# 0xPolygonHermez/pil2-stark-js

Measured on AMD Instinct MI355X. Metric: STARK prove time (ms_per_step) and trace-cells/s, synthetic Fibonacci AIR, GL Poseidon Merkle + FRI, blow-up 8, higher is better.
Workload: dtype u64; 1 GPU; full proof (commit, Q, evals, FRI 27/22/17/12/7, 64 queries) of 2^24 rows x 100 cols -> 2^27 rows, plain linear hash, per GPU; mode=prove, config=c3, nBits=24, nCols=100, nBitsExt=27, hash=GL-Poseidon-12, parallelism=single GPU

## Files before the change

### include/pil2gl.h

```cpp
#pragma once
#include <stdint.h>
#include "pil2gl_expr.h"
#include "pil2gl_bn_expr.h"
#ifdef __cplusplus
extern "C" {
#endif

#define PIL2GL_OK        0
#define PIL2GL_EINVAL   -1
#define PIL2GL_ENODEV   -2
#define PIL2GL_ENOMEM   -3
#define PIL2GL_EHIP     -4

int         pil2gl_init(int device);
void        pil2gl_shutdown(void);
const char *pil2gl_last_error(void);
int         pil2gl_version(void);
int         pil2gl_device_info(char *name, uint32_t nameLen, uint32_t *numCUs, uint64_t *totalMem);

int pil2gl_dev_alloc(uint64_t nWords, uint64_t **out);
int pil2gl_dev_free(uint64_t *p);
int pil2gl_dev_zero(uint64_t *p, uint64_t nWords, void *stream);
int pil2gl_dev_upload(uint64_t *dst, const uint64_t *hostSrc, uint64_t nWords);
int pil2gl_dev_download(uint64_t *hostDst, const uint64_t *src, uint64_t nWords);
int pil2gl_sync(void *stream);

int pil2gl_host_alloc(uint64_t nWords, uint64_t **out);
int pil2gl_host_free(uint64_t *p);
int pil2gl_host_register(uint64_t *p, uint64_t nWords);
int pil2gl_host_unregister(uint64_t *p);
int pil2gl_dev_upload_async(uint64_t *dst, const uint64_t *hostSrc, uint64_t nWords);
int pil2gl_dev_download_async(uint64_t *hostDst, const uint64_t *src, uint64_t nWords);
int pil2gl_copy_after(void *stream);
int pil2gl_copy_fence(void *stream);
int pil2gl_copy_sync(void);
int pil2gl_land_rows_dev(const uint64_t *src, uint64_t srcCols, uint64_t *dst, uint64_t dstCols, uint64_t nRows,
                         uint64_t *hostFirstBad, void *stream);
int pil2gl_dev_load_file(const char *fileName, uint64_t byteOffset, uint64_t nRows, uint64_t srcCols,
                         uint64_t *dst, uint64_t dstCols, uint64_t chunkWords, uint64_t *hostFirstBad);
int pil2gl_dev_save_file(const char *fileName, uint64_t byteOffset, const uint64_t *src, uint64_t nWords, uint64_t chunkWords);

int pil2gl_interpolate(const uint64_t *src, uint64_t nPols, uint32_t nBits, uint64_t *dst, uint32_t nBitsExt);
int pil2gl_interpolate_dev(const uint64_t *src, uint64_t nPols, uint32_t nBits, uint64_t *dst, uint32_t nBitsExt, void *stream);
int pil2gl_interpolate_cosets_dev(const uint64_t *src, uint64_t nPols, uint32_t nBits, uint64_t *dst, uint32_t nBitsExt,
                                  uint32_t cosetBegin, uint32_t cosetCount, void *stream);
int pil2gl_extend_cosets_unshifted_dev(const uint64_t *src, uint64_t nPols, uint32_t nBits, uint64_t *dst, uint32_t nBitsExt,
                                       uint32_t cosetBegin, uint32_t cosetCount, void *stream);
int pil2gl_extend_coefs_brev_dev(const uint64_t *coefBrev, uint64_t nPols, uint32_t nBits, uint64_t *dst, uint32_t nBitsExt, void *stream);
int pil2gl_extend_coefs_brev_cosets_dev(const uint64_t *coefBrev, uint64_t nPols, uint32_t nBits, uint64_t *dst, uint32_t nBitsExt,
                                        uint32_t cosetBegin, uint32_t cosetCount, void *stream);
int pil2gl_interpolate_cosets_ws_dev(const uint64_t *src, uint64_t nPols, uint32_t nBits, uint64_t *dst, uint32_t nBitsExt,
                                     uint32_t cosetBegin, uint32_t cosetCount, uint64_t *workspace, void *stream);
int pil2gl_fft(const uint64_t *src, uint64_t nPols, uint32_t nBits, uint64_t *dst);
int pil2gl_ifft(const uint64_t *src, uint64_t nPols, uint32_t nBits, uint64_t *dst);
int pil2gl_fft_dev(const uint64_t *src, uint64_t nPols, uint32_t nBits, uint64_t *dst, void *stream);
int pil2gl_ifft_dev(const uint64_t *src, uint64_t nPols, uint32_t nBits, uint64_t *dst, void *stream);
int pil2gl_fft_block_dev(uint64_t *buf, uint64_t start_pos, uint64_t nPols, uint32_t nBits, uint32_t s, uint32_t blockBits, uint32_t layers, void *stream);
int pil2gl_interpolate_prepare_block_dev(uint64_t *buf, uint64_t width, uint64_t height, uint64_t start, uint64_t inc, void *stream);

int pil2gl_poseidon(const uint64_t *in, const uint64_t *cap, uint64_t count, uint32_t nOut, uint64_t *out);
int pil2gl_poseidon_dev(const uint64_t *in, const uint64_t *cap, uint64_t count, uint32_t nOut, uint64_t *out, void *stream);
int pil2gl_sponge_absorb(const uint64_t *hostBlocks, uint64_t nBlocks, const uint64_t hostCap[4], uint64_t hostOut12[12]);
int pil2gl_linear_hash_rows(const uint64_t *in, uint64_t width, uint64_t height, int split, uint64_t *out);
int pil2gl_linear_hash_rows_dev(const uint64_t *in, uint64_t width, uint64_t height, int split, uint64_t *out, void *stream);
int pil2gl_merkelize_level(const uint64_t *in, uint64_t nOps, uint64_t *out);
int pil2gl_merkelize_level_dev(const uint64_t *in, uint64_t nOps, uint64_t *out, void *stream);
uint64_t pil2gl_merkle_num_nodes(uint64_t height);
int pil2gl_merkelize(const uint64_t *elems, uint64_t width, uint64_t height, int split, uint64_t *nodes);
int pil2gl_merkelize_dev(const uint64_t *elems, uint64_t width, uint64_t height, int split, uint64_t *nodes, void *stream);
int pil2gl_merkelize_digests_dev(uint64_t *nodes, uint64_t height, void *stream);
int pil2gl_group_proof_dev(const uint64_t *elems, const uint64_t *nodes, uint64_t width, uint64_t height,
                           uint64_t idx, uint64_t *hostVals, uint64_t *hostSiblings, uint32_t *nLevels);

int pil2gl_group_proofs_dev(const uint64_t *elems, const uint64_t *nodes, uint64_t width, uint64_t height,
                            const uint64_t *hostIdxs, uint32_t nIdx, uint64_t *hostOut, uint32_t *nLevels);
int pil2gl_roots_from_group_proofs(const uint64_t *hostProofs, uint64_t width, uint32_t levels, const uint64_t *hostIdxs, uint32_t nIdx,
                                   int splitLinearHash, uint64_t *hostRoots );

int pil2gl_fri_fold(const uint64_t *pol, uint32_t polBits, uint32_t outBits, uint64_t shiftInv,
                    const uint64_t challenge[3], uint64_t *out);
int pil2gl_fri_fold_dev(const uint64_t *pol, uint32_t polBits, uint32_t outBits, uint64_t shiftInv,
                        const uint64_t challenge[3], uint64_t *out, void *stream);
int pil2gl_fri_verify_fold(const uint64_t *groups, uint32_t foldBits, uint32_t nQueries, const uint64_t *sinv,
                           const uint64_t challenge[3], uint64_t *out );
int pil2gl_fri_verify_fold_dev(const uint64_t *groups, uint32_t foldBits, uint32_t nQueries, const uint64_t *sinv,
                               const uint64_t challenge[3], uint64_t *out, void *stream);
int pil2gl_fri_transpose(const uint64_t *pol, uint32_t polBits, uint32_t transposeBits, uint64_t *out);
int pil2gl_fri_transpose_dev(const uint64_t *pol, uint32_t polBits, uint32_t transposeBits, uint64_t *out, void *stream);

int pil2gl_build_x_dev(uint32_t nBits, uint64_t shift, uint64_t *x, void *stream);
int pil2gl_geometric_dev(uint64_t first, uint64_t ratio, uint64_t n, uint64_t *out, void *stream);
int pil2gl_build_zhinv_dev(uint32_t nBits, uint32_t nBitsExt, uint64_t *out, void *stream);
int pil2gl_build_one_row_zerofier_inv_dev(uint32_t nBits, uint32_t nBitsExt, uint64_t rowIndex, uint64_t *out, void *stream);
int pil2gl_build_frame_zerofier_dev(uint32_t nBits, uint32_t nBitsExt, uint64_t offsetMin, uint64_t offsetMax, uint64_t *out, void *stream);
int pil2gl_compute_q_split_dev(const uint64_t *qq1, uint32_t nBits, uint32_t nBitsExt, uint32_t qDim, uint32_t qDeg, uint64_t *qq2, void *stream);
int pil2gl_compute_q_split_brev_dev(const uint64_t *qq1, uint32_t nBits, uint32_t nBitsExt, uint32_t qDim, uint32_t qDeg, uint64_t *coefBrev, void *stream);
int pil2gl_compute_q_stark_dev(const glx_program *prog, const glx_ctx *ctx, uint32_t qSection, uint32_t nBits, uint32_t nBitsExt,
                               uint32_t qDim, uint32_t qDeg, uint64_t *dstExt, void *stream);
int pil2gl_x_div_x_sub_xi_dev(uint32_t nBitsExt, const uint64_t xi[3], uint64_t nOpen, uint64_t iOpen, uint64_t *out, void *stream);
int pil2gl_x_div_x_sub_xi_cosets_dev(uint32_t nBitsExt, uint32_t extBits, const uint64_t xi[3], uint64_t nOpen, uint64_t iOpen,
                                     uint32_t cosetBegin, uint32_t cosetCount, uint64_t *out, void *stream);
int pil2gl_build_lev_dev(uint32_t nBits, const uint64_t xi[3], uint64_t *lev, void *stream);
typedef struct { const uint64_t *buf; uint64_t width; uint64_t offset; uint32_t dim; uint32_t levIndex; } pil2gl_eval_desc;
int pil2gl_compute_evals_dev(const pil2gl_eval_desc *descs, uint32_t nEvals, uint32_t nBits, uint32_t extendBits,
                             const uint64_t *const *levs, uint32_t nLevs, uint64_t *hostEvals , void *stream);

int pil2gl_rows_dot_ext_dev(const uint64_t *buf, uint64_t width, uint64_t nRows, const uint64_t *hostCoef, uint32_t nOut,
                            uint64_t *acc, int accumulate, void *stream);
int pil2gl_rows_dot_ext_multi_dev(const uint64_t *const *bufs, const uint64_t *widths, uint32_t nBufs, uint64_t nRows,
                                  const uint64_t *const *hostCoefs, uint32_t nOut, uint64_t *acc, int accumulate, void *stream);
int pil2gl_rows_dot_ext_multi_step_dev(const uint64_t *const *bufs, const uint64_t *widths, uint32_t nBufs, uint64_t nRows, uint32_t rowStepBits,
                                       const uint64_t *const *hostCoefs, uint32_t nOut, uint64_t *acc, int accumulate, void *stream);
int pil2gl_fri_combine_dev(const uint64_t *acc, const uint64_t *hostK, const uint64_t vf1[3], const uint64_t *xDivXSubXi,
                           uint32_t nOpen, uint64_t nRows, uint64_t *f, void *stream);
int pil2gl_fri_combine_order_dev(const uint64_t *acc, const uint64_t *hostK, const uint64_t vf1[3], const uint64_t *xDivXSubXi,
                                 uint32_t nOpen, const uint32_t *order, uint64_t nRows, uint64_t *f, void *stream);
int pil2gl_compute_fri_pol_dev(const uint64_t *const *bufs, const uint64_t *widths, uint32_t nBufs, const uint64_t *const *hostCoefs, uint32_t nOpen,
                               const uint64_t *hostK, const uint64_t vf1[3], const uint32_t *order, const uint64_t *xis,
                               uint32_t nBits, uint32_t nBitsExt, uint64_t *fExt, void *stream);
int pil2gl_cols_dot_ext_dev(const uint64_t *buf, uint64_t width, uint64_t nRows, uint64_t rowStep, const uint64_t *const *levs,
                            uint32_t nLev, uint64_t *hostOut, void *stream);
int pil2gl_cols_dot_ext_multi_dev(const uint64_t *const *bufs, const uint64_t *widths, uint32_t nBufs, uint64_t nRows, uint64_t rowStep,
                                  const uint64_t *const *levs, uint32_t nLev, uint64_t *const *hostOuts, void *stream);
int pil2gl_cols_dot_ext_range_dev(const uint64_t *const *bufs, const uint64_t *strides, const uint64_t *colBegin, const uint64_t *widths, uint32_t nBufs,
                                  uint64_t nRows, uint64_t rowStep, const uint64_t *const *levs, uint32_t nLev, uint64_t *const *hostOuts, void *stream);

int pil2gl_eval_program_dev(const glx_program *prog, const glx_ctx *ctx, void *stream);
int pil2gl_jit_cache_set_dir(const char *dir);
int pil2gl_jit_cache_stats(uint64_t out[8]);
int pil2gl_precompile_program(const glx_program *prog, const glx_ctx *ctx, uint32_t outInfo[4]);
int pil2gl_precompile_q_stark(const glx_program *prog, const glx_ctx *ctx, uint32_t qSection, uint32_t nBits, uint32_t nBitsExt,
                              uint32_t qDim, uint32_t qDeg, uint32_t outInfo[4]);
int pil2gl_first_nonzero_row_dev(const uint64_t *col, uint32_t dim, uint64_t first, uint64_t last, uint64_t *hostRow, uint64_t *hostVal, void *stream);

int pil2gl_gprod_dev(const uint64_t *num, uint32_t dimNum, const uint64_t *den, uint32_t dimDen, uint64_t n, uint64_t *out, void *stream);
int pil2gl_gsum_dev(const uint64_t *num, uint32_t dimNum, const uint64_t *den, uint32_t dimDen, uint64_t n, uint64_t *out, void *stream);
int pil2gl_h1h2_dev(const uint64_t *f, const uint64_t *t, uint64_t n, uint32_t dim, uint64_t *h1, uint64_t *h2, void *stream);
int pil2gl_debug_hint_plan(uint64_t n, uint32_t *outInfo );
uint64_t pil2gl_debug_h1h2_home(const uint64_t *words, uint32_t dim, uint64_t capacity);

int pil2gl_bn128_poseidon(const uint64_t *in, const uint64_t *init, uint64_t count, uint32_t nIn, uint32_t nOut, uint64_t *out);
int pil2gl_bn128_sponge_absorb(const uint64_t *hostBlocks, uint64_t nBlocks, uint32_t nIn, const uint64_t hostInit[4], uint64_t *hostOut);
int pil2gl_bn128_poseidon_dev(const uint64_t *in, const uint64_t *init, uint64_t count, uint32_t nIn, uint32_t nOut, uint64_t *out, void *stream);
int pil2gl_bn128_linear_hash_rows(const uint64_t *in, uint64_t width, uint64_t height, uint32_t arity, int custom, uint64_t *out);
int pil2gl_bn128_linear_hash_rows_dev(const uint64_t *in, uint64_t width, uint64_t height, uint32_t arity, int custom, uint64_t *out, void *stream);
int pil2gl_bn128_merkelize_level_dev(const uint64_t *in, uint64_t nOps, uint32_t arity, uint64_t *out, void *stream);
uint64_t pil2gl_bn128_merkle_num_nodes(uint64_t height, uint32_t arity);
int pil2gl_bn128_merkelize(const uint64_t *elems, uint64_t width, uint64_t height, uint32_t arity, int custom, uint64_t *nodes);
int pil2gl_bn128_merkelize_dev(const uint64_t *elems, uint64_t width, uint64_t height, uint32_t arity, int custom, uint64_t *nodes, void *stream);
int pil2gl_bn128_group_proof_dev(const uint64_t *elems, const uint64_t *nodes, uint64_t width, uint64_t height, uint32_t arity,
                                 uint64_t idx, uint64_t *hostVals, uint64_t *hostSiblings, uint32_t *nLevels);
int pil2gl_bn128_group_proofs_dev(const uint64_t *elems, const uint64_t *nodes, uint64_t width, uint64_t height, uint32_t arity,
                                  const uint64_t *hostIdxs, uint32_t nIdx, uint64_t *hostVals, uint64_t *hostSiblings, uint32_t *nLevels);
int pil2gl_bn128_roots_from_group_proofs(const uint64_t *hostVals, const uint64_t *hostSiblings, uint64_t width, uint32_t levels, uint32_t arity,
                                         int custom, int siblingsMontgomery, const uint64_t *hostIdxs, uint32_t nIdx, uint64_t *hostRoots );
int pil2gl_bn128_convert(const uint64_t *in, uint64_t n, int toMontgomery, uint64_t *out);
int pil2gl_bn128_convert_dev(const uint64_t *in, uint64_t n, int toMontgomery, uint64_t *out, void *stream);

int pil2gl_bn128_fft(const uint64_t *src, uint64_t nPols, uint32_t nBits, uint64_t *dst);
int pil2gl_bn128_ifft(const uint64_t *src, uint64_t nPols, uint32_t nBits, uint64_t *dst);
int pil2gl_bn128_interpolate(const uint64_t *src, uint64_t nPols, uint32_t nBits, uint64_t *dstCoefs, uint64_t *dst, uint32_t nBitsExt);
int pil2gl_bn128_fft_dev(const uint64_t *src, uint64_t nPols, uint32_t nBits, uint64_t *dst, void *stream);
int pil2gl_bn128_ifft_dev(const uint64_t *src, uint64_t nPols, uint32_t nBits, uint64_t *dst, void *stream);
int pil2gl_bn128_interpolate_dev(const uint64_t *src, uint64_t nPols, uint32_t nBits, uint64_t *dstCoefs, uint64_t *dst, uint32_t nBitsExt, void *stream);
int pil2gl_debug_bn128_fft_plan(uint32_t nBits, uint32_t *layersPerSweep, uint32_t room, uint32_t *nSweeps);
uint32_t pil2gl_debug_bn128_fft_tile_bytes(void);

int pil2gl_bn128_g1_msm(const uint64_t *bases, const uint64_t *scalars, uint64_t n, uint64_t scalarStride, uint32_t scalarsMontgomery, uint64_t *out);
int pil2gl_bn128_g1_msm_dev(const uint64_t *bases, const uint64_t *scalars, uint64_t n, uint64_t scalarStride, uint32_t scalarsMontgomery,
                            uint64_t *out, void *stream);
int pil2gl_debug_bn128_msm_plan(uint64_t n, uint32_t *out, uint64_t *scratchBytes);
#define PIL2GL_G1_EMPTY_SLOT 0xFFFFFFFFu
typedef struct { uint64_t first, rows; uint32_t m, reserved; } pil2gl_g1_poly;
int pil2gl_bn128_g1_commit(const uint64_t *bases, uint64_t nBases, const uint64_t *scalars, uint64_t rowStride, uint32_t scalarsMontgomery,
                           const pil2gl_g1_poly *polys, uint32_t K, const uint32_t *slots, uint64_t *out);
int pil2gl_bn128_g1_commit_dev(const uint64_t *bases, uint64_t nBases, const uint64_t *scalars, uint64_t rowStride, uint32_t scalarsMontgomery,
                               const pil2gl_g1_poly *polys, uint32_t K, const uint32_t *slots, uint64_t *out, void *stream);
int pil2gl_debug_bn128_msm_batch_plan(uint32_t K, const uint64_t *counts, uint32_t *out, uint64_t *scratchBytes);
int pil2gl_debug_bn128_commit_locate(const pil2gl_g1_poly *polys, uint32_t K, const uint32_t *slots, uint64_t rowStride, uint64_t lane, uint64_t out[4]);
int pil2gl_debug_bn128_msm_digits(const uint64_t scalar[4], uint32_t c, int32_t *digits, uint32_t room, uint32_t *nDigits);

int pil2gl_bn128_eval_program(const glx_program *prog, const bnx_ctx *ctx);
int pil2gl_bn128_eval_program_dev(const glx_program *prog, const bnx_ctx *ctx, void *stream);
int pil2gl_bn128_first_nonzero_row_dev(const uint64_t *col, uint64_t width, uint64_t column, uint64_t first, uint64_t last,
                                       uint64_t *hostRow, uint64_t *hostVal, void *stream);
int pil2gl_debug_bn128_plan_program(const glx_program *prog, const bnx_ctx *ctx, uint32_t *outInfo );

int pil2gl_bn128_poly_div_xk_sub(const uint64_t *src, uint64_t n, uint64_t stride, uint64_t k, const uint64_t hostBeta[4], uint64_t *dst);
int pil2gl_bn128_poly_div_xk_sub_dev(const uint64_t *src, uint64_t n, uint64_t stride, uint64_t k, const uint64_t hostBeta[4], uint64_t *dst, void *stream);
int pil2gl_bn128_poly_eval(const uint64_t *src, uint64_t n, uint64_t stride, const uint64_t *hostPoints, uint32_t nPoints, uint64_t *out);
int pil2gl_bn128_poly_eval_dev(const uint64_t *src, uint64_t n, uint64_t stride, const uint64_t *hostPoints, uint32_t nPoints, uint64_t *out, void *stream);
int pil2gl_debug_bn128_poly_plan(uint64_t n, uint64_t k, uint32_t *outInfo , uint64_t *scratchBytes);

int pil2gl_bn128_poly_fma(uint64_t *acc, uint64_t nAcc, uint64_t accStride, const uint64_t *hostScale ,
                          const uint64_t *src, uint64_t nSrc, uint64_t srcStride,
                          const uint64_t *hostCoefs , const uint64_t *hostExps , uint32_t t);
int pil2gl_bn128_poly_fma_dev(uint64_t *acc, uint64_t nAcc, uint64_t accStride, const uint64_t *hostScale ,
                              const uint64_t *src, uint64_t nSrc, uint64_t srcStride,
                              const uint64_t *hostCoefs , const uint64_t *hostExps , uint32_t t, void *stream);
int pil2gl_bn128_poly_degree(const uint64_t *src, uint64_t n, uint64_t stride, uint64_t *degree);
int pil2gl_bn128_poly_degree_dev(const uint64_t *src, uint64_t n, uint64_t stride, uint64_t *degree, void *stream);

int pil2gl_bn128_batch_inverse(const uint64_t *src, uint64_t srcStride, uint64_t n, uint64_t *dst, uint64_t dstStride);
int pil2gl_bn128_batch_inverse_dev(const uint64_t *src, uint64_t srcStride, uint64_t n, uint64_t *dst, uint64_t dstStride, void *stream);
int pil2gl_bn128_gprod(const uint64_t *num, uint64_t numStride, const uint64_t *den, uint64_t denStride, uint64_t n,
                       uint64_t *out, uint64_t outStride);
int pil2gl_bn128_gprod_dev(const uint64_t *num, uint64_t numStride, const uint64_t *den, uint64_t denStride, uint64_t n,
                           uint64_t *out, uint64_t outStride, void *stream);
int pil2gl_bn128_gsum(const uint64_t hostNum[4], const uint64_t *den, uint64_t denStride, uint64_t n, uint64_t *out, uint64_t outStride);
int pil2gl_bn128_gsum_dev(const uint64_t hostNum[4], const uint64_t *den, uint64_t denStride, uint64_t n,
                          uint64_t *out, uint64_t outStride, void *stream);
int pil2gl_debug_bn128_scan_plan(uint64_t n, uint32_t op, uint32_t *outInfo , uint64_t *scratchBytes);

int pil2gl_bn128_h1h2(const uint64_t *f, uint64_t fStride, const uint64_t *t, uint64_t tStride, uint64_t n,
                      uint64_t *h1, uint64_t h1Stride, uint64_t *h2, uint64_t h2Stride, uint64_t *missingRow);
int pil2gl_bn128_h1h2_dev(const uint64_t *f, uint64_t fStride, const uint64_t *t, uint64_t tStride, uint64_t n,
                          uint64_t *h1, uint64_t h1Stride, uint64_t *h2, uint64_t h2Stride, uint64_t *missingRow, void *stream);
int pil2gl_debug_bn128_h1h2_plan(uint64_t n, uint32_t *outInfo , uint64_t *scratchBytes);

int pil2gl_wtns_adds_plan(const uint64_t *hostAddIdx, uint64_t idxStride, uint64_t nAdds, uint64_t nWitness, const uint64_t *hostCoef,
                          uint64_t coefStride, uint32_t coefWords, uint32_t *outAdds, uint64_t *outCoef, uint32_t *outLevelStart,
                          uint32_t levelCap, uint32_t *nLevels);
int pil2gl_wtns_adds_dev(uint64_t *w, uint64_t nWitness, const uint32_t *adds, const uint64_t *coefs, uint64_t nAdds,
                         const uint32_t *hostLevelStart, uint32_t nLevels, void *stream);
int pil2gl_bn128_wtns_adds_dev(uint64_t *w, uint64_t nWitness, const uint32_t *adds, const uint64_t *coefs, uint64_t nAdds,
                               const uint32_t *hostLevelStart, uint32_t nLevels, void *stream);
int pil2gl_wtns_gather_dev(const uint64_t *w, uint64_t nW, const uint32_t *sMap32, uint64_t nRows, uint64_t nCols, uint64_t *dst,
                           uint64_t dstCols, uint64_t *hostFirstBad, void *stream);
int pil2gl_bn128_wtns_gather_dev(const uint64_t *w, uint64_t nW, const uint32_t *sMap32, uint64_t nRows, uint64_t nCols, uint64_t *dst,
                                 uint64_t dstCols, int toMontgomery, uint64_t *hostFirstBad, void *stream);
int pil2gl_wtns_exec(const uint64_t *hostW, uint64_t nWitness, const uint64_t *hostAddIdx, const uint64_t *hostAddCoef, uint64_t nAdds,
                     const uint64_t *hostSMap64, uint64_t nRows, uint64_t nCols, uint64_t *hostDst);
int pil2gl_bn128_wtns_exec(const uint64_t *hostW, uint64_t nWitness, const uint64_t *hostAddIdx, const uint64_t *hostAddCoef, uint64_t nAdds,
                           const uint64_t *hostSMap64, uint64_t nRows, uint64_t nCols, uint64_t *hostDst, int toMontgomery);
int pil2gl_debug_wtns_plan(const uint64_t *hostAddIdx, uint64_t idxStride, uint64_t nAdds, uint64_t nWitness, uint32_t *outInfo ,
                           uint32_t *outWidths, uint32_t widthCap);

#define PIL2GL_CONN_SMAP_ROWS_U64 0
#define PIL2GL_CONN_SMAP_COLS_U32 1
int pil2gl_conn_plan(uint64_t nRows, uint64_t nCols, uint64_t nW, uint64_t N, uint32_t elemWords, uint32_t *outInfo , uint64_t *scratchBytes);
int pil2gl_conn_pols_dev(const uint32_t *sMap32, uint64_t nRows, uint64_t nCols, uint64_t nW, uint64_t N, const uint64_t *hostW, const uint64_t *hostKs1,
                         uint64_t *dst, uint64_t dstStride, uint64_t dstOffset, uint64_t *scratch, uint64_t scratchBytes, uint64_t *hostFirstBad,
                         void *stream);
int pil2gl_bn128_conn_pols_dev(const uint32_t *sMap32, uint64_t nRows, uint64_t nCols, uint64_t nW, uint64_t N, const uint64_t *hostW,
                               const uint64_t *hostKs1, uint64_t *dst, uint64_t dstStride, uint64_t dstOffset, uint64_t *scratch, uint64_t scratchBytes,
                               uint64_t *hostFirstBad, void *stream);
int pil2gl_conn_pols(const void *hostSMap, int sMapLayout, uint64_t nRows, uint64_t nCols, uint64_t nW, uint64_t N, const uint64_t *hostW,
                     const uint64_t *hostKs1, uint64_t *hostDst);
int pil2gl_bn128_conn_pols(const void *hostSMap, int sMapLayout, uint64_t nRows, uint64_t nCols, uint64_t nW, uint64_t N, const uint64_t *hostW,
                           const uint64_t *hostKs1, uint64_t *hostDst);

int pil2gl_conn_check_plan(uint64_t N, uint64_t nCols, uint32_t elemWords, uint32_t *outInfo , uint64_t *scratchBytes);
int pil2gl_conn_check_dev(const uint64_t *a, uint64_t aStride, uint64_t aOffset, const uint64_t *S, uint64_t sStride, uint64_t sOffset, uint64_t N,
                          uint64_t nCols, const uint64_t *hostW, const uint64_t *hostKs1, uint64_t *scratch, uint64_t scratchBytes,
                          uint64_t *hostReport , void *stream);
int pil2gl_bn128_conn_check_dev(const uint64_t *a, uint64_t aStride, uint64_t aOffset, const uint64_t *S, uint64_t sStride, uint64_t sOffset, uint64_t N,
                                uint64_t nCols, const uint64_t *hostW, const uint64_t *hostKs1, uint64_t *scratch, uint64_t scratchBytes,
                                uint64_t *hostReport , void *stream);
int pil2gl_conn_check(const uint64_t *hostA, const uint64_t *hostS, uint64_t N, uint64_t nCols, const uint64_t *hostW, const uint64_t *hostKs1,
                      uint64_t *hostReport );
int pil2gl_bn128_conn_check(const uint64_t *hostA, const uint64_t *hostS, uint64_t N, uint64_t nCols, const uint64_t *hostW, const uint64_t *hostKs1,
                            uint64_t *hostReport );
uint64_t pil2gl_debug_conn_check_probe(void);

int pil2gl_tuple_check_plan(uint64_t n, uint64_t k, uint32_t elemWords, uint32_t mode, uint32_t *outInfo , uint64_t *scratchBytes);
int pil2gl_tuple_check_dev(const uint64_t *f, uint64_t fStride, const uint64_t *hostFCols, const uint64_t *t, uint64_t tStride,
                           const uint64_t *hostTCols, const uint64_t *selF, uint64_t selFStride, uint64_t selFCol, const uint64_t *selT,
                           uint64_t selTStride, uint64_t selTCol, uint64_t n, uint64_t k, uint32_t mode, uint64_t *scratch,
                           uint64_t scratchBytes, uint64_t *hostReport , void *stream);
int pil2gl_bn128_tuple_check_dev(const uint64_t *f, uint64_t fStride, const uint64_t *hostFCols, const uint64_t *t, uint64_t tStride,
                                 const uint64_t *hostTCols, const uint64_t *selF, uint64_t selFStride, uint64_t selFCol, const uint64_t *selT,
                                 uint64_t selTStride, uint64_t selTCol, uint64_t n, uint64_t k, uint32_t mode, uint64_t *scratch,
                                 uint64_t scratchBytes, uint64_t *hostReport , void *stream);
int pil2gl_tuple_check(const uint64_t *hostF, uint64_t fStride, const uint64_t *hostFCols, const uint64_t *hostT, uint64_t tStride,
                       const uint64_t *hostTCols, const uint64_t *hostSelF, uint64_t selFStride, uint64_t selFCol, const uint64_t *hostSelT,
                       uint64_t selTStride, uint64_t selTCol, uint64_t n, uint64_t k, uint32_t mode, uint64_t *hostReport );
int pil2gl_bn128_tuple_check(const uint64_t *hostF, uint64_t fStride, const uint64_t *hostFCols, const uint64_t *hostT, uint64_t tStride,
                             const uint64_t *hostTCols, const uint64_t *hostSelF, uint64_t selFStride, uint64_t selFCol,
                             const uint64_t *hostSelT, uint64_t selTStride, uint64_t selTCol, uint64_t n, uint64_t k, uint32_t mode,
                             uint64_t *hostReport );
uint64_t pil2gl_debug_tuple_home(const uint64_t *words, uint64_t k, uint32_t elemWords, uint64_t capacity);
uint64_t pil2gl_debug_tuple_check_probe(void);

typedef struct pil2gl_tuple_side {
    const uint64_t *base;
    uint64_t stride;
    const uint64_t *hostCols;
    const uint64_t *sel;
    uint64_t selStride, selCol;
} pil2gl_tuple_side;
int pil2gl_lookup_mult_plan(uint64_t n, uint64_t k, uint64_t nF, uint32_t elemWords, uint32_t *outInfo , uint64_t *scratchBytes);
int pil2gl_lookup_mult_dev(const pil2gl_tuple_side *hostF, uint64_t nF, const pil2gl_tuple_side *hostT, uint64_t *m, uint64_t mStride,
                           uint64_t mCol, uint64_t n, uint64_t k, uint64_t *scratch, uint64_t scratchBytes, uint64_t *hostReport ,
                           void *stream);
int pil2gl_bn128_lookup_mult_dev(const pil2gl_tuple_side *hostF, uint64_t nF, const pil2gl_tuple_side *hostT, uint64_t *m, uint64_t mStride,
                                 uint64_t mCol, uint64_t n, uint64_t k, uint64_t *scratch, uint64_t scratchBytes,
                                 uint64_t *hostReport , void *stream);
int pil2gl_lookup_mult(const pil2gl_tuple_side *hostF, uint64_t nF, const pil2gl_tuple_side *hostT, uint64_t *hostM, uint64_t mStride,
                       uint64_t mCol, uint64_t n, uint64_t k, uint64_t *hostReport );
int pil2gl_bn128_lookup_mult(const pil2gl_tuple_side *hostF, uint64_t nF, const pil2gl_tuple_side *hostT, uint64_t *hostM, uint64_t mStride,
                             uint64_t mCol, uint64_t n, uint64_t k, uint64_t *hostReport );
uint64_t pil2gl_debug_lookup_mult_probe(void);

int pil2gl_synth_fibonacci_dev(uint32_t nBits, uint32_t nPairs, const uint64_t *hostInit, uint64_t *cm, void *stream);

uint64_t pil2gl_add(uint64_t a, uint64_t b);
uint64_t pil2gl_mul(uint64_t a, uint64_t b);
uint64_t pil2gl_square(uint64_t a);

int pil2gl_selftest_field(const uint64_t *a, const uint64_t *b, uint64_t n, uint64_t *mul, uint64_t *add, uint64_t *sub);
int pil2gl_debug_compact_program(const glx_program *prog, glx_op *outOps, uint32_t *outInfo);
int pil2gl_debug_jit_compile(const glx_program *prog, const glx_ctx *ctx, uint64_t *codeBytes, uint32_t *fusedOps);
int pil2gl_debug_plan_program(const glx_program *prog, const glx_ctx *ctx, uint32_t *outInfo);
uint64_t pil2gl_debug_bn128_path_launches(void);
#define PIL2GL_PLAN_FFT 0
#define PIL2GL_PLAN_IFFT 1
#define PIL2GL_PLAN_INTERPOLATE 2
#define PIL2GL_PLAN_EXTEND_COEFS 3
#define PIL2GL_PLAN_LAUNCH_WORDS 14
int pil2gl_debug_plan_transform(uint32_t op, uint32_t nBits, uint64_t nPols, uint32_t nBitsExt, uint32_t cosetCount,
                                uint32_t *out, uint32_t maxLaunches, uint32_t *nLaunches);
#define PIL2GL_PLAN_GRID_WORDS 5
int pil2gl_debug_plan_transform_grid(uint32_t op, uint32_t nBits, uint64_t nPols, uint32_t nBitsExt, uint32_t cosetCount,
                                     uint32_t *out, uint32_t maxLaunches, uint32_t *nLaunches);
int pil2gl_debug_transform_walk(uint32_t op, uint32_t nBits, uint64_t nPols, uint32_t nBitsExt, uint32_t cosetCount, uint32_t launch,
                                uint32_t firstBlock, uint32_t count, uint32_t *out);
int pil2gl_debug_transform_walk_cover(uint32_t op, uint32_t nBits, uint64_t nPols, uint32_t nBitsExt, uint32_t cosetCount, uint32_t launch,
                                      uint64_t *counts);
int pil2gl_selftest_products(const uint64_t *a, const uint64_t *b, uint64_t n, uint64_t *x, uint64_t *pb, uint64_t *flag);
int pil2gl_selftest_mds(const uint64_t *states, uint64_t n, uint32_t layers, int mfma, uint64_t *out);
int pil2gl_selftest_poseidon(const uint64_t *states, uint64_t n, int what, uint64_t *out);
int pil2gl_selftest_clock(uint32_t iters, double *mhz);
int pil2gl_selftest_ext(const uint64_t *a, const uint64_t *b, uint64_t n, uint64_t *mul, uint64_t *inv);

#ifdef __cplusplus
}
#endif
```

### pil2-stark-js_amd/csrc/expr.hip

```cpp
#include "common.h"
#include "gl_field.cuh"
#include <vector>
#include <string.h>
#include <algorithm>
#include <array>
#include <map>
#include <stdlib.h>

using namespace gl;

namespace {

struct DevRef { u32 kind_dim;
                u32 section;
                int32_t rowOff;
                u32 index; };
struct DevOp { u32 op; u32 aux; DevRef dest, src[2]; };

enum { GLX_LZ_BEGIN = 4, GLX_LZ_MAD = 5, GLX_LZ_END = 6 };

#define GLX_MAX_SECTIONS 24
struct DevCtx {
    const DevOp *__restrict__ ops; u32 nOps;
    u32 nBits;
// ... 49 lines not shown
    extern __shared__ u64 lds_tmp[];
    u64 *T; u32 stride;
    if (LDS_TMP) { T = lds_tmp + threadIdx.x; stride = blockDim.x; }
    else { T = gtmp + (size_t)blockIdx.x * blockDim.x + threadIdx.x; stride = gridDim.x * blockDim.x; }
    const u64 nRows = 1ull << c.nBits;
    for (u64 row = (u64)blockIdx.x * blockDim.x + threadIdx.x; row < nRows; row += (u64)gridDim.x * blockDim.x) {
        u64 LZ[3][6];
        for (u32 k = 0; k < c.nOps; k++) {
            const DevOp op = c.ops[k];
            u64 a0, a1, a2, b0 = 0, b1 = 0, b2 = 0, r0, r1, r2;
            if (op.op == GLX_LZ_BEGIN) {
#pragma unroll
                for (int q = 0; q < 3; q++)
#pragma unroll
                    for (int i = 0; i < 6; i++) LZ[q][i] = 0;
                continue;
            }
            if (op.op == GLX_LZ_MAD) {
                load_ref(op.src[0], c, row, T, stride, a0, a1, a2);
                const u32 *L = c.limbs + op.aux;
                lz_mad(LZ, a0, L);
                if ((op.src[0].kind_dim >> 8) == 3) { lz_mad(LZ, a1, L + 9); lz_mad(LZ, a2, L + 18); }
                continue;
            }
            const u32 da = op.src[0].kind_dim >> 8;
            u32 db = 1;
            if (op.op != GLX_LZ_END) load_ref(op.src[0], c, row, T, stride, a0, a1, a2);
            if (op.op < GLX_OP_COPY) { load_ref(op.src[1], c, row, T, stride, b0, b1, b2); db = op.src[1].kind_dim >> 8; }
            if (op.op == GLX_LZ_END) { r0 = fold6(LZ[0]); r1 = fold6(LZ[1]); r2 = fold6(LZ[2]); }
            else if (op.op == GLX_OP_ADD) {
                r0 = add(a0, b0);
                if (da == 3 && db == 3) { r1 = add(a1, b1); r2 = add(a2, b2); }
                else if (da == 3) { r1 = a1; r2 = a2; } else { r1 = b1; r2 = b2; }
            } else if (op.op == GLX_OP_SUB) {
                r0 = sub(a0, b0);
                if (da == 3 && db == 3) { r1 = sub(a1, b1); r2 = sub(a2, b2); }
                else if (da == 3) { r1 = a1; r2 = a2; } else { r1 = neg(b1); r2 = neg(b2); }
            } else if (op.op == GLX_OP_MUL) {
                if (da == 3 && db == 3) { E3 x = { { a0, a1, a2 } }, y = { { b0, b1, b2 } }; E3 z = e3_mul(x, y); r0 = z.v[0]; r1 = z.v[1]; r2 = z.v[2]; }
                else if (da == 3) { r0 = mul(a0, b0); r1 = mul(a1, b0); r2 = mul(a2, b0); }
                else { r0 = mul(a0, b0); r1 = mul(a0, b1); r2 = mul(a0, b2); }
            } else { r0 = a0; r1 = a1; r2 = a2; }
            const DevRef d = op.dest;
            if ((d.kind_dim & 0xff) == GLX_TMP) {
                u64 *t = T + (size_t)(3 * d.index) * stride;
                t[0] = r0; t[stride] = r1; t[2 * (size_t)stride] = r2;
            } else {
                const u64 mask = (1ull << c.nBits) - 1;
                const u64 rr = (row + (u64)(int64_t)d.rowOff) & mask;
                u64 *q = c.secPtr[d.section] + rr * c.secWidth[d.section] + d.index;
                q[0] = r0;
                if ((d.kind_dim >> 8) == 3) { q[1] = r1; q[2] = r2; }
            }
        }
    }
}

}

using namespace pil2gl;

struct IOp { u32 op; u32 aux; glx_ref dest; glx_ref src[2]; };
static inline int n_src(u32 op) { return op < GLX_OP_COPY ? 2 : (op == GLX_OP_COPY || op == GLX_LZ_MAD) ? 1 : 0; }
static inline bool has_dest(u32 op) { return op <= GLX_OP_COPY || op == GLX_LZ_END; }

static int validate_program(const glx_program *prog, const glx_ctx *ctx) {
    for (u32 k = 0; k < prog->nOps; k++) {
        const glx_op &o = prog->ops[k];
        if (o.op > GLX_OP_COPY) return fail(PIL2GL_EINVAL, "Invalid op: %u", o.op);
        const int ns = o.op == GLX_OP_COPY ? 1 : 2;
        for (int s = 0; s < ns + 1; s++) {
            const glx_ref &r = s < ns ? o.src[s] : o.dest;
            if (r.dim != 1 && r.dim != 3) return fail(PIL2GL_EINVAL, "invalid dim %u in op %u", r.dim, k);
            if (r.kind == GLX_TMP) { if (r.index >= prog->nTmp) return fail(PIL2GL_EINVAL, "tmp %u out of range in op %u", r.index, k); }
            else if (r.kind == GLX_SEC) {
                if (!ctx) continue;
                if (r.section >= ctx->nSections) return fail(PIL2GL_EINVAL, "section %u out of range in op %u", r.section, k);
                if ((u64)r.index + r.dim > ctx->sections[r.section].width) return fail(PIL2GL_EINVAL, "column %u out of range in op %u", r.index, k);
            } else if (r.kind == GLX_SCALAR) {
                if (s == ns) return fail(PIL2GL_EINVAL, "Invalid reference type set");
                if (ctx && (u64)r.index + r.dim > ctx->nScalars) return fail(PIL2GL_EINVAL, "scalar %u out of range in op %u", r.index, k);
            } else return fail(PIL2GL_EINVAL, "Invalid reference type get");
        }
    }
    return PIL2GL_OK;
}

static int value_number(const glx_program *prog, const glx_ctx *ctx, std::vector<IOp> &out, u32 &nVal) {
    std::map<std::array<u64, 4>, u32> scalarIndex;
    struct Key { u32 op; u64 a, b; bool operator<(const Key &o) const { return op != o.op ? op < o.op : a != o.a ? a < o.a : b < o.b; } };
    std::map<Key, u32> table;
    std::map<std::pair<u64, u64>, u32> loads;
    std::vector<u32> valDim;
    const u32 NONE = 0xFFFFFFFFu;
    std::vector<u32> cur(prog->nTmp, NONE);
    auto tmp_ref = [&](u32 v) { glx_ref r; memset(&r, 0, sizeof r); r.kind = GLX_TMP; r.dim = (uint8_t)valDim[v]; r.index = v; return r; };
    auto operand_key = [](const glx_ref &r) { return ((u64)r.kind << 60) | ((u64)r.dim << 56) | (u64)r.index; };
    out.clear();
    for (u32 k = 0; k < prog->nOps; k++) {
        const glx_op &o = prog->ops[k];
        const int ns = o.op == GLX_OP_COPY ? 1 : 2;
        glx_ref src[2]; memset(src, 0, sizeof src);
        for (int s = 0; s < ns; s++) {
            const glx_ref &r = o.src[s];
            if (r.kind == GLX_TMP) {
                if (cur[r.index] == NONE) return fail(PIL2GL_EINVAL, "tmp %u read before written in op %u", r.index, k);
                src[s] = tmp_ref(cur[r.index]);
                src[s].dim = r.dim < src[s].dim ? r.dim : src[s].dim;
            } else if (r.kind == GLX_SEC) {
                const std::pair<u64, u64> lk(((u64)r.section << 40) | ((u64)r.dim << 32) | (u32)r.prime, r.index);
                auto it = loads.find(lk);
                if (it == loads.end()) {
                    const u32 v = (u32)valDim.size(); valDim.push_back(r.dim);
                    IOp ld; memset(&ld, 0, sizeof ld); ld.op = GLX_OP_COPY; ld.dest = tmp_ref(v); ld.src[0] = r;
                    out.push_back(ld);
                    it = loads.emplace(lk, v).first;
                }
                src[s] = tmp_ref(it->second);
            } else {
                src[s] = r;
                if (ctx && ctx->scalars) {
                    const u64 *w = ctx->scalars + r.index;
                    const std::array<u64, 4> key = { r.dim, w[0], r.dim == 3 ? w[1] : 0, r.dim == 3 ? w[2] : 0 };
                    src[s].index = scalarIndex.emplace(key, r.index).first->second;
                }
            }
        }
        if (o.dest.kind == GLX_SEC) {
            IOp st; memset(&st, 0, sizeof st); st.op = o.op; st.dest = o.dest; st.src[0] = src[0]; st.src[1] = src[1];
            out.push_back(st);
            for (auto it = loads.begin(); it != loads.end();) { if ((it->first.first >> 40) == o.dest.section) it = loads.erase(it); else ++it; }
            continue;
        }
        if (o.op == GLX_OP_COPY && src[0].kind == GLX_TMP && src[0].dim == o.dest.dim) { cur[o.dest.index] = src[0].index; continue; }
        Key key = { o.op | ((u32)o.dest.dim << 8), operand_key(src[0]), ns == 2 ? operand_key(src[1]) : 0 };
        if ((o.op == GLX_OP_ADD || o.op == GLX_OP_MUL) && key.b < key.a) std::swap(key.a, key.b);
        auto it = table.find(key);
        if (it == table.end()) {
            const u32 v = (u32)valDim.size(); valDim.push_back(o.dest.dim);
            IOp n; memset(&n, 0, sizeof n); n.op = o.op; n.dest = tmp_ref(v); n.src[0] = src[0]; n.src[1] = src[1];
            out.push_back(n);
            it = table.emplace(key, v).first;
        }
        cur[o.dest.index] = it->second;
    }
    nVal = (u32)valDim.size();
    return PIL2GL_OK;
}

static void push_limbs(std::vector<u32> &pool, u64 v) {
    pool.push_back((u32)v & 0x3FFFFF); pool.push_back((u32)(v >> 22) & 0x3FFFFF); pool.push_back((u32)(v >> 44));
}

static void fuse_horner(std::vector<IOp> &ops, u32 nVal, const glx_ctx *ctx, std::vector<u32> &limbPool) {
    const u32 NONE = 0xFFFFFFFFu;
    std::vector<u32> def(nVal, NONE), uses(nVal, 0);
    for (u32 k = 0; k < ops.size(); k++) {
        for (int s = 0; s < n_src(ops[k].op); s++) if (ops[k].src[s].kind == GLX_TMP) uses[ops[k].src[s].index]++;
        if (has_dest(ops[k].op) && ops[k].dest.kind == GLX_TMP) def[ops[k].dest.index] = k;
    }
    struct Link { u32 mulIdx, addIdx; glx_ref X, A, C; };
    auto link_at = [&](u32 k, Link &L) {
        const IOp &a = ops[k];
        if (a.op != GLX_OP_ADD || a.dest.dim != 3) return false;
        for (int s = 0; s < 2; s++) {
            const glx_ref &m = a.src[s];
            if (m.kind != GLX_TMP || uses[m.index] != 1 || def[m.index] == NONE) continue;
            const IOp &mu = ops[def[m.index]];
            if (mu.op != GLX_OP_MUL) continue;
            for (int t = 0; t < 2; t++) {
                if (mu.src[t].kind == GLX_SCALAR && mu.src[t].dim == 3 && mu.src[1 - t].kind != GLX_SEC) {
                    L.mulIdx = def[m.index]; L.addIdx = k; L.X = mu.src[t]; L.A = mu.src[1 - t]; L.C = a.src[1 - s];
                    return L.C.kind != GLX_SEC;
                }
            }
        }
        return false;
    };
    std::vector<bool> removed(ops.size(), false);
    std::vector<std::vector<IOp>> insertAt(ops.size());
    u32 busyUntil = 0;
    std::vector<bool> consumed(ops.size(), false);
    for (u32 k = (u32)ops.size(); k-- > 0;) {
        Link L;
        if (consumed[k] || !link_at(k, L)) continue;
        std::vector<Link> chain; chain.push_back(L);
        for (;;) {
            const glx_ref &A = chain.back().A;
            if (A.kind != GLX_TMP || uses[A.index] != 1 || def[A.index] == NONE) break;
            Link P2;
            if (!link_at(def[A.index], P2) || P2.X.index != L.X.index) break;
            chain.push_back(P2);
        }
        const u32 n = (u32)chain.size();
        if (n < 4 || n > 300) continue;
        const u32 first = chain.back().mulIdx, last = chain.front().addIdx;
        if (busyUntil && last >= busyUntil) continue;
        bool ordered = true;
        for (u32 i = 0; i + 1 < n; i++) ordered &= chain[i + 1].addIdx < chain[i].mulIdx;
        if (!ordered) continue;
        busyUntil = first;
        const u64 *xp = ctx->scalars + L.X.index;
        std::vector<std::array<u64, 3>> pw(n + 1);
        pw[0] = { 1, 0, 0 };
        for (u32 i = 1; i <= n; i++) { u64 t[3]; h_e3_mul(pw[i - 1].data(), xp, t); pw[i] = { t[0], t[1], t[2] }; }
        auto weight = [&](const std::array<u64, 3> &W, u32 dim) {
            const u32 off = (u32)limbPool.size();
            std::array<u64, 3> w = W;
            for (u32 t = 0; t < dim; t++) {
                for (int q = 0; q < 3; q++) push_limbs(limbPool, w[q]);
                w = { w[2], h_add(w[0], w[2]), w[1] };
            }
            return off;
        };
        auto mad = [&](const glx_ref &v, const std::array<u64, 3> &W) {
            IOp m; memset(&m, 0, sizeof m); m.op = GLX_LZ_MAD; m.src[0] = v; m.aux = weight(W, v.dim); return m;
        };
        for (u32 i = 0; i < n; i++) { removed[chain[i].mulIdx] = true; removed[chain[i].addIdx] = true; consumed[chain[i].addIdx] = true; }
        IOp bg; memset(&bg, 0, sizeof bg); bg.op = GLX_LZ_BEGIN;
        insertAt[first].push_back(bg);
        insertAt[first].push_back(mad(chain[n - 1].A, pw[n]));
        for (u32 i = 0; i < n; i++) {
            const Link &lk = chain[n - 1 - i];
            insertAt[lk.addIdx].push_back(mad(lk.C, pw[n - 1 - i]));
        }
        IOp en; memset(&en, 0, sizeof en); en.op = GLX_LZ_END; en.dest = ops[last].dest;
        insertAt[last].push_back(en);
    }
    std::vector<IOp> res;
    for (u32 k = 0; k < ops.size(); k++) {
        for (const IOp &i : insertAt[k]) res.push_back(i);
        if (!removed[k]) res.push_back(ops[k]);
    }
    ops.swap(res);
}

static int allocate_slots(std::vector<IOp> &ops, u32 nVal, u32 &nSlots) {
    const u32 NONE = 0xFFFFFFFFu;
    std::vector<u32> lastUse(nVal, NONE);
    for (u32 k = 0; k < ops.size(); k++)
        for (int s = 0; s < n_src(ops[k].op); s++) if (ops[k].src[s].kind == GLX_TMP) lastUse[ops[k].src[s].index] = k;
    std::vector<u32> slotOf(nVal, NONE), freeSlots;
    nSlots = 0;
    for (u32 k = 0; k < ops.size(); k++) {
        IOp &o = ops[k];
        u32 dying[2]; int nd = 0;
        for (int s = 0; s < n_src(o.op); s++) {
            glx_ref &r = o.src[s];
            if (r.kind != GLX_TMP) continue;
            const u32 id = r.index;
            if (slotOf[id] == NONE) return fail(PIL2GL_EINVAL, "internal: value %u used before definition", id);
            r.index = slotOf[id];
            if (lastUse[id] == k && !(nd == 1 && dying[0] == id)) dying[nd++] = id;
        }
        for (int f = 0; f < nd; f++) { freeSlots.push_back(slotOf[dying[f]]); slotOf[dying[f]] = NONE; }
        if (has_dest(o.op) && o.dest.kind == GLX_TMP) {
            const u32 id = o.dest.index;
            if (!freeSlots.empty()) { slotOf[id] = freeSlots.back(); freeSlots.pop_back(); }
            else slotOf[id] = nSlots++;
            o.dest.index = slotOf[id];
            if (lastUse[id] == NONE) { freeSlots.push_back(slotOf[id]); slotOf[id] = NONE; }
        }
    }
    return PIL2GL_OK;
}

static int compile_program(const glx_program *prog, const glx_ctx *ctx, std::vector<IOp> &ops, u32 &nSlots, std::vector<u32> &limbPool, bool fuse) {
    P2_TRY(validate_program(prog, ctx));
    u32 nVal = 0;
    P2_TRY(value_number(prog, ctx, ops, nVal));
    if (fuse && ctx && ctx->scalars) fuse_horner(ops, nVal, ctx, limbPool);
    return allocate_slots(ops, nVal, nSlots);
}

extern "C" int pil2gl_debug_compact_program(const glx_program *prog, glx_op *outOps, uint32_t *nSlots ) {
    if (!prog || !outOps || !nSlots) return fail(PIL2GL_EINVAL, "null argument");
    std::vector<IOp> ops; std::vector<u32> pool; u32 n = 0;
    P2_TRY(compile_program(prog, nullptr, ops, n, pool, false));
    if (ops.size() > 2ull * prog->nOps + 16) return fail(PIL2GL_EINVAL, "internal: program grew unexpectedly");
    for (size_t k = 0; k < ops.size(); k++) { memset(&outOps[k], 0, sizeof(glx_op)); outOps[k].op = ops[k].op; outOps[k].dest = ops[k].dest; outOps[k].src[0] = ops[k].src[0]; outOps[k].src[1] = ops[k].src[1]; }
    nSlots[0] = n; nSlots[1] = (uint32_t)ops.size();
    return PIL2GL_OK;
}

#include <hip/hiprtc.h>
#include <sstream>
#include <set>
#include <string>

static const char *kFieldSrc =
#include "gl_field_src.inc"
    ;

struct JitArgs {
    const u64 *scalars; const u32 *limbs; u64 *sec[GLX_MAX_SECTIONS]; u32 nBits; u32 pad_;
};
struct JitEntry { hipModule_t mod; hipFunction_t fn; };
static std::map<std::string, JitEntry> g_jit_cache;
namespace pil2gl {
void jit_clear() {
    std::lock_guard<std::recursive_mutex> lk(runtime_lock());
    for (auto &kv : g_jit_cache) (void)hipModuleUnload(kv.second.mod);
    g_jit_cache.clear();
}
}

static std::string jit_source(const std::vector<IOp> &ops, u32 nSlots, const glx_ctx *ctx) {
    std::ostringstream o;
    o << "typedef unsigned long uint64_t; typedef unsigned int uint32_t; typedef long int64_t; typedef int int32_t;\n" << kFieldSrc << "\nusing namespace gl;\n";
    o << "struct JitArgs { const u64 *scalars; const u32 *limbs; u64 *sec[" << GLX_MAX_SECTIONS << "]; u32 nBits; u32 pad_; };\n";
    o << "__device__ __forceinline__ u64 fold6(const u64 S[6]) { u64 r = canon(S[0]); r = add(r, mul(S[1], 1ull << 22)); r = add(r, mul(S[2], 1ull << 44));"
         " r = add(r, mul(S[3], 1ull << 32)); r = add(r, mul(S[4], 1ull << 54)); r = add(r, mul(S[5], ((1ull << 32) - 1) << 12)); return r; }\n";
    o << "__device__ __forceinline__ void lz_mad(u64 S[3][6], u64 v, const u32 *__restrict__ L) { const u32 p0 = (u32)v, p1 = (u32)(v >> 32);\n"
         " _Pragma(\"unroll\") for (int k = 0; k < 3; k++) { const u32 w0 = L[3*k], w1 = L[3*k+1], w2 = L[3*k+2];\n"
         "  S[k][0] += (u64)p0 * w0; S[k][1] += (u64)p0 * w1; S[k][2] += (u64)p0 * w2; S[k][3] += (u64)p1 * w0; S[k][4] += (u64)p1 * w1; S[k][5] += (u64)p1 * w2; } }\n";
    o << "__device__ __noinline__ E3 e3_mul_call(E3 a, E3 b) { return e3_mul(a, b); }\n";
    const char *mcEnv = getenv("PIL2GL_EXPR_MULCALL");
    const bool mulCall = mcEnv ? mcEnv[0] == '1' : ops.size() >= 200;
    const char *lzEnv = getenv("PIL2GL_EXPR_LAZYMUL");
    const bool lazyMul = !(lzEnv && lzEnv[0] == '0');
    const std::string MULC = mulCall ? "mul_call(" : "mul(", MULC_END = ")";
    const std::string MULL = (mulCall && lazyMul) ? "mull_call(" : MULC, MULL_END = ")";
    if (mulCall) {
        o << "__device__ __noinline__ u64 mul_call(u64 a, u64 b) { return " << (lazyMul ? "canon(mul_lazy_x(a, b))" : "mul(a, b)") << "; }\n";
        if (lazyMul) o << "__device__ __noinline__ u64 mull_call(u64 a, u64 b) { return mul_lazy_x(a, b); }\n";
    }
    std::vector<bool> lazyOK(ops.size(), false);
    for (size_t k = 0; k < ops.size(); k++) {
        const IOp &p = ops[k];
        if (p.op != GLX_OP_MUL || p.dest.kind != GLX_TMP || (p.src[0].dim == 3 && p.src[1].dim == 3)) continue;
        bool ok = true, live = true;
        for (size_t j = k + 1; j < ops.size() && ok && live; j++) {
            const IOp &q = ops[j];
            for (int t = 0; t < n_src(q.op); t++) {
                if (q.src[t].kind != GLX_TMP || q.src[t].index != p.dest.index) continue;
                const bool tolerant = q.op == GLX_LZ_MAD || (q.op == GLX_OP_MUL && !(q.src[0].dim == 3 && q.src[1].dim == 3));
                ok &= tolerant;
            }
            if (has_dest(q.op) && q.dest.kind == GLX_TMP && q.dest.index == p.dest.index) live = false;
        }
        lazyOK[k] = ok;
    }
    auto row_off = [&](const glx_ref &r) { return (int64_t)r.prime * ((int64_t)1 << ctx->primeShift); };
    o << "extern \"C\" __global__ void __launch_bounds__(256) jit_eval(JitArgs A) {\n";
    o << " const u64 row = (u64)blockIdx.x * blockDim.x + threadIdx.x; if (row >= (1ull << A.nBits)) return;\n";
    o << " const u64 mask = (1ull << A.nBits) - 1; const u64 *__restrict__ SC = A.scalars; const u32 *__restrict__ LM = A.limbs;\n";
    o << " u64 LZ[3][6];\n";
    for (u32 s = 0; s < nSlots; s++) o << " u64 t" << s << "_0 = 0, t" << s << "_1 = 0, t" << s << "_2 = 0;\n";
    auto addr = [&](const glx_ref &r) {
        std::ostringstream a;
        a << "A.sec[" << r.section << "] + ((row + (u64)(" << row_off(r) << "ll)) & mask) * " << ctx->sections[r.section].width << "ull + " << r.index;
        return a.str();
    };
    auto rd = [&](const glx_ref &r, int c) {
        std::ostringstream a;
        if (c >= (int)r.dim) { a << "0ull"; return a.str(); }
        if (r.kind == GLX_TMP) a << "t" << r.index << "_" << c;
        else if (r.kind == GLX_SCALAR) a << "SC[" << (r.index + c) << "]";
        else a << "(" << addr(r) << ")[" << c << "]";
        return a.str();
    };
    for (size_t k = 0; k < ops.size(); k++) {
        const IOp &p = ops[k];
        if (p.op == GLX_LZ_BEGIN) { o << " for (int q = 0; q < 3; q++) for (int i = 0; i < 6; i++) LZ[q][i] = 0;\n"; continue; }
        if (p.op == GLX_LZ_MAD) {
            o << " lz_mad(LZ, " << rd(p.src[0], 0) << ", LM + " << p.aux << ");";
            if (p.src[0].dim == 3) o << " lz_mad(LZ, " << rd(p.src[0], 1) << ", LM + " << p.aux + 9 << "); lz_mad(LZ, " << rd(p.src[0], 2) << ", LM + " << p.aux + 18 << ");";
            o << "\n"; continue;
        }
        const glx_ref &a = p.src[0], &b = p.src[1];
        std::string r[3];
        const u32 da = a.dim, db = b.dim;
        switch (p.op) {
        case GLX_LZ_END: r[0] = "fold6(LZ[0])"; r[1] = "fold6(LZ[1])"; r[2] = "fold6(LZ[2])"; break;
        case GLX_OP_ADD:
            r[0] = "add(" + rd(a, 0) + ", " + rd(b, 0) + ")";
            for (int c = 1; c < 3; c++) r[c] = (da == 3 && db == 3) ? "add(" + rd(a, c) + ", " + rd(b, c) + ")" : da == 3 ? rd(a, c) : rd(b, c);
            break;
        case GLX_OP_SUB:
            r[0] = "sub(" + rd(a, 0) + ", " + rd(b, 0) + ")";
            for (int c = 1; c < 3; c++) r[c] = (da == 3 && db == 3) ? "sub(" + rd(a, c) + ", " + rd(b, c) + ")" : da == 3 ? rd(a, c) : "neg(" + rd(b, c) + ")";
            break;
        case GLX_OP_MUL:
            if (da == 3 && db == 3) {
                o << " { E3 x_ = { { " << rd(a, 0) << ", " << rd(a, 1) << ", " << rd(a, 2) << " } }, y_ = { { " << rd(b, 0) << ", " << rd(b, 1) << ", " << rd(b, 2) << " } }; E3 z_ = e3_mul_call(x_, y_);";
                r[0] = "z_.v[0]"; r[1] = "z_.v[1]"; r[2] = "z_.v[2]";
            } else {
                const std::string &M = lazyOK[k] ? MULL : MULC, &ME = lazyOK[k] ? MULL_END : MULC_END;
                if (da == 3) { for (int c = 0; c < 3; c++) r[c] = M + rd(a, c) + ", " + rd(b, 0) + ME; }
                else { for (int c = 0; c < 3; c++) r[c] = c < (int)db || c == 0 ? M + rd(a, 0) + ", " + rd(b, c) + ME : "0ull"; }
            }
            break;
        default: for (int c = 0; c < 3; c++) r[c] = rd(a, c); break;
        }
        const glx_ref &d = p.dest;
        const bool braced = (p.op == GLX_OP_MUL && da == 3 && db == 3);
        if (!braced) o << " {";
        if (d.kind == GLX_TMP) {
            o << " const u64 n0_ = " << r[0] << ", n1_ = " << (d.dim == 3 ? r[1] : "0ull") << ", n2_ = " << (d.dim == 3 ? r[2] : "0ull") << ";";
            o << " t" << d.index << "_0 = n0_; t" << d.index << "_1 = n1_; t" << d.index << "_2 = n2_; }\n";
        } else {
            o << " u64 *q_ = " << addr(d) << "; q_[0] = " << r[0] << ";";
            if (d.dim == 3) o << " q_[1] = " << r[1] << "; q_[2] = " << r[2] << ";";
            o << " }\n";
        }
    }
    o << "}\n";
    return o.str();
}

static std::string jit_arch() {
    int dev = 0;
    hipDeviceProp_t pr;
    if (hipGetDevice(&dev) == hipSuccess && hipGetDeviceProperties(&pr, dev) == hipSuccess && pr.gcnArchName[0]) {
        std::string a(pr.gcnArchName);
        return a.substr(0, a.find(':'));
    }
    (void)hipGetLastError();
    return "gfx950";
}

static std::vector<std::string> jit_options(const std::string &arch) {
    return { "--offload-arch=" + arch, "-O3", "-ffp-contract=off" };
}
static int jit_build(const std::string &src, std::vector<char> &code) {
    if (const char *dump = getenv("PIL2GL_EXPR_DUMP")) {
        if (FILE *f = fopen(dump, "w")) { fwrite(src.data(), 1, src.size(), f); fclose(f); }
    }
    hiprtcProgram prog;
    if (hiprtcCreateProgram(&prog, src.c_str(), "pil2gl_expr.hip", 0, nullptr, nullptr) != HIPRTC_SUCCESS) return fail(PIL2GL_EHIP, "hiprtcCreateProgram failed");
    const std::vector<std::string> optStr = jit_options(jit_arch());
    std::vector<const char *> opts;
    for (const std::string &o : optStr) opts.push_back(o.c_str());
    hiprtcResult rc = hiprtcCompileProgram(prog, (int)opts.size(), opts.data());
    if (rc != HIPRTC_SUCCESS) {
        size_t n = 0; hiprtcGetProgramLogSize(prog, &n);
        std::string log(n, 0); if (n) hiprtcGetProgramLog(prog, &log[0]);
        hiprtcDestroyProgram(&prog);
        return fail(PIL2GL_EHIP, "hiprtc compile failed: %.300s", log.c_str());
    }
    size_t sz = 0; hiprtcGetCodeSize(prog, &sz);
    code.resize(sz); hiprtcGetCode(prog, code.data());
    hiprtcDestroyProgram(&prog);
    return PIL2GL_OK;
}

#include <errno.h>
#include <fcntl.h>
#include <sys/stat.h>
#include <unistd.h>
#include <chrono>

#define JIT_FILE_VERSION 1u
static const char kJitMagic[8] = { 'P', '2', 'G', 'L', 'J', 'I', 'T', 0 };
enum { JS_MEM_HITS, JS_DISK_HITS, JS_COMPILES, JS_DISK_WRITES, JS_REJECTED, JS_FAILED_WRITES, JS_COMPILE_NS, JS_LOAD_NS };
static u64 g_jit_stats[8];
static std::string g_jit_dir;
static bool g_jit_dir_init = false;

static inline u64 rotl64(u64 x, int r) { return (x << r) | (x >> (64 - r)); }
static inline u64 avalanche64(u64 x) { x ^= x >> 33; x *= 0xFF51AFD7ED558CCDull; x ^= x >> 33; x *= 0xC4CEB9FE1A85EC53ull; x ^= x >> 33; return x; }
static void jit_hash128(const void *data, size_t n, u64 out[2]) {
    const unsigned char *p = (const unsigned char *)data;
    u64 a = 0x9E3779B97F4A7C15ull ^ (u64)n, b = 0xC2B2AE3D27D4EB4Full + (u64)n;
    for (size_t i = 0; i < n; i += 8) {
        u64 w = 0;
        const size_t m = n - i < 8 ? n - i : 8;
        for (size_t k = 0; k < m; k++) w |= (u64)p[i + k] << (8 * k);
        a = rotl64(a ^ w, 27) * 0x87C37B91114253D5ull + 0x52DCE729ull;
        b = rotl64(b + w, 31) * 0x4CF5AD432745937Full ^ (a >> 29);
    }
    a += b; b += a;
    a = avalanche64(a); b = avalanche64(b ^ rotl64(a, 17));
    out[0] = a + b; out[1] = b;
}

struct JitIdent { std::string arch, opts; int rtcMajor, rtcMinor; };
static JitIdent jit_ident() {
    JitIdent id; id.arch = jit_arch(); id.rtcMajor = id.rtcMinor = 0;
    for (const std::string &o : jit_options(id.arch)) { if (!id.opts.empty()) id.opts += '\n'; id.opts += o; }
    (void)hiprtcVersion(&id.rtcMajor, &id.rtcMinor);
    return id;
}
static std::string jit_key(const JitIdent &id, const std::string &src) {
    std::string all = "p2gl-jit " + std::to_string(JIT_FILE_VERSION) + "\n" + id.arch + "\n" + id.opts + "\n" + std::to_string(id.rtcMajor) + "." + std::to_string(id.rtcMinor) + "\n";
    all += src;
    u64 h[2]; jit_hash128(all.data(), all.size(), h);
    char hex[33]; snprintf(hex, sizeof hex, "%016llx%016llx", (unsigned long long)h[0], (unsigned long long)h[1]);
    return hex;
}
static void put_u32(std::string &s, u32 v) { for (int k = 0; k < 4; k++) s += (char)(v >> (8 * k)); }
static void put_u64(std::string &s, u64 v) { for (int k = 0; k < 8; k++) s += (char)(v >> (8 * k)); }
static u64 get_le(const unsigned char *p, int n) { u64 v = 0; for (int k = 0; k < n; k++) v |= (u64)p[k] << (8 * k); return v; }

static std::string jit_dir_apply(const char *dir) {
    if (!dir || !dir[0]) { g_jit_dir.clear(); return ""; }
    if (mkdir(dir, 0700) != 0 && errno != EEXIST) return std::string("cannot create ") + dir + ": " + strerror(errno);
    struct stat st;
    if (stat(dir, &st) != 0 || !S_ISDIR(st.st_mode)) return std::string(dir) + " is not a directory";
    if (access(dir, R_OK | W_OK | X_OK) != 0) return std::string(dir) + " cannot be written: " + strerror(errno);
    g_jit_dir = dir;
    return "";
}
static void jit_dir_init() {
    if (g_jit_dir_init) return;
    g_jit_dir_init = true;
    const std::string why = jit_dir_apply(getenv("PIL2GL_JIT_CACHE_DIR"));
    if (!why.empty()) fprintf(stderr, "pil2gl: PIL2GL_JIT_CACHE_DIR ignored (%s)\n", why.c_str());
}
static u64 now_ns() { return (u64)std::chrono::duration_cast<std::chrono::nanoseconds>(std::chrono::steady_clock::now().time_since_epoch()).count(); }

static int jit_disk_load(const std::string &path, const JitIdent &id, const std::string &src, std::vector<char> &code) {
    const int fd = open(path.c_str(), O_RDONLY | O_NOFOLLOW | O_CLOEXEC);
    if (fd < 0) return errno == ENOENT ? 0 : -1;
    struct stat st;
    std::vector<unsigned char> f;
    bool ok = fstat(fd, &st) == 0 && S_ISREG(st.st_mode) && st.st_uid == geteuid() && (st.st_mode & 022) == 0 && st.st_size >= 64 && st.st_size < ((off_t)1 << 31);
    if (ok) {
        f.resize((size_t)st.st_size);
        size_t got = 0;
        while (got < f.size()) { const ssize_t r = read(fd, f.data() + got, f.size() - got); if (r <= 0) break; got += (size_t)r; }
        char extra;
        ok = got == f.size() && read(fd, &extra, 1) == 0;
    }
    close(fd);
    if (!ok) return -1;
    if (memcmp(f.data(), kJitMagic, 8) != 0 || get_le(&f[8], 4) != JIT_FILE_VERSION) return -1;
    const u64 hdr = get_le(&f[12], 4), aLen = get_le(&f[24], 4), oLen = get_le(&f[28], 4), sLen = get_le(&f[32], 8), cLen = get_le(&f[40], 8);
    if ((int)get_le(&f[16], 4) != id.rtcMajor || (int)get_le(&f[20], 4) != id.rtcMinor) return -1;
    if (aLen != id.arch.size() || oLen != id.opts.size() || sLen != src.size() || hdr != 64 + aLen + oLen || cLen == 0) return -1;
    if (cLen > f.size() || hdr + sLen + cLen != f.size()) return -1;
    if (memcmp(&f[64], id.arch.data(), aLen) != 0 || memcmp(&f[64 + aLen], id.opts.data(), oLen) != 0 || memcmp(&f[hdr], src.data(), sLen) != 0) return -1;
    u64 sum[2]; jit_hash128(&f[hdr + sLen], cLen, sum);
    if (sum[0] != get_le(&f[48], 8) || sum[1] != get_le(&f[56], 8)) return -1;
    code.assign((const char *)&f[hdr + sLen], (const char *)&f[hdr + sLen] + cLen);
    return 1;
}
static bool jit_disk_store(const std::string &path, const JitIdent &id, const std::string &src, const std::vector<char> &code) {
    std::string h(kJitMagic, 8);
    u64 sum[2]; jit_hash128(code.data(), code.size(), sum);
    put_u32(h, JIT_FILE_VERSION); put_u32(h, (u32)(64 + id.arch.size() + id.opts.size())); put_u32(h, (u32)id.rtcMajor); put_u32(h, (u32)id.rtcMinor);
    put_u32(h, (u32)id.arch.size()); put_u32(h, (u32)id.opts.size()); put_u64(h, src.size()); put_u64(h, code.size()); put_u64(h, sum[0]); put_u64(h, sum[1]);
    h += id.arch; h += id.opts;
    static unsigned serial = 0;
    const std::string tmp = path + ".tmp." + std::to_string((long)getpid()) + "." + std::to_string(serial++);
    const int fd = open(tmp.c_str(), O_WRONLY | O_CREAT | O_EXCL | O_NOFOLLOW | O_CLOEXEC, 0600);
    if (fd < 0) return false;
    bool ok = true;
    const struct { const char *p; size_t n; } parts[3] = { { h.data(), h.size() }, { src.data(), src.size() }, { code.data(), code.size() } };
    for (int k = 0; k < 3 && ok; k++)
        for (size_t put = 0; put < parts[k].n && ok;) { const ssize_t w = write(fd, parts[k].p + put, parts[k].n - put); if (w <= 0) ok = false; else put += (size_t)w; }
    ok = fchmod(fd, 0600) == 0 && ok;
    ok = close(fd) == 0 && ok;
    if (ok && rename(tmp.c_str(), path.c_str()) != 0) ok = false;
    if (!ok) (void)unlink(tmp.c_str());
    return ok;
}
static int jit_code(const std::string &src, std::vector<char> &code, u32 *origin) {
    jit_dir_init();
    JitIdent id; std::string path;
    if (!g_jit_dir.empty()) {
        const u64 t0 = now_ns();
        id = jit_ident();
        path = g_jit_dir + "/" + jit_key(id, src) + ".p2gl";
        const int r = jit_disk_load(path, id, src, code);
        g_jit_stats[JS_LOAD_NS] += now_ns() - t0;
        if (r == 1) { g_jit_stats[JS_DISK_HITS]++; if (origin) *origin = 2; return PIL2GL_OK; }
        if (r < 0) g_jit_stats[JS_REJECTED]++;
    }
    const u64 t0 = now_ns();
    P2_TRY(jit_build(src, code));
    g_jit_stats[JS_COMPILES]++; g_jit_stats[JS_COMPILE_NS] += now_ns() - t0;
    if (origin) *origin = 1;
    if (!g_jit_dir.empty()) g_jit_stats[jit_disk_store(path, id, src, code) ? JS_DISK_WRITES : JS_FAILED_WRITES]++;
    return PIL2GL_OK;
}
static int jit_get(const std::string &src, hipFunction_t *fn) {
    std::lock_guard<std::recursive_mutex> lk(runtime_lock());
    auto it = g_jit_cache.find(src);
    if (it != g_jit_cache.end()) { g_jit_stats[JS_MEM_HITS]++; *fn = it->second.fn; return PIL2GL_OK; }
    std::vector<char> code;
    P2_TRY(jit_code(src, code, nullptr));
    JitEntry e;
    HIP_TRY(hipModuleLoadData(&e.mod, code.data()));
    HIP_TRY(hipModuleGetFunction(&e.fn, e.mod, "jit_eval"));
    g_jit_cache.emplace(src, e);
    *fn = e.fn;
    return PIL2GL_OK;
}
extern "C" int pil2gl_jit_cache_set_dir(const char *dir) {
    std::lock_guard<std::recursive_mutex> lk(runtime_lock());
    const std::string why = jit_dir_apply(dir);
    if (!why.empty()) return fail(PIL2GL_EINVAL, "jit cache directory: %s", why.c_str());
    g_jit_dir_init = true;
    memset(g_jit_stats, 0, sizeof g_jit_stats);
    return PIL2GL_OK;
}
extern "C" int pil2gl_jit_cache_stats(uint64_t out[8]) {
    if (!out) return fail(PIL2GL_EINVAL, "null argument");
    std::lock_guard<std::recursive_mutex> lk(runtime_lock());
    for (int k = 0; k < 8; k++) out[k] = k >= JS_COMPILE_NS ? (g_jit_stats[k] + 500000) / 1000000 : g_jit_stats[k];
    return PIL2GL_OK;
}

static bool jit_routed(size_t nOps, u32 nBits, u32 nSlots) {
    const char *e = getenv("PIL2GL_EXPR_JIT");
    const bool want = e ? atoi(e) != 0 : (nOps >= 64 && nBits >= 16);
    return want && nSlots <= 200;
}
static int plan_program(const glx_program *prog, const glx_ctx *ctx, std::vector<IOp> &ops, u32 &nSlots, std::vector<u32> &limbPool) {
    P2_TRY(compile_program(prog, ctx, ops, nSlots, limbPool, getenv("PIL2GL_EXPR_NOFUSE") == nullptr));
    if (ctx->nSections > GLX_MAX_SECTIONS) return fail(PIL2GL_EINVAL, "too many sections (%u > %d)", ctx->nSections, GLX_MAX_SECTIONS);
    for (size_t k = 0; k < ops.size(); k++)
        for (int s = 0; s < 3; s++) {
            const glx_ref &r = s < 2 ? ops[k].src[s] : ops[k].dest;
            const int64_t off = (int64_t)r.prime * ((int64_t)1 << ctx->primeShift);
            if (off != (int64_t)(int32_t)off) return fail(PIL2GL_EINVAL, "row offset overflow in op %zu", k);
        }
    for (u32 i = 0; i < ctx->nSections; i++) if (ctx->sections[i].width >> 32) return fail(PIL2GL_EINVAL, "section %u too wide", i);
    return PIL2GL_OK;
}

extern "C" int pil2gl_precompile_program(const glx_program *prog, const glx_ctx *ctx, uint32_t outInfo[4]) {
    if (!prog || !ctx || !outInfo || (prog->nOps && !prog->ops) || (ctx->nSections && !ctx->sections)) return fail(PIL2GL_EINVAL, "null argument");
    if (ctx->nBits > 31) return fail(PIL2GL_EINVAL, "domain too large");
    std::lock_guard<std::recursive_mutex> lk(runtime_lock());
    jit_dir_init();
    if (g_jit_dir.empty()) return fail(PIL2GL_EINVAL, "no jit cache directory set (pil2gl_jit_cache_set_dir / PIL2GL_JIT_CACHE_DIR)");
    outInfo[0] = outInfo[1] = outInfo[2] = outInfo[3] = 0;
    if (prog->nOps == 0) return PIL2GL_OK;
    std::vector<IOp> ops; std::vector<u32> limbPool; u32 nSlots = 0;
    P2_TRY(plan_program(prog, ctx, ops, nSlots, limbPool));
    outInfo[3] = nSlots;
    if (!jit_routed(ops.size(), ctx->nBits, nSlots)) return PIL2GL_OK;
    std::vector<char> code; u32 origin = 0;
    P2_TRY(jit_code(jit_source(ops, nSlots, ctx), code, &origin));
    outInfo[0] = 1; outInfo[1] = origin; outInfo[2] = (uint32_t)code.size();
    return PIL2GL_OK;
}

extern "C" int pil2gl_debug_jit_compile(const glx_program *prog, const glx_ctx *ctx, uint64_t *codeBytes, uint32_t *fusedOps) {
    if (!prog || !ctx || !codeBytes) return fail(PIL2GL_EINVAL, "null argument");
    std::vector<IOp> ops; std::vector<u32> pool; u32 n = 0;
    P2_TRY(compile_program(prog, ctx, ops, n, pool, true));
    std::vector<char> code;
    P2_TRY(jit_build(jit_source(ops, n, ctx), code));
    *codeBytes = code.size();
    if (fusedOps) { u32 f = 0; for (const IOp &o : ops) f += o.op == GLX_LZ_MAD; *fusedOps = f; }
    return PIL2GL_OK;
}

extern "C" int pil2gl_debug_plan_program(const glx_program *prog, const glx_ctx *ctx, uint32_t *outInfo ) {
    if (!prog || !ctx || !outInfo) return fail(PIL2GL_EINVAL, "null argument");
    std::vector<IOp> ops; std::vector<u32> pool; u32 n = 0;
    P2_TRY(compile_program(prog, ctx, ops, n, pool, getenv("PIL2GL_EXPR_NOFUSE") == nullptr));
    u32 f = 0; for (const IOp &o : ops) f += o.op == GLX_LZ_MAD;
    outInfo[0] = n; outInfo[1] = (uint32_t)ops.size(); outInfo[2] = f;
    return PIL2GL_OK;
}

extern "C" int pil2gl_eval_program_dev(const glx_program *prog, const glx_ctx *ctx, void *stream) {
    P2_TRY(ensure_init());
    if (!prog || !ctx || (prog->nOps && !prog->ops)) return fail(PIL2GL_EINVAL, "null program");
    if (ctx->nBits > 31) return fail(PIL2GL_EINVAL, "domain too large");
    if (prog->nOps == 0) return PIL2GL_OK;
    hipStream_t st = as_stream(stream);
    std::vector<IOp> ops; std::vector<u32> limbPool; u32 nSlots = 0;
    P2_TRY(plan_program(prog, ctx, ops, nSlots, limbPool));
    std::vector<DevOp> dops(ops.size());
    for (size_t k = 0; k < ops.size(); k++) {
        auto cv = [&](const glx_ref &r) { DevRef d; d.kind_dim = (u32)r.kind | ((u32)r.dim << 8); d.section = r.section; d.rowOff = (int32_t)((int64_t)r.prime * ((int64_t)1 << ctx->primeShift)); d.index = r.index; return d; };
        dops[k].op = ops[k].op; dops[k].aux = ops[k].aux; dops[k].dest = cv(ops[k].dest); dops[k].src[0] = cv(ops[k].src[0]); dops[k].src[1] = cv(ops[k].src[1]);
    }
    const u64 opsWords = ((u64)dops.size() * sizeof(DevOp) + 7) / 8, limbWords = (limbPool.size() * 4 + 7) / 8;
    u64 *d;
    P2_TRY(scratch(SCR_EXPR_PROGRAM, opsWords + ctx->nScalars + limbWords + 2, &d));
    HIP_TRY(hipMemcpyAsync(d, dops.data(), dops.size() * sizeof(DevOp), hipMemcpyHostToDevice, st));
    if (ctx->nScalars) HIP_TRY(hipMemcpyAsync(d + opsWords, ctx->scalars, (u64)ctx->nScalars * 8, hipMemcpyHostToDevice, st));
    if (!limbPool.empty()) HIP_TRY(hipMemcpyAsync(d + opsWords + ctx->nScalars + 1, limbPool.data(), limbPool.size() * 4, hipMemcpyHostToDevice, st));
    DevCtx c;
    c.ops = (const DevOp *)d; c.nOps = (u32)dops.size();
    c.scalars = d + opsWords;
    c.limbs = (const u32 *)(d + opsWords + ctx->nScalars + 1);
    c.nBits = ctx->nBits;
    for (u32 i = 0; i < GLX_MAX_SECTIONS; i++) { c.secPtr[i] = i < ctx->nSections ? ctx->sections[i].ptr : nullptr; c.secWidth[i] = i < ctx->nSections ? (u32)ctx->sections[i].width : 0; }
    const u64 nRows = 1ull << ctx->nBits;
    {
        if (jit_routed(ops.size(), ctx->nBits, nSlots)) {
            hipFunction_t fn;
            if (jit_get(jit_source(ops, nSlots, ctx), &fn) != PIL2GL_OK) {
                static bool warned = false;
                if (!warned) { fprintf(stderr, "pil2gl: run-time compilation unavailable (%s); using the interpreter kernel\n", pil2gl_last_error()); warned = true; }
                goto interpreter;
            }
            if (getenv("PIL2GL_JIT_INFO") && getenv("PIL2GL_JIT_INFO")[0] == '1') {
                int regs = 0, lds = 0, loc = 0, maxt = 0;
                (void)hipFuncGetAttribute(&regs, HIP_FUNC_ATTRIBUTE_NUM_REGS, fn); (void)hipFuncGetAttribute(&lds, HIP_FUNC_ATTRIBUTE_SHARED_SIZE_BYTES, fn);
                (void)hipFuncGetAttribute(&loc, HIP_FUNC_ATTRIBUTE_LOCAL_SIZE_BYTES, fn); (void)hipFuncGetAttribute(&maxt, HIP_FUNC_ATTRIBUTE_MAX_THREADS_PER_BLOCK, fn);
                fprintf(stderr, "pil2gl jit_eval: %zu ops, regs %d, lds %d, scratch %d, max threads %d\n", ops.size(), regs, lds, loc, maxt);
            }
            JitArgs A; memset(&A, 0, sizeof A);
            A.scalars = c.scalars; A.limbs = c.limbs; A.nBits = ctx->nBits;
            for (u32 i = 0; i < ctx->nSections; i++) A.sec[i] = ctx->sections[i].ptr;
            size_t asz = sizeof A;
            void *cfg[] = { HIP_LAUNCH_PARAM_BUFFER_POINTER, &A, HIP_LAUNCH_PARAM_BUFFER_SIZE, &asz, HIP_LAUNCH_PARAM_END };
            HIP_TRY(hipModuleLaunchKernel(fn, (unsigned)((nRows + 255) / 256), 1, 1, 256, 1, 1, 0, st, nullptr, cfg));
            HIP_TRY(hipStreamSynchronize(st));
            return PIL2GL_OK;
        }
    }
interpreter:
    const u32 slots = nSlots ? nSlots : 1;
    if ((size_t)slots * 3 * 64 * 8 <= 60 * 1024) {
        u32 threads = 256;
        while ((size_t)slots * 3 * threads * 8 > 60 * 1024) threads /= 2;
        const size_t lds = (size_t)slots * 3 * threads * 8;
        HIP_TRY(hipFuncSetAttribute((const void *)eval_kernel<true>, hipFuncAttributeMaxDynamicSharedMemorySize, 64 * 1024));
        const u64 blocks = std::min<u64>((nRows + threads - 1) / threads, 256ull * 64);
        eval_kernel<true><<<(unsigned)blocks, threads, lds, st>>>(c, nullptr);
    } else {
        const u32 threads = 256;
        const u64 blocks = std::min<u64>((nRows + threads - 1) / threads, 256ull * 8);
        u64 *gtmp;
        P2_TRY(scratch(SCR_EXPR_TMP, (u64)slots * 3 * blocks * threads, &gtmp));
        eval_kernel<false><<<(unsigned)blocks, threads, 0, st>>>(c, gtmp);
    }
    KERNEL_CHECK();
    HIP_TRY(hipStreamSynchronize(st));
    return PIL2GL_OK;
}

__global__ void first_nonzero_kernel(const u64 *__restrict__ col, u32 dim, u64 first, u64 last, unsigned long long *__restrict__ best) {
    const u64 r = first + (u64)blockIdx.x * blockDim.x + threadIdx.x;
    bool nz = false;
    if (r < last) for (u32 k = 0; k < dim; k++) nz |= col[r * dim + k] != 0;
    const u64 mask = __ballot(nz);
    if (mask && (threadIdx.x & 63) == 0) atomicMin(best, (unsigned long long)(r + __builtin_ctzll(mask)));
}
extern "C" int pil2gl_first_nonzero_row_dev(const uint64_t *col, uint32_t dim, uint64_t first, uint64_t last, uint64_t *hostRow, uint64_t *hostVal, void *stream) {
    P2_TRY(ensure_init());
    if (!hostRow || !hostVal) return fail(PIL2GL_EINVAL, "null buffer");
    if (dim != 1 && dim != 3) return fail(PIL2GL_EINVAL, "dim must be 1 or 3 (got %u)", dim);
    if (last < first) return fail(PIL2GL_EINVAL, "empty range [%llu, %llu)", (unsigned long long)first, (unsigned long long)last);
    *hostRow = ~0ull;
    for (u32 k = 0; k < dim; k++) hostVal[k] = 0;
    if (last == first) return PIL2GL_OK;
    if (!col) return fail(PIL2GL_EINVAL, "null buffer");
    const u64 blocks = (last - first + 255) / 256;
    if (blocks > 0x7fffffffull) return fail(PIL2GL_EINVAL, "grid too large");
    hipStream_t st = as_stream(stream);
    u64 *d;
    P2_TRY(scratch(SCR_EXPR_PROGRAM, 1, &d));
    HIP_TRY(hipMemsetAsync(d, 0xff, 8, st));
    first_nonzero_kernel<<<(unsigned)blocks, 256, 0, st>>>(col, dim, first, last, (unsigned long long *)d);
    KERNEL_CHECK();
    HIP_TRY(hipMemcpyAsync(hostRow, d, 8, hipMemcpyDeviceToHost, st));
    HIP_TRY(hipStreamSynchronize(st));
    if (*hostRow != ~0ull) HIP_TRY(hipMemcpy(hostVal, col + *hostRow * dim, (size_t)dim * 8, hipMemcpyDeviceToHost));
    return PIL2GL_OK;
}
```

### pil2-stark-js_amd/csrc/merkle.hip

```cpp
#include "common.h"
#include <vector>
#include <string.h>
#include "poseidon_gl.cuh"
#include <algorithm>

using namespace gl;

namespace {

__device__ __forceinline__ void sponge(const u64 *__restrict__ v, u32 width, u64 digest[4], const MdsMfma &m) {
    u64 st[12];
    st[8] = st[9] = st[10] = st[11] = 0;
    for (u32 i = 0; i < width; i += 8) {
        const u32 n = min(8u, width - i);
#pragma unroll
        for (u32 j = 0; j < 8; j++) st[j] = j < n ? v[i + j] : 0;
        poseidon_perm<0, 4>(st, m);
        st[8] = st[0]; st[9] = st[1]; st[10] = st[2]; st[11] = st[3];
    }
    digest[0] = canon(st[8]); digest[1] = canon(st[9]); digest[2] = canon(st[10]); digest[3] = canon(st[11]);
}
__device__ __forceinline__ void linear_hash_plain(const u64 *__restrict__ v, u32 width, u64 digest[4], const MdsMfma &m) {
    if (width <= 4) {
#pragma unroll
// ... 82 lines not shown
    u64 *o = out + 4 * i;
    o[0] = st[0]; o[1] = st[1]; o[2] = st[2]; o[3] = st[3];
}

__global__ void __launch_bounds__(256, 2) merkle_path_roots_kernel(const u64 *__restrict__ leaf, const u64 *__restrict__ sib, const u64 *__restrict__ idx,
                                                                  u64 count, u32 levels, u64 *__restrict__ roots) {
    const u64 i0 = (u64)blockIdx.x * blockDim.x + threadIdx.x;
    const bool live = i0 < count;
    const u64 i = live ? i0 : count - 1;
    MdsMfma m;
    poseidon_init(m);
    u64 cur[4];
#pragma unroll
    for (int j = 0; j < 4; j++) cur[j] = canon(leaf[4 * i + j]);
    u64 pos = idx[i];
    for (u32 l = 0; l < levels; l++) {
        const u64 *s = sib + (i * levels + l) * 4;
        const bool right = pos & 1;
        u64 st[12];
#pragma unroll
        for (int j = 0; j < 4; j++) { const u64 sv = canon(s[j]); st[j] = right ? sv : cur[j]; st[4 + j] = right ? cur[j] : sv; }
        st[8] = st[9] = st[10] = st[11] = 0;
        poseidon_perm(st, m);
#pragma unroll
        for (int j = 0; j < 4; j++) cur[j] = st[j];
        pos >>= 1;
    }
    if (!live) return;
#pragma unroll
    for (int j = 0; j < 4; j++) roots[4 * i + j] = cur[j];
}

__global__ void __launch_bounds__(64) sponge_chain_kernel(const u64 *__restrict__ blocks, u64 nBlocks, const u64 *__restrict__ cap, u64 *__restrict__ out12) {
    constexpr u32 MC[12] = { 17, 15, 41, 16, 2, 28, 13, 13, 39, 18, 34, 20 };
    __shared__ u64 sh[12];
    const u32 lane = threadIdx.x;
    const bool act = lane < 12;
    const u32 l = act ? lane : 0;
    u32 mrow[12];
#pragma unroll
    for (int j = 0; j < 12; j++) mrow[j] = MC[(j + 12 - l) % 12] + ((l == 0 && j == 0) ? 8u : 0u);
    u64 carry = (act && l >= 8) ? canon(cap[l - 8]) : 0;
    u64 s = 0;
    for (u64 b = 0; b < nBlocks; b++) {
        s = l < 8 ? canon(blocks[8 * b + l]) : carry;
        for (int r = 0; r < 30; r++) {
            s = add_lazy_canon(s, POSEIDON_GL_RC[r * 12 + l]);
            const bool full = r < 4 || r >= 26;
            if (full || l == 0) s = pow7_lazy(s);
            if (act) sh[l] = s;
            __builtin_amdgcn_s_waitcnt(0xC07F);
            __builtin_amdgcn_wave_barrier();
            u64 al = 0, ah = 0;
#pragma unroll
            for (int j = 0; j < 12; j++) { const u64 v = sh[j]; al += (u64)(u32)v * mrow[j]; ah += (u64)(u32)(v >> 32) * mrow[j]; }
            __builtin_amdgcn_wave_barrier();
            const u64 lo = al + (ah << 32);
            const u64 hi = (ah >> 32) + (lo < al ? 1 : 0);
            s = reduce128_lazy(lo, hi);
        }
        s = canon(s);
        if (act) sh[l] = s;
        __builtin_amdgcn_s_waitcnt(0xC07F);
        __builtin_amdgcn_wave_barrier();
        carry = (l >= 8) ? sh[l - 8] : 0;
        __builtin_amdgcn_wave_barrier();
    }
    if (act) out12[l] = s;
}

__global__ void __launch_bounds__(256, 4) poseidon_batch_kernel(const u64 *__restrict__ in, const u64 *__restrict__ cap, u64 count, u32 nOut, u64 *__restrict__ out) {
    const u64 i0 = (u64)blockIdx.x * blockDim.x + threadIdx.x;
    const bool live = i0 < count;
    const u64 i = live ? i0 : count - 1;
    MdsMfma m;
    poseidon_init(m);
    u64 st[12];
#pragma unroll
    for (int j = 0; j < 8; j++) st[j] = canon(in[8 * i + j]);
#pragma unroll
    for (int j = 0; j < 4; j++) st[8 + j] = cap ? canon(cap[4 * i + j]) : 0;
    poseidon_perm(st, m);
    if (!live) return;
    for (u32 j = 0; j < nOut; j++) out[(u64)nOut * i + j] = st[j];
}

__global__ void __launch_bounds__(256, 2) mds_selftest_kernel(const u64 *__restrict__ in, u64 n, u32 layers, int mfma, u64 *__restrict__ out) {
    const u64 i0 = (u64)blockIdx.x * blockDim.x + threadIdx.x;
    const bool live = i0 < n;
    const u64 i = live ? i0 : n - 1;
    MdsMfma m;
    mds_mfma_init(m);
    u64 st[12];
#pragma unroll
    for (int j = 0; j < 12; j++) st[j] = in[12 * i + j];
    for (u32 l = 0; l < layers; l++) { if (mfma) mds_layer_mfma(st, m); else mds_layer(st); }
    if (!live) return;
#pragma unroll
    for (int j = 0; j < 12; j++) out[12 * i + j] = canon(st[j]);
}

__global__ void __launch_bounds__(256, 2) poseidon_selftest_kernel(const u64 *__restrict__ in, u64 n, int what, u64 *__restrict__ out) {
    const u64 i0 = (u64)blockIdx.x * blockDim.x + threadIdx.x;
    const bool live = i0 < n;
    const u64 i = live ? i0 : n - 1;
    MdsMfma m;
    mds_mfma_init(m);
    poseidon_init(m);
    u64 st[12];
#pragma unroll
    for (int j = 0; j < 12; j++) st[j] = in[12 * i + j];
    if (what == 0) poseidon_perm(st, m);
    else if (what == 1) poseidon_perm_single(st, m);
    else if (what == 2) poseidon_perm(st);
    else poseidon_partial_rounds(st, m, what == 3 ? 0 : 1);
    if (!live) return;
#pragma unroll
    for (int j = 0; j < 12; j++) out[12 * i + j] = canon(st[j]);
}

__global__ void __launch_bounds__(256, 4) clock_probe_kernel(u64 *__restrict__ sink, int iters, u64 *__restrict__ clk) {
    MdsMfma m;
    poseidon_init(m);
    u64 st[12];
    const u64 id = (u64)blockIdx.x * blockDim.x + threadIdx.x;
#pragma unroll
    for (int j = 0; j < 12; j++) st[j] = ((id * 12 + j) * 0x9E3779B97F4A7C15ull) >> 1;
    const u64 c0 = __builtin_readcyclecounter(), r0 = wall_clock64();
    for (int i = 0; i < iters; i++) poseidon_perm<0>(st, m);
    const u64 c1 = __builtin_readcyclecounter(), r1 = wall_clock64();
    u64 x = 0;
#pragma unroll
    for (int j = 0; j < 12; j++) x ^= st[j];
    sink[id] = x;
    if (threadIdx.x == 0) { clk[2 * blockIdx.x] = c1 - c0; clk[2 * blockIdx.x + 1] = r1 - r0; }
}

__global__ void group_proofs_kernel(const u64 *__restrict__ elems, const u64 *__restrict__ nodes, u64 width, u64 height,
                                    const u64 *__restrict__ idxs, u32 nLevels, u64 *__restrict__ out) {
    const u64 stride = width + 4ull * nLevels;
    u64 *o = out + (u64)blockIdx.x * stride;
    u64 idx = idxs[blockIdx.x];
    for (u64 c = threadIdx.x; c < width; c += blockDim.x) o[c] = elems[idx * width + c];
    if (threadIdx.x < 4) {
        u64 offset = 0, n = height * 4;
        for (u32 l = 0; l < nLevels; l++) {
            o[width + 4 * l + threadIdx.x] = nodes[offset + (idx ^ 1) * 4 + threadIdx.x];
            const u64 nextN = ((n - 1) / 8 + 1) * 4;
            offset += nextN * 2; n = nextN; idx >>= 1;
        }
    }
}

}

using namespace pil2gl;

extern "C" {

uint64_t pil2gl_merkle_num_nodes(uint64_t height) {
    if (height == 0) return 0;
    uint64_t n = height * 4;
    uint64_t nextN = ((n - 1) / 8 + 1) * 4;
    uint64_t acc = nextN * 2;
    while (n > 4) {
        n = nextN;
        nextN = ((n - 1) / 8 + 1) * 4;
        if (n > 4) acc += nextN * 2; else acc += 4;
    }
    return acc;
}

int pil2gl_linear_hash_rows_dev(const uint64_t *in, uint64_t width, uint64_t height, int split, uint64_t *out, void *stream) {
    P2_TRY(ensure_init());
    if (height == 0) return PIL2GL_OK;
    if (!out || (!in && width)) return fail(PIL2GL_EINVAL, "null buffer");
    if (width >= (1ull << 31)) return fail(PIL2GL_EINVAL, "row width too large");
    u64 blocks = (height + 255) / 256;
    if (blocks > 0x7fffffffull) return fail(PIL2GL_EINVAL, "grid too large");
    if (split && width > 8) linear_hash_split_kernel<<<(unsigned)((height + SPLIT_BLOCK - 1) / SPLIT_BLOCK), SPLIT_BLOCK, 0, as_stream(stream)>>>(in, width, height, out);
    else linear_hash_kernel<<<(unsigned)blocks, 256, 0, as_stream(stream)>>>(in, width, height, out);
    KERNEL_CHECK();
    return PIL2GL_OK;
}

int pil2gl_merkelize_level_dev(const uint64_t *in, uint64_t nOps, uint64_t *out, void *stream) {
    P2_TRY(ensure_init());
    if (nOps == 0) return PIL2GL_OK;
    if (!in || !out) return fail(PIL2GL_EINVAL, "null buffer");
    if (nOps > (0x7fffffffull << 8)) return fail(PIL2GL_EINVAL, "grid too large");
    merkle_level_kernel<<<(unsigned)((nOps + 255) / 256), 256, 0, as_stream(stream)>>>(in, nOps, out);
    KERNEL_CHECK();
    return PIL2GL_OK;
}

int pil2gl_poseidon_dev(const uint64_t *in, const uint64_t *cap, uint64_t count, uint32_t nOut, uint64_t *out, void *stream) {
    P2_TRY(ensure_init());
    if (count == 0) return PIL2GL_OK;
    if (!in || !out) return fail(PIL2GL_EINVAL, "null buffer");
    if (nOut < 1 || nOut > 12) return fail(PIL2GL_EINVAL, "nOut must be 1..12");
    if (count > (0x7fffffffull << 8)) return fail(PIL2GL_EINVAL, "grid too large");
    poseidon_batch_kernel<<<(unsigned)((count + 255) / 256), 256, 0, as_stream(stream)>>>(in, cap, count, nOut, out);
    KERNEL_CHECK();
    return PIL2GL_OK;
}

int pil2gl_merkelize_digests_dev(uint64_t *nodes, uint64_t height, void *stream) {
    P2_TRY(ensure_init());
    if (height == 0) return fail(PIL2GL_EINVAL, "height must be > 0");
    if (!nodes) return fail(PIL2GL_EINVAL, "null buffer");
    hipStream_t st = as_stream(stream);
    u64 total = pil2gl_merkle_num_nodes(height);
    if (total > height * 4) HIP_TRY(hipMemsetAsync(nodes + height * 4, 0, (total - height * 4) * 8, st));
    u64 pIn = 0, n64 = height * 4;
    u64 nextN64 = ((n64 - 1) / 8 + 1) * 4;
    u64 pOut = pIn + nextN64 * 2;
    while (n64 > 4) {
        P2_TRY(pil2gl_merkelize_level_dev(nodes + pIn, nextN64 / 4, nodes + pOut, stream));
        n64 = nextN64;
        nextN64 = ((n64 - 1) / 8 + 1) * 4;
        pIn = pOut;
        pOut = pIn + nextN64 * 2;
    }
    return PIL2GL_OK;
}

int pil2gl_merkelize_dev(const uint64_t *elems, uint64_t width, uint64_t height, int split, uint64_t *nodes, void *stream) {
    P2_TRY(ensure_init());
    if (height == 0) return fail(PIL2GL_EINVAL, "height must be > 0");
    if (!nodes || (!elems && width)) return fail(PIL2GL_EINVAL, "null buffer");
    P2_TRY(pil2gl_linear_hash_rows_dev(elems, width, height, split, nodes, stream));
    return pil2gl_merkelize_digests_dev(nodes, height, stream);
}

int pil2gl_group_proof_dev(const uint64_t *elems, const uint64_t *nodes, uint64_t width, uint64_t height,
                           uint64_t idx, uint64_t *hostVals, uint64_t *hostSiblings, uint32_t *nLevels) {
    P2_TRY(ensure_init());
    if (idx >= height) return fail(PIL2GL_EINVAL, "Out of range");
    if (!nodes || !hostSiblings || (width && (!elems || !hostVals))) return fail(PIL2GL_EINVAL, "null buffer");
    if (width) HIP_TRY(hipMemcpy(hostVals, elems + idx * width, width * 8, hipMemcpyDeviceToHost));
    u64 offset = 0, n = height * 4;
    uint32_t lvl = 0;
    while (n > 4) {
        u64 si = (idx ^ 1) * 4;
        HIP_TRY(hipMemcpy(hostSiblings + 4 * lvl, nodes + offset + si, 32, hipMemcpyDeviceToHost));
        u64 nextN = ((n - 1) / 8 + 1) * 4;
        offset += nextN * 2; n = nextN; idx >>= 1; lvl++;
    }
    if (nLevels) *nLevels = lvl;
    return PIL2GL_OK;
}

int pil2gl_group_proofs_dev(const uint64_t *elems, const uint64_t *nodes, uint64_t width, uint64_t height,
                            const uint64_t *hostIdxs, uint32_t nIdx, uint64_t *hostOut, uint32_t *nLevels) {
    P2_TRY(ensure_init());
    if (!nIdx) return PIL2GL_OK;
    if (!nodes || !hostIdxs || !hostOut || (!elems && width)) return fail(PIL2GL_EINVAL, "null buffer");
    u32 lv = 0;
    for (u64 n = height * 4; n > 4; n = ((n - 1) / 8 + 1) * 4) lv++;
    for (u32 i = 0; i < nIdx; i++) if (hostIdxs[i] >= height) return fail(PIL2GL_EINVAL, "Out of range");
    const u64 stride = width + 4ull * lv;
    u64 *d;
    P2_TRY(scratch(SCR_GROUP_PROOFS, (u64)nIdx * (stride + 1), &d));
    u64 *dIdx = d + (u64)nIdx * stride;
    HIP_TRY(hipMemcpy(dIdx, hostIdxs, (u64)nIdx * 8, hipMemcpyHostToDevice));
    group_proofs_kernel<<<nIdx, 64>>>(elems, nodes, width, height, dIdx, lv, d);
    KERNEL_CHECK();
    HIP_TRY(hipMemcpy(hostOut, d, (u64)nIdx * stride * 8, hipMemcpyDeviceToHost));
    if (nLevels) *nLevels = lv;
    return PIL2GL_OK;
}

int pil2gl_roots_from_group_proofs(const uint64_t *hostProofs, uint64_t width, uint32_t levels, const uint64_t *hostIdxs, uint32_t nIdx,
                                   int splitLinearHash, uint64_t *hostRoots) {
    P2_TRY(ensure_init());
    if (!nIdx) return PIL2GL_OK;
    if (!hostProofs || !hostIdxs || !hostRoots) return fail(PIL2GL_EINVAL, "null buffer");
    if (levels > 64) return fail(PIL2GL_EINVAL, "too many levels");
    const u64 stride = width + 4ull * levels, nv = (u64)nIdx * width, ns = (u64)nIdx * levels * 4;
    std::vector<u64> h(nv + ns + nIdx + 1);
    for (u32 q = 0; q < nIdx; q++) {
        memcpy(h.data() + (u64)q * width, hostProofs + q * stride, width * 8);
        memcpy(h.data() + nv + (u64)q * levels * 4, hostProofs + q * stride + width, 4ull * levels * 8);
        h[nv + ns + q] = hostIdxs[q];
    }
    u64 *d;
    P2_TRY(scratch(SCR_GROUP_PROOFS, nv + ns + nIdx + 8ull * nIdx + 1, &d));
    u64 *dVals = d, *dSib = d + nv, *dIdx = dSib + ns, *dLeaf = dIdx + nIdx, *dRoots = dLeaf + 4ull * nIdx;
    HIP_TRY(hipMemcpy(d, h.data(), (nv + ns + nIdx) * 8, hipMemcpyHostToDevice));
    P2_TRY(pil2gl_linear_hash_rows_dev(dVals, width, nIdx, splitLinearHash, dLeaf, nullptr));
    merkle_path_roots_kernel<<<(nIdx + 255) / 256, 256>>>(dLeaf, dSib, dIdx, nIdx, levels, dRoots);
    KERNEL_CHECK();
    HIP_TRY(hipMemcpy(hostRoots, dRoots, 4ull * nIdx * 8, hipMemcpyDeviceToHost));
    return PIL2GL_OK;
}

int pil2gl_sponge_absorb(const uint64_t *hostBlocks, uint64_t nBlocks, const uint64_t hostCap[4], uint64_t hostOut12[12]) {
    P2_TRY(ensure_init());
    if (!hostBlocks || !hostCap || !hostOut12) return fail(PIL2GL_EINVAL, "null buffer");
    if (nBlocks == 0) return fail(PIL2GL_EINVAL, "nothing to absorb");
    Stage s(8 * nBlocks + 4 + 12);
    const u64 *dBlocks = s.put(hostBlocks, 8 * nBlocks), *dCap = s.put(hostCap, 4);
    u64 *dOut = s.take(12);
    P2_TRY(s.rc());
    sponge_chain_kernel<<<1, 64>>>(dBlocks, nBlocks, dCap, dOut);
    KERNEL_CHECK();
    return s.get(hostOut12, dOut, 12);
}

int pil2gl_linear_hash_rows(const uint64_t *in, uint64_t width, uint64_t height, int split, uint64_t *out) {
    Stage s(width * height + height * 4);
    const u64 *dIn = s.put(in, width * height);
    u64 *dOut = s.take(height * 4);
    P2_TRY(s.rc());
    P2_TRY(pil2gl_linear_hash_rows_dev(dIn, width, height, split, dOut, nullptr));
    return s.get(out, dOut, height * 4);
}
int pil2gl_merkelize_level(const uint64_t *in, uint64_t nOps, uint64_t *out) {
    Stage s(nOps * 12);
    const u64 *dIn = s.put(in, nOps * 8);
    u64 *dOut = s.take(nOps * 4);
    P2_TRY(s.rc());
    P2_TRY(pil2gl_merkelize_level_dev(dIn, nOps, dOut, nullptr));
    return s.get(out, dOut, nOps * 4);
}
int pil2gl_poseidon(const uint64_t *in, const uint64_t *cap, uint64_t count, uint32_t nOut, uint64_t *out) {
    if (nOut < 1 || nOut > 12) return fail(PIL2GL_EINVAL, "nOut must be 1..12");
    const u64 nCap = cap ? count * 4 : 0;
    Stage s(count * 8 + nCap + count * nOut);
    const u64 *dIn = s.put(in, count * 8), *dCap = s.put(cap, nCap);
    u64 *dOut = s.take(count * nOut);
    P2_TRY(s.rc());
    P2_TRY(pil2gl_poseidon_dev(dIn, dCap, count, nOut, dOut, nullptr));
    return s.get(out, dOut, count * nOut);
}
int pil2gl_selftest_mds(const uint64_t *states, uint64_t n, uint32_t layers, int mfma, uint64_t *out) {
    if (n == 0) return PIL2GL_OK;
    Stage s(n * 24);
    const u64 *dIn = s.put(states, n * 12);
    u64 *dOut = s.take(n * 12);
    P2_TRY(s.rc());
    mds_selftest_kernel<<<(unsigned)((n + 255) / 256), 256>>>(dIn, n, layers, mfma, dOut);
    KERNEL_CHECK();
    return s.get(out, dOut, n * 12);
}
int pil2gl_selftest_poseidon(const uint64_t *states, uint64_t n, int what, uint64_t *out) {
    if (n == 0) return PIL2GL_OK;
    if (what < 0 || what > 4) return fail(PIL2GL_EINVAL, "what must be 0..4");
    Stage s(n * 24);
    const u64 *dIn = s.put(states, n * 12);
    u64 *dOut = s.take(n * 12);
    P2_TRY(s.rc());
    poseidon_selftest_kernel<<<(unsigned)((n + 255) / 256), 256>>>(dIn, n, what, dOut);
    KERNEL_CHECK();
    return s.get(out, dOut, n * 12);
}
int pil2gl_selftest_clock(uint32_t iters, double *mhz ) {
    P2_TRY(ensure_init());
    if (!mhz || iters == 0 || iters > 4096) return fail(PIL2GL_EINVAL, "iters must be 1..4096");
    const unsigned blocks = 256 * 4 * 8;
    u64 *d;
    P2_TRY(scratch(SCR_CLOCK_PROBE, (u64)blocks * 256 + 2ull * blocks, &d));
    clock_probe_kernel<<<blocks, 256>>>(d, (int)iters, d + (u64)blocks * 256);
    KERNEL_CHECK();
    std::vector<u64> h(2 * blocks);
    HIP_TRY(hipMemcpy(h.data(), d + (u64)blocks * 256, 16ull * blocks, hipMemcpyDeviceToHost));
    std::vector<double> v;
    for (unsigned i = 0; i < blocks; i++) if (h[2 * i + 1]) v.push_back(100.0 * (double)h[2 * i] / (double)h[2 * i + 1]);
    if (v.empty()) return fail(PIL2GL_EHIP, "no clock samples");
    std::sort(v.begin(), v.end());
    mhz[0] = v[v.size() / 2]; mhz[1] = v[v.size() / 20]; mhz[2] = v[v.size() * 19 / 20];
    return PIL2GL_OK;
}
int pil2gl_merkelize(const uint64_t *elems, uint64_t width, uint64_t height, int split, uint64_t *nodes) {
    if (height == 0) return fail(PIL2GL_EINVAL, "height must be > 0");
    const u64 nN = pil2gl_merkle_num_nodes(height);
    Stage s(width * height + nN);
    const u64 *dElems = s.put(elems, width * height);
    u64 *dNodes = s.take(nN);
    P2_TRY(s.rc());
    P2_TRY(pil2gl_merkelize_dev(dElems, width, height, split, dNodes, nullptr));
    return s.get(nodes, dNodes, nN);
}

}
```

### pil2-stark-js_amd/python/pil2gl/__init__.py

```python
import ctypes as C

import numpy as np

from . import _lib
from ._lib import Pil2glError, load, call

P = 0xFFFFFFFF00000001
SHIFT = 7

try:
    import torch
except Exception:
    torch = None


def _is_dev(b):
    return torch is not None and isinstance(b, torch.Tensor)


def _ptr(b):
    if b is None:
        return None
    if _is_dev(b):
        if not b.is_cuda:
# ... 178 lines not shown
        raise Pil2glError("h1h2_home: a key is dim words")
    home = int(load().pil2gl_debug_h1h2_home(C.c_void_p(w.ctypes.data), dim, capacity))
    if home == 0xFFFFFFFFFFFFFFFF:
        raise Pil2glError("h1h2_home: dim is 1 or 3 and the capacity a power of two")
    return home


def firstNonZeroRow(col, dim, first, last):
    row = np.zeros(1, np.uint64); val = np.zeros(3, np.uint64)
    call("pil2gl_first_nonzero_row_dev", _ptr(col), dim, first, last, _ptr(row), _ptr(val), _stream())
    return None if int(row[0]) == 0xFFFFFFFFFFFFFFFF else (int(row[0]), [int(v) for v in val[:dim]])


def poseidon(inputs, capacity=None, nOuts=4):
    if len(inputs) != 8:
        raise Pil2glError("Invalid Input size (must be 8)")
    if capacity is not None and len(capacity) != 4:
        raise Pil2glError("Invalid Capacity size (must be 4)")
    i = np.array([int(v) % P for v in inputs], dtype=np.uint64)
    c = np.array([int(v) % P for v in capacity], dtype=np.uint64) if capacity is not None else None
    o = np.zeros(nOuts, np.uint64)
    call("pil2gl_poseidon", _ptr(i), _ptr(c), 1, nOuts, _ptr(o))
    return [int(v) for v in o]


def poseidon_batch(inp, cap=None, nOuts=4):
    inp = np.ascontiguousarray(inp, dtype=np.uint64).reshape(-1, 8)
    if cap is not None:
        cap = np.ascontiguousarray(cap, dtype=np.uint64).reshape(-1, 4)
    out = np.zeros((inp.shape[0], nOuts), np.uint64)
    call("pil2gl_poseidon", _ptr(inp), _ptr(cap), inp.shape[0], nOuts, _ptr(out))
    return out


def linearHash(buffIn, width, splitLinearHash=False, out=None):
    n = int(np.prod(buffIn.shape))
    height = n // width if width else 0
    if _is_dev(buffIn):
        if out is None:
            out = torch.empty(height * 4, dtype=torch.int64, device=buffIn.device)
        call("pil2gl_linear_hash_rows_dev", _ptr(buffIn), width, height, int(bool(splitLinearHash)), _ptr(out), _stream())
    else:
        if out is None:
            out = np.zeros(height * 4, np.uint64)
        call("pil2gl_linear_hash_rows", _ptr(buffIn), width, height, int(bool(splitLinearHash)), _ptr(out))
    return out


def merkelizeLevel(buffIn, out=None):
    nOps = int(np.prod(buffIn.shape)) // 8
    if _is_dev(buffIn):
        if out is None:
            out = torch.empty(nOps * 4, dtype=torch.int64, device=buffIn.device)
        call("pil2gl_merkelize_level_dev", _ptr(buffIn), nOps, _ptr(out), _stream())
    else:
        if out is None:
            out = np.zeros(nOps * 4, np.uint64)
        call("pil2gl_merkelize_level", _ptr(buffIn), nOps, _ptr(out))
    return out


class _LinearHash:

    def __init__(self, split):
        self.split = bool(split)

    def hash(self, vals):
        flat = []
        for v in vals:
            if isinstance(v, (list, tuple, np.ndarray)):
                flat.extend(int(x) for x in v)
            else:
                flat.append(int(v))
        if not flat:
            return [0, 0, 0, 0]
        a = np.array(flat, dtype=np.uint64)
        return [int(x) for x in linearHash(a, len(flat), self.split)]


class MerkleHash:

    def __init__(self, splitLinearHash=False):
        self.splitLinearHash = bool(splitLinearHash)
        self.lh = _LinearHash(splitLinearHash)
        load()

    def _getNNodes(self, n):
        return int(load().pil2gl_merkle_num_nodes(n // 4))

    def merkelize(self, buff, width, height):
        if height <= 0:
            raise Pil2glError("height must be > 0")
        _check_len(buff, width * height, "buff")
        n_nodes = self._getNNodes(height * 4)
        if _is_dev(buff):
            nodes = torch.empty(n_nodes, dtype=torch.int64, device=buff.device)
            call("pil2gl_merkelize_dev", _ptr(buff), width, height, int(self.splitLinearHash), _ptr(nodes), _stream())
        else:
            nodes = np.zeros(n_nodes, np.uint64)
            call("pil2gl_merkelize", _ptr(buff), width, height, int(self.splitLinearHash), _ptr(nodes))
        return {"elements": buff, "nodes": nodes, "width": width, "height": height}

    def merkelizeDigests(self, leaves, height):
        n_nodes = self._getNNodes(height * 4)
        _check_len(leaves, height * 4, "leaves")
        nodes = torch.empty(n_nodes, dtype=torch.int64, device=leaves.device)
        nodes[:height * 4] = leaves.reshape(-1)[:height * 4]
        call("pil2gl_merkelize_digests_dev", _ptr(nodes), height, _stream())
        return nodes

    def getElement(self, tree, idx, subIdx):
        return _word(tree["elements"], tree["width"] * idx + subIdx)

    def root(self, tree):
        n = tree["nodes"]
        last = n[-4:]
        if _is_dev(last):
            last = last.cpu().numpy().view(np.uint64)
        return [int(v) for v in last]

    def getGroupProof(self, tree, idx):
        if idx < 0 or idx >= tree["height"]:
            raise Pil2glError("Out of range")
        width, height = tree["width"], tree["height"]
        if _is_dev(tree["nodes"]):
            vals = np.zeros(max(width, 1), np.uint64); sib = np.zeros((64, 4), np.uint64); nl = C.c_uint32()
            call("pil2gl_group_proof_dev", _ptr(tree["elements"]), _ptr(tree["nodes"]), width, height, idx,
                 _ptr(vals), _ptr(sib), C.byref(nl))
            return [int(v) for v in vals[:width]], [[int(x) for x in s] for s in sib[:nl.value]]
        el = tree["elements"].reshape(-1)
        v = [int(x) for x in el[idx * width:(idx + 1) * width]]
        nodes = tree["nodes"]; mp = []; offset = 0; n = height * 4
        while n > 4:
            si = (idx ^ 1) * 4
            mp.append([int(x) for x in nodes[offset + si:offset + si + 4]])
            nextN = ((n - 1) // 8 + 1) * 4
            offset += nextN * 2; n = nextN; idx >>= 1
        return v, mp

    def getGroupProofs(self, tree, idxs):
        if not _is_dev(tree["nodes"]):
            return [self.getGroupProof(tree, i) for i in idxs]
        width, height = tree["width"], tree["height"]
        for i in idxs:
            if i < 0 or i >= height:
                raise Pil2glError("Out of range")
        nl = 0; n = height * 4
        while n > 4:
            n = ((n - 1) // 8 + 1) * 4; nl += 1
        ii = np.array(idxs, dtype=np.uint64); out = np.zeros((len(idxs), width + 4 * nl), np.uint64); lv = C.c_uint32()
        call("pil2gl_group_proofs_dev", _ptr(tree["elements"]), _ptr(tree["nodes"]), width, height, _ptr(ii), len(idxs), _ptr(out), C.byref(lv))
        vals, sibs = out[:, :width].tolist(), out[:, width:].reshape(len(idxs), nl, 4).tolist()
        return list(zip(vals, sibs))

    def calculateRootFromGroupProof(self, mp, idx, vals):
        value = self.lh.hash(vals)
        for sib in mp:
            if idx & 1 == 0:
                value = poseidon(list(value) + list(sib))
            else:
                value = poseidon(list(sib) + list(value))
            idx >>= 1
        return value

    def calculateRootsFromGroupProofs(self, proofs, idxs):
        if not proofs:
            return []
        width, nl = len(proofs[0][0]), len(proofs[0][1])
        packed = np.zeros((len(proofs), width + 4 * nl), np.uint64)
        for q, (vals, sib) in enumerate(proofs):
            if len(vals) != width or len(sib) != nl:
                raise Pil2glError("openings of different shapes in one batch")
            packed[q, :width] = [int(v) % P for v in vals]
            packed[q, width:] = [int(x) % P for s_ in sib for x in s_]
        ii = np.array([int(i) for i in idxs], dtype=np.uint64); roots = np.zeros((len(proofs), 4), np.uint64)
        call("pil2gl_roots_from_group_proofs", _ptr(packed), width, nl, _ptr(ii), len(proofs), int(self.splitLinearHash), _ptr(roots))
        return [[int(v) for v in r] for r in roots]

    def verifyGroupProofs(self, root, proofs, idxs):
        return all(self.eqRoot(r, root) for r in self.calculateRootsFromGroupProofs(proofs, idxs))

    def eqRoot(self, r1, r2):
        return all(int(a) % P == int(b) % P for a, b in zip(r1, r2))

    def verifyGroupProof(self, root, mp, idx, groupElements):
        return self.eqRoot(self.calculateRootFromGroupProof(mp, idx, groupElements), root)

    def writeToFile(self, tree, fileName):
        with open(fileName, "wb") as f:
            np.array([tree["width"], tree["height"]], dtype="<u8").tofile(f)
            _to_host(tree["elements"]).astype("<u8", copy=False).tofile(f)
            _to_host(tree["nodes"]).astype("<u8", copy=False).tofile(f)

    def readFromFile(self, fileName, device=None):
        with open(fileName, "rb") as f:
            width, height = (int(v) for v in np.fromfile(f, dtype="<u8", count=2))
            elements = np.fromfile(f, dtype="<u8", count=width * height).astype(np.uint64)
            nodes = np.fromfile(f, dtype="<u8", count=self._getNNodes(height * 4)).astype(np.uint64)
        if device is not None:
            elements = torch.from_numpy(elements.view(np.int64)).to(device)
            nodes = torch.from_numpy(nodes.view(np.int64)).to(device)
        return {"elements": elements, "nodes": nodes, "width": width, "height": height}


def buildMerkleHash(splitLinearHash=False):
    return MerkleHash(splitLinearHash)


def _to_host(b):
    if _is_dev(b):
        return b.reshape(-1).cpu().numpy().view(np.uint64)
    return b.reshape(-1)


def _word(b, i):
    if _is_dev(b):
        return int(b.reshape(-1)[i:i + 1].cpu().numpy().view(np.uint64)[0])
    return int(b.reshape(-1)[i])


class Transcript:

    def __init__(self):
        self.state = [0, 0, 0, 0]
        self.pending = []
        self.out = []

    def getState(self):
        if self.pending:
            self.updateState()
        return self.state

    def getField(self):
        return [self.getFields1(), self.getFields1(), self.getFields1()]

    def getFields1(self):
        if not self.out:
            self.updateState()
        return self.out.pop(0)

    def put(self, a):
        flat = []

        def walk(v):
            if isinstance(v, (list, tuple, np.ndarray)):
                for x in v:
                    walk(x)
            else:
                flat.append(int(v) % P)
        walk(a)
        i = 0
        while i < len(flat):
            need = 8 - len(self.pending)
            if len(flat) - i < need:
                self.pending.extend(flat[i:]); self.out = []
                return
            n_full = 1 + (len(flat) - i - need) // 8
            take = need + 8 * (n_full - 1)
            blocks = np.array(self.pending + flat[i:i + take], dtype=np.uint64)
            if n_full == 1:
                self.out = poseidon(blocks.tolist(), self.state, 12)
            else:
                cap = np.array([int(x) % P for x in self.state], dtype=np.uint64); out = np.zeros(12, np.uint64)
                call("pil2gl_sponge_absorb", _ptr(blocks), n_full, _ptr(cap), _ptr(out))
                self.out = [int(v) for v in out]
            self.pending = []; self.state = self.out[:4]
            i += take

    def updateState(self):
        while len(self.pending) < 8:
            self.pending.append(0)
        self.out = poseidon(self.pending, self.state, 12)
        self.pending = []
        self.state = self.out[:4]

    def _add1(self, a):
        self.out = []
        self.pending.append(a)
        if len(self.pending) == 8:
            self.out = poseidon(self.pending, self.state, 12)
            self.pending = []
            self.state = self.out[:4]

    def getPermutations(self, n, nBits):
        totalBits = n * nBits
        NFields = (totalBits - 1) // 63 + 1
        fields = [self.getFields1() for _ in range(NFields)]
        res = []; curField = 0; curBit = 0
        for _ in range(n):
            a = 0
            for j in range(nBits):
                if (fields[curField] >> curBit) & 1:
                    a += 1 << j
                curBit += 1
                if curBit == 63:
                    curBit = 0; curField += 1
            res.append(a)
        return res


def _inv(a):
    return pow(int(a), P - 2, P)


def _root_of_unity(bits):
    w = 7277203076849721926
# ... 121 lines not shown
```

### pil2-stark-js_amd/python/pil2gl/_lib.py

```python
import ctypes as C
import os

_HERE = os.path.dirname(os.path.abspath(__file__))
PKG_ROOT = os.path.dirname(os.path.dirname(_HERE))
LIB_PATH = os.environ.get("PIL2GL_LIB") or os.path.join(PKG_ROOT, "lib", "libpil2gl.so")

u64p = C.POINTER(C.c_uint64)
vp = C.c_void_p


class Pil2glError(RuntimeError):
    pass


class GlxRef(C.Structure):
    _fields_ = [("kind", C.c_uint8), ("dim", C.c_uint8), ("section", C.c_uint16),
                ("prime", C.c_int32), ("index", C.c_uint32), ("pad_", C.c_uint32)]


class GlxOp(C.Structure):
    _fields_ = [("op", C.c_uint32), ("pad_", C.c_uint32), ("dest", GlxRef), ("src", GlxRef * 2)]


class GlxSection(C.Structure):
    _fields_ = [("ptr", C.c_void_p), ("width", C.c_uint64)]


class GlxCtx(C.Structure):
    _fields_ = [("nBits", C.c_uint32), ("primeShift", C.c_uint32), ("nSections", C.c_uint32),
                ("nScalars", C.c_uint32), ("sections", C.POINTER(GlxSection)), ("scalars", u64p)]


class BnxCtx(C.Structure):
    _fields_ = [("nBits", C.c_uint32), ("primeShift", C.c_uint32), ("nSections", C.c_uint32),
                ("nScalars", C.c_uint32), ("sections", C.POINTER(GlxSection)), ("scalars", u64p)]


class GlxProgram(C.Structure):
    _fields_ = [("nOps", C.c_uint32), ("nTmp", C.c_uint32), ("ops", C.POINTER(GlxOp))]


class EvalDesc(C.Structure):
    _fields_ = [("buf", C.c_void_p), ("width", C.c_uint64), ("offset", C.c_uint64),
                ("dim", C.c_uint32), ("levIndex", C.c_uint32)]


class TupleSide(C.Structure):
    _fields_ = [("base", C.c_void_p), ("stride", C.c_uint64), ("hostCols", C.c_void_p), ("sel", C.c_void_p),
                ("selStride", C.c_uint64), ("selCol", C.c_uint64)]


class G1Poly(C.Structure):
    _fields_ = [("first", C.c_uint64), ("rows", C.c_uint64), ("m", C.c_uint32), ("reserved", C.c_uint32)]


_U64, _U32, _I = C.c_uint64, C.c_uint32, C.c_int
SIGNATURES = {
    "pil2gl_init": (_I, [_I]),
    "pil2gl_shutdown": (None, []),
    "pil2gl_last_error": (C.c_char_p, []),
    "pil2gl_version": (_I, []),
    "pil2gl_device_info": (_I, [C.c_char_p, _U32, C.POINTER(_U32), C.POINTER(_U64)]),
    "pil2gl_dev_alloc": (_I, [_U64, C.POINTER(vp)]),
    "pil2gl_dev_free": (_I, [vp]),
    "pil2gl_dev_zero": (_I, [vp, _U64, vp]),
    "pil2gl_dev_upload": (_I, [vp, vp, _U64]),
    "pil2gl_add": (_U64, [_U64, _U64]),
    "pil2gl_mul": (_U64, [_U64, _U64]),
    "pil2gl_square": (_U64, [_U64]),
    "pil2gl_dev_download": (_I, [vp, vp, _U64]),
    "pil2gl_sync": (_I, [vp]),
    "pil2gl_host_alloc": (_I, [_U64, C.POINTER(vp)]),
    "pil2gl_host_free": (_I, [vp]),
    "pil2gl_host_register": (_I, [vp, _U64]),
    "pil2gl_host_unregister": (_I, [vp]),
    "pil2gl_dev_upload_async": (_I, [vp, vp, _U64]),
    "pil2gl_dev_download_async": (_I, [vp, vp, _U64]),
    "pil2gl_copy_after": (_I, [vp]),
    "pil2gl_copy_fence": (_I, [vp]),
    "pil2gl_copy_sync": (_I, []),
    "pil2gl_land_rows_dev": (_I, [vp, _U64, vp, _U64, _U64, C.POINTER(_U64), vp]),
    "pil2gl_dev_load_file": (_I, [C.c_char_p, _U64, _U64, _U64, vp, _U64, _U64, C.POINTER(_U64)]),
    "pil2gl_dev_save_file": (_I, [C.c_char_p, _U64, vp, _U64, _U64]),
    "pil2gl_interpolate": (_I, [vp, _U64, _U32, vp, _U32]),
    "pil2gl_interpolate_dev": (_I, [vp, _U64, _U32, vp, _U32, vp]),
    "pil2gl_interpolate_cosets_dev": (_I, [vp, _U64, _U32, vp, _U32, _U32, _U32, vp]),
    "pil2gl_extend_cosets_unshifted_dev": (_I, [vp, _U64, _U32, vp, _U32, _U32, _U32, vp]),
    "pil2gl_interpolate_cosets_ws_dev": (_I, [vp, _U64, _U32, vp, _U32, _U32, _U32, vp, vp]),
    "pil2gl_fft": (_I, [vp, _U64, _U32, vp]),
    "pil2gl_ifft": (_I, [vp, _U64, _U32, vp]),
    "pil2gl_fft_dev": (_I, [vp, _U64, _U32, vp, vp]),
    "pil2gl_ifft_dev": (_I, [vp, _U64, _U32, vp, vp]),
    "pil2gl_poseidon": (_I, [vp, vp, _U64, _U32, vp]),
    "pil2gl_poseidon_dev": (_I, [vp, vp, _U64, _U32, vp, vp]),
    "pil2gl_linear_hash_rows": (_I, [vp, _U64, _U64, _I, vp]),
    "pil2gl_linear_hash_rows_dev": (_I, [vp, _U64, _U64, _I, vp, vp]),
    "pil2gl_merkelize_level": (_I, [vp, _U64, vp]),
    "pil2gl_merkelize_level_dev": (_I, [vp, _U64, vp, vp]),
    "pil2gl_merkle_num_nodes": (_U64, [_U64]),
    "pil2gl_merkelize": (_I, [vp, _U64, _U64, _I, vp]),
    "pil2gl_merkelize_dev": (_I, [vp, _U64, _U64, _I, vp, vp]),
    "pil2gl_merkelize_digests_dev": (_I, [vp, _U64, vp]),
    "pil2gl_group_proof_dev": (_I, [vp, vp, _U64, _U64, _U64, vp, vp, C.POINTER(_U32)]),
    "pil2gl_group_proofs_dev": (_I, [vp, vp, _U64, _U64, vp, _U32, vp, C.POINTER(_U32)]),
    "pil2gl_roots_from_group_proofs": (_I, [vp, _U64, _U32, vp, _U32, C.c_int, vp]),
    "pil2gl_sponge_absorb": (_I, [vp, _U64, vp, vp]),
    "pil2gl_bn128_sponge_absorb": (_I, [vp, _U64, _U32, vp, vp]),
    "pil2gl_fri_fold": (_I, [vp, _U32, _U32, _U64, vp, vp]),
    "pil2gl_fri_fold_dev": (_I, [vp, _U32, _U32, _U64, vp, vp, vp]),
    "pil2gl_fri_verify_fold": (_I, [vp, _U32, _U32, vp, vp, vp]),
    "pil2gl_fri_verify_fold_dev": (_I, [vp, _U32, _U32, vp, vp, vp, vp]),
    "pil2gl_fri_transpose": (_I, [vp, _U32, _U32, vp]),
    "pil2gl_fri_transpose_dev": (_I, [vp, _U32, _U32, vp, vp]),
    "pil2gl_build_x_dev": (_I, [_U32, _U64, vp, vp]),
    "pil2gl_geometric_dev": (_I, [_U64, _U64, _U64, vp, vp]),
    "pil2gl_build_zhinv_dev": (_I, [_U32, _U32, vp, vp]),
    "pil2gl_build_one_row_zerofier_inv_dev": (_I, [_U32, _U32, _U64, vp, vp]),
    "pil2gl_build_frame_zerofier_dev": (_I, [_U32, _U32, _U64, _U64, vp, vp]),
    "pil2gl_compute_q_split_dev": (_I, [vp, _U32, _U32, _U32, _U32, vp, vp]),
    "pil2gl_compute_q_split_brev_dev": (_I, [vp, _U32, _U32, _U32, _U32, vp, vp]),
    "pil2gl_compute_q_stark_dev": (_I, [C.POINTER(GlxProgram), C.POINTER(GlxCtx), _U32, _U32, _U32, _U32, _U32, vp, vp]),
    "pil2gl_extend_coefs_brev_dev": (_I, [vp, _U64, _U32, vp, _U32, vp]),
    "pil2gl_extend_coefs_brev_cosets_dev": (_I, [vp, _U64, _U32, vp, _U32, _U32, _U32, vp]),
    "pil2gl_x_div_x_sub_xi_dev": (_I, [_U32, vp, _U64, _U64, vp, vp]),
    "pil2gl_x_div_x_sub_xi_cosets_dev": (_I, [_U32, _U32, vp, _U64, _U64, _U32, _U32, vp, vp]),
    "pil2gl_build_lev_dev": (_I, [_U32, vp, vp, vp]),
    "pil2gl_compute_evals_dev": (_I, [C.POINTER(EvalDesc), _U32, _U32, _U32, C.POINTER(vp), _U32, vp, vp]),
    "pil2gl_rows_dot_ext_dev": (_I, [vp, _U64, _U64, vp, _U32, vp, _I, vp]),
    "pil2gl_rows_dot_ext_multi_dev": (_I, [vp, vp, _U32, _U64, vp, _U32, vp, _I, vp]),
    "pil2gl_rows_dot_ext_multi_step_dev": (_I, [vp, vp, _U32, _U64, _U32, vp, _U32, vp, _I, vp]),
    "pil2gl_fri_combine_dev": (_I, [vp, vp, vp, vp, _U32, _U64, vp, vp]),
    "pil2gl_fri_combine_order_dev": (_I, [vp, vp, vp, vp, _U32, vp, _U64, vp, vp]),
    "pil2gl_compute_fri_pol_dev": (_I, [vp, vp, _U32, vp, _U32, vp, vp, vp, vp, _U32, _U32, vp, vp]),
    "pil2gl_cols_dot_ext_dev": (_I, [vp, _U64, _U64, _U64, C.POINTER(vp), _U32, vp, vp]),
    "pil2gl_cols_dot_ext_multi_dev": (_I, [vp, vp, _U32, _U64, _U64, vp, _U32, vp, vp]),
    "pil2gl_cols_dot_ext_range_dev": (_I, [vp, vp, vp, vp, _U32, _U64, _U64, vp, _U32, vp, vp]),
    "pil2gl_eval_program_dev": (_I, [C.POINTER(GlxProgram), C.POINTER(GlxCtx), vp]),
    "pil2gl_jit_cache_set_dir": (_I, [C.c_char_p]),
    "pil2gl_jit_cache_stats": (_I, [C.POINTER(_U64)]),
    "pil2gl_precompile_program": (_I, [C.POINTER(GlxProgram), C.POINTER(GlxCtx), C.POINTER(_U32)]),
    "pil2gl_precompile_q_stark": (_I, [C.POINTER(GlxProgram), C.POINTER(GlxCtx), _U32, _U32, _U32, _U32, _U32, C.POINTER(_U32)]),
    "pil2gl_first_nonzero_row_dev": (_I, [vp, _U32, _U64, _U64, vp, vp, vp]),
    "pil2gl_fft_block_dev": (_I, [vp, _U64, _U64, _U32, _U32, _U32, _U32, vp]),
    "pil2gl_interpolate_prepare_block_dev": (_I, [vp, _U64, _U64, _U64, _U64, vp]),
    "pil2gl_synth_fibonacci_dev": (_I, [_U32, _U32, vp, vp, vp]),
    "pil2gl_debug_compact_program": (_I, [C.POINTER(GlxProgram), C.POINTER(GlxOp), C.POINTER(_U32)]),
    "pil2gl_debug_jit_compile": (_I, [C.POINTER(GlxProgram), C.POINTER(GlxCtx), C.POINTER(_U64), C.POINTER(_U32)]),
    "pil2gl_debug_plan_program": (_I, [C.POINTER(GlxProgram), C.POINTER(GlxCtx), C.POINTER(_U32)]),
    "pil2gl_debug_plan_transform": (_I, [_U32, _U32, _U64, _U32, _U32, C.POINTER(_U32), _U32, C.POINTER(_U32)]),
    "pil2gl_debug_plan_transform_grid": (_I, [_U32, _U32, _U64, _U32, _U32, C.POINTER(_U32), _U32, C.POINTER(_U32)]),
    "pil2gl_debug_transform_walk": (_I, [_U32, _U32, _U64, _U32, _U32, _U32, _U32, _U32, vp]),
    "pil2gl_debug_transform_walk_cover": (_I, [_U32, _U32, _U64, _U32, _U32, _U32, C.POINTER(_U64)]),
    "pil2gl_gprod_dev": (_I, [vp, _U32, vp, _U32, _U64, vp, vp]),
    "pil2gl_gsum_dev": (_I, [vp, _U32, vp, _U32, _U64, vp, vp]),
    "pil2gl_h1h2_dev": (_I, [vp, vp, _U64, _U32, vp, vp, vp]),
    "pil2gl_debug_hint_plan": (_I, [_U64, C.POINTER(_U32)]),
    "pil2gl_debug_h1h2_home": (_U64, [vp, _U32, _U64]),
    "pil2gl_bn128_poseidon": (_I, [vp, vp, _U64, _U32, _U32, vp]),
    "pil2gl_bn128_poseidon_dev": (_I, [vp, vp, _U64, _U32, _U32, vp, vp]),
    "pil2gl_bn128_linear_hash_rows": (_I, [vp, _U64, _U64, _U32, _I, vp]),
    "pil2gl_bn128_linear_hash_rows_dev": (_I, [vp, _U64, _U64, _U32, _I, vp, vp]),
    "pil2gl_bn128_merkelize_level_dev": (_I, [vp, _U64, _U32, vp, vp]),
    "pil2gl_bn128_merkle_num_nodes": (_U64, [_U64, _U32]),
    "pil2gl_bn128_merkelize": (_I, [vp, _U64, _U64, _U32, _I, vp]),
    "pil2gl_bn128_merkelize_dev": (_I, [vp, _U64, _U64, _U32, _I, vp, vp]),
    "pil2gl_bn128_group_proof_dev": (_I, [vp, vp, _U64, _U64, _U32, _U64, vp, vp, vp]),
    "pil2gl_bn128_group_proofs_dev": (_I, [vp, vp, _U64, _U64, _U32, vp, _U32, vp, vp, vp]),
    "pil2gl_bn128_roots_from_group_proofs": (_I, [vp, vp, _U64, _U32, _U32, _I, _I, vp, _U32, vp]),
    "pil2gl_debug_bn128_path_launches": (_U64, []),
    "pil2gl_bn128_convert": (_I, [vp, _U64, _I, vp]),
    "pil2gl_bn128_convert_dev": (_I, [vp, _U64, _I, vp, vp]),
    "pil2gl_bn128_fft": (_I, [vp, _U64, _U32, vp]),
    "pil2gl_bn128_ifft": (_I, [vp, _U64, _U32, vp]),
    "pil2gl_bn128_interpolate": (_I, [vp, _U64, _U32, vp, vp, _U32]),
    "pil2gl_bn128_fft_dev": (_I, [vp, _U64, _U32, vp, vp]),
    "pil2gl_bn128_ifft_dev": (_I, [vp, _U64, _U32, vp, vp]),
    "pil2gl_bn128_interpolate_dev": (_I, [vp, _U64, _U32, vp, vp, _U32, vp]),
    "pil2gl_debug_bn128_fft_plan": (_I, [_U32, C.POINTER(_U32), _U32, C.POINTER(_U32)]),
    "pil2gl_debug_bn128_fft_tile_bytes": (_U32, []),
    "pil2gl_bn128_g1_msm": (_I, [vp, vp, _U64, _U64, _U32, vp]),
    "pil2gl_bn128_g1_msm_dev": (_I, [vp, vp, _U64, _U64, _U32, vp, vp]),
    "pil2gl_debug_bn128_msm_plan": (_I, [_U64, C.POINTER(_U32), C.POINTER(_U64)]),
    "pil2gl_bn128_g1_commit": (_I, [vp, _U64, vp, _U64, _U32, C.POINTER(G1Poly), _U32, C.POINTER(_U32), vp]),
    "pil2gl_bn128_g1_commit_dev": (_I, [vp, _U64, vp, _U64, _U32, C.POINTER(G1Poly), _U32, C.POINTER(_U32), vp, vp]),
    "pil2gl_debug_bn128_msm_batch_plan": (_I, [_U32, C.POINTER(_U64), C.POINTER(_U32), C.POINTER(_U64)]),
    "pil2gl_debug_bn128_commit_locate": (_I, [C.POINTER(G1Poly), _U32, C.POINTER(_U32), _U64, _U64, C.POINTER(_U64)]),
    "pil2gl_debug_bn128_msm_digits": (_I, [C.POINTER(_U64), _U32, C.POINTER(C.c_int32), _U32, C.POINTER(_U32)]),
    "pil2gl_bn128_eval_program": (_I, [C.POINTER(GlxProgram), C.POINTER(BnxCtx)]),
    "pil2gl_bn128_eval_program_dev": (_I, [C.POINTER(GlxProgram), C.POINTER(BnxCtx), vp]),
    "pil2gl_bn128_first_nonzero_row_dev": (_I, [vp, _U64, _U64, _U64, _U64, vp, vp, vp]),
    "pil2gl_debug_bn128_plan_program": (_I, [C.POINTER(GlxProgram), C.POINTER(BnxCtx), C.POINTER(_U32)]),
    "pil2gl_bn128_poly_div_xk_sub": (_I, [vp, _U64, _U64, _U64, vp, vp]),
    "pil2gl_bn128_poly_div_xk_sub_dev": (_I, [vp, _U64, _U64, _U64, vp, vp, vp]),
    "pil2gl_bn128_poly_eval": (_I, [vp, _U64, _U64, vp, _U32, vp]),
    "pil2gl_bn128_poly_eval_dev": (_I, [vp, _U64, _U64, vp, _U32, vp, vp]),
    "pil2gl_debug_bn128_poly_plan": (_I, [_U64, _U64, C.POINTER(_U32), C.POINTER(_U64)]),
    "pil2gl_bn128_poly_fma": (_I, [vp, _U64, _U64, vp, vp, _U64, _U64, vp, vp, _U32]),
    "pil2gl_bn128_poly_fma_dev": (_I, [vp, _U64, _U64, vp, vp, _U64, _U64, vp, vp, _U32, vp]),
    "pil2gl_bn128_poly_degree": (_I, [vp, _U64, _U64, C.POINTER(_U64)]),
    "pil2gl_bn128_poly_degree_dev": (_I, [vp, _U64, _U64, C.POINTER(_U64), vp]),
    "pil2gl_bn128_batch_inverse": (_I, [vp, _U64, _U64, vp, _U64]),
    "pil2gl_bn128_batch_inverse_dev": (_I, [vp, _U64, _U64, vp, _U64, vp]),
    "pil2gl_bn128_gprod": (_I, [vp, _U64, vp, _U64, _U64, vp, _U64]),
    "pil2gl_bn128_gprod_dev": (_I, [vp, _U64, vp, _U64, _U64, vp, _U64, vp]),
    "pil2gl_bn128_gsum": (_I, [vp, vp, _U64, _U64, vp, _U64]),
    "pil2gl_bn128_gsum_dev": (_I, [vp, vp, _U64, _U64, vp, _U64, vp]),
    "pil2gl_debug_bn128_scan_plan": (_I, [_U64, _U32, C.POINTER(_U32), C.POINTER(_U64)]),
    "pil2gl_bn128_h1h2": (_I, [vp, _U64, vp, _U64, _U64, vp, _U64, vp, _U64, C.POINTER(_U64)]),
    "pil2gl_bn128_h1h2_dev": (_I, [vp, _U64, vp, _U64, _U64, vp, _U64, vp, _U64, C.POINTER(_U64), vp]),
    "pil2gl_debug_bn128_h1h2_plan": (_I, [_U64, C.POINTER(_U32), C.POINTER(_U64)]),
    "pil2gl_wtns_adds_plan": (_I, [vp, _U64, _U64, _U64, vp, _U64, _U32, vp, vp, vp, _U32, C.POINTER(_U32)]),
    "pil2gl_wtns_adds_dev": (_I, [vp, _U64, vp, vp, _U64, vp, _U32, vp]),
    "pil2gl_bn128_wtns_adds_dev": (_I, [vp, _U64, vp, vp, _U64, vp, _U32, vp]),
    "pil2gl_wtns_gather_dev": (_I, [vp, _U64, vp, _U64, _U64, vp, _U64, C.POINTER(_U64), vp]),
    "pil2gl_bn128_wtns_gather_dev": (_I, [vp, _U64, vp, _U64, _U64, vp, _U64, _I, C.POINTER(_U64), vp]),
    "pil2gl_wtns_exec": (_I, [vp, _U64, vp, vp, _U64, vp, _U64, _U64, vp]),
    "pil2gl_bn128_wtns_exec": (_I, [vp, _U64, vp, vp, _U64, vp, _U64, _U64, vp, _I]),
    "pil2gl_debug_wtns_plan": (_I, [vp, _U64, _U64, _U64, C.POINTER(_U32), vp, _U32]),
    "pil2gl_conn_plan": (_I, [_U64, _U64, _U64, _U64, _U32, C.POINTER(_U32), C.POINTER(_U64)]),
    "pil2gl_conn_pols_dev": (_I, [vp, _U64, _U64, _U64, _U64, vp, vp, vp, _U64, _U64, vp, _U64, C.POINTER(_U64), vp]),
    "pil2gl_bn128_conn_pols_dev": (_I, [vp, _U64, _U64, _U64, _U64, vp, vp, vp, _U64, _U64, vp, _U64, C.POINTER(_U64), vp]),
    "pil2gl_conn_pols": (_I, [vp, _I, _U64, _U64, _U64, _U64, vp, vp, vp]),
    "pil2gl_bn128_conn_pols": (_I, [vp, _I, _U64, _U64, _U64, _U64, vp, vp, vp]),
    "pil2gl_conn_check_plan": (_I, [_U64, _U64, _U32, C.POINTER(_U32), C.POINTER(_U64)]),
    "pil2gl_conn_check_dev": (_I, [vp, _U64, _U64, vp, _U64, _U64, _U64, _U64, vp, vp, vp, _U64, vp, vp]),
    "pil2gl_bn128_conn_check_dev": (_I, [vp, _U64, _U64, vp, _U64, _U64, _U64, _U64, vp, vp, vp, _U64, vp, vp]),
    "pil2gl_conn_check": (_I, [vp, vp, _U64, _U64, vp, vp, vp]),
    "pil2gl_bn128_conn_check": (_I, [vp, vp, _U64, _U64, vp, vp, vp]),
    "pil2gl_debug_conn_check_probe": (_U64, []),
    "pil2gl_tuple_check_plan": (_I, [_U64, _U64, _U32, _U32, C.POINTER(_U32), C.POINTER(_U64)]),
    "pil2gl_tuple_check_dev": (_I, [vp, _U64, vp, vp, _U64, vp, vp, _U64, _U64, vp, _U64, _U64, _U64, _U64, _U32, vp, _U64, vp, vp]),
    "pil2gl_bn128_tuple_check_dev": (_I, [vp, _U64, vp, vp, _U64, vp, vp, _U64, _U64, vp, _U64, _U64, _U64, _U64, _U32, vp, _U64, vp, vp]),
    "pil2gl_tuple_check": (_I, [vp, _U64, vp, vp, _U64, vp, vp, _U64, _U64, vp, _U64, _U64, _U64, _U64, _U32, vp]),
    "pil2gl_bn128_tuple_check": (_I, [vp, _U64, vp, vp, _U64, vp, vp, _U64, _U64, vp, _U64, _U64, _U64, _U64, _U32, vp]),
    "pil2gl_debug_tuple_home": (_U64, [vp, _U64, _U32, _U64]),
    "pil2gl_debug_tuple_check_probe": (_U64, []),
    "pil2gl_lookup_mult_plan": (_I, [_U64, _U64, _U64, _U32, C.POINTER(_U32), C.POINTER(_U64)]),
    "pil2gl_lookup_mult_dev": (_I, [C.POINTER(TupleSide), _U64, C.POINTER(TupleSide), vp, _U64, _U64, _U64, _U64, vp, _U64, vp, vp]),
    "pil2gl_bn128_lookup_mult_dev": (_I, [C.POINTER(TupleSide), _U64, C.POINTER(TupleSide), vp, _U64, _U64, _U64, _U64, vp, _U64, vp, vp]),
    "pil2gl_lookup_mult": (_I, [C.POINTER(TupleSide), _U64, C.POINTER(TupleSide), vp, _U64, _U64, _U64, _U64, vp]),
    "pil2gl_bn128_lookup_mult": (_I, [C.POINTER(TupleSide), _U64, C.POINTER(TupleSide), vp, _U64, _U64, _U64, _U64, vp]),
    "pil2gl_debug_lookup_mult_probe": (_U64, []),
    "pil2gl_selftest_field":(_I, [vp, vp, _U64, vp, vp, vp]),
    "pil2gl_selftest_ext": (_I, [vp, vp, _U64, vp, vp]),
    "pil2gl_selftest_products": (_I, [vp, vp, _U64, vp, vp, vp]),
    "pil2gl_selftest_mds": (_I, [vp, _U64, _U32, _I, vp]),
    "pil2gl_selftest_poseidon": (_I, [vp, _U64, _I, vp]),
    "pil2gl_selftest_clock": (_I, [C.c_uint32, vp]),
}

_lib = None


def load():
    global _lib
    if _lib is not None:
        return _lib
    if not os.path.exists(LIB_PATH):
        raise Pil2glError("libpil2gl.so not built (%s): run `make -C pil2-stark-js_amd` or __graft_entry__.build(); "
                          "there is no CPU fallback" % LIB_PATH)
    L = C.CDLL(LIB_PATH)
    for name, (res, args) in SIGNATURES.items():
        fn = getattr(L, name)
        fn.restype = res
        fn.argtypes = args
    _lib = L
    return L


def check(rc):
    if rc != 0:
        msg = load().pil2gl_last_error()
        raise Pil2glError("pil2gl error %d: %s" % (rc, msg.decode() if msg else "?"))


def call(name, *args):
    check(getattr(load(), name)(*args))
```

### pil2-stark-js_amd/python/pil2gl/stark.py

```python
import ctypes as C

import numpy as np

from . import _lib
from ._lib import call

P = 0xFFFFFFFF00000001
SHIFT = 7
TMP, SEC, SCALAR = 0, 1, 2
OPC = {"add": 0, "sub": 1, "mul": 2, "copy": 3}


def _inv(a):
    return pow(int(a) % P, P - 2, P)


def root_of_unity(bits):
    w = 7277203076849721926
    for _ in range(32 - bits):
        w = w * w % P
    return w


def ext_mul(a, b):
# ... 500 lines not shown
            sec_index[name] = len(sections); sections.append(name)
        return sec_index[name]

    def scalar(v):
        off = len(scalars)
        if isinstance(v, (list, tuple, np.ndarray)):
            scalars.extend(int(x) % P for x in v); return off, 3
        scalars.append(int(v) % P); return off, 1

    def ref(r):
        t = r["type"]
        if t == "tmp":
            return (TMP, r["dim"], 0, 0, r["id"])
        if t == "const":
            return (SEC, 1, section("const_" + dom), r.get("prime", 0), r["id"])
        if t == "cm":
            p = info["cmPolsMap"][r["id"]]
            return (SEC, p["dim"], section("cm%d_%s" % (p["stage"], dom)), r.get("prime", 0), p["stagePos"])
        if t.startswith("tree"):
            return (SEC, r["dim"], section("cm%d_%s" % (int(t[4:]), dom)), 0, r["treePos"])
        if t == "q":
            return (SEC, r["dim"], section("q_ext"), 0, 0)
        if t == "f":
            return (SEC, 3, section("f_ext"), 0, 0)
        if t == "$ret":
            return (SEC, r["dim"], section("$ret"), 0, 0)
        if t == "x":
            return (SEC, r.get("dim", 1), section("x_" + dom), 0, 0)
        if t == "Zi":
            return (SEC, 1, section("Zi_ext#%d" % r["boundaryId"]), 0, 0)
        if t == "xDivXSubXi":
            return (SEC, 3, section("xDivXSubXi_ext"), 0, 3 * r["id"])
        if t == "number":
            v = r["value"]
            o, d = scalar(int(v, 0) if isinstance(v, str) else int(v)); return (SCALAR, d, 0, 0, o)
        if t == "public":
            o, d = scalar(ctx["publics"][r["id"]]); return (SCALAR, d, 0, 0, o)
        if t == "challenge":
            ch = ctx["challenges"][r["stage"] - 1][r["stageId"]] if "stage" in r else ctx["challengesFlat"][r["id"]]
            o, _ = scalar(ch); return (SCALAR, 3, 0, 0, o)
        if t == "subproofValue":
            sv = ctx["subproofValues"]
            v = sv[r["subproofId"]][r["id"]] if ctx.get("global") else sv[r["id"]]
            o, d = scalar(v); return (SCALAR, d, 0, 0, o)
        if t == "eval":
            o, _ = scalar(ctx["evals"][r["id"]]); return (SCALAR, 3, 0, 0, o)
        raise ValueError("Invalid reference type get: " + t)
    ops, n_tmp = [], 0
    for c in code:
        for r in [c["dest"]] + c["src"]:
            if r["type"] == "tmp":
                n_tmp = max(n_tmp, r["id"] + 1)
    for c in code:
        if c["op"] == "muladd":
            prod = (TMP, max(r.get("dim", 1) for r in c["src"][:2]), 0, 0, n_tmp)
            ops.append((OPC["mul"], prod, ref(c["src"][0]), ref(c["src"][1])))
            ops.append((OPC["add"], ref(c["dest"]), prod, ref(c["src"][2])))
            continue
        if c["op"] not in OPC:
            raise ValueError("Invalid op:" + c["op"])
        ops.append((OPC[c["op"]], ref(c["dest"]), ref(c["src"][0]), ref(c["src"][1]) if c["op"] != "copy" else None))
    if any(c["op"] == "muladd" for c in code):
        n_tmp += 1
    return ops, n_tmp, sections, np.array(scalars if scalars else [0], dtype=np.uint64)


def make_c_program(ops, n_tmp):
    arr = (_lib.GlxOp * len(ops))()
    for k, (op, d, s0, s1) in enumerate(ops):
        arr[k].op = op
        for tgt, r in ((arr[k].dest, d), (arr[k].src[0], s0), (arr[k].src[1], s1)):
            if r is not None:
                tgt.kind, tgt.dim, tgt.section, tgt.prime, tgt.index = r
    prog = _lib.GlxProgram(len(ops), n_tmp, arr)
    prog._keep = arr
    return prog


class GpuBackend:
    name = "gpu"

    def __init__(self, device=0, split=False, hash_type="GL", arity=16, custom=False):
        import torch
        import pil2gl
        self.torch, self.gl = torch, pil2gl
        pil2gl.init(device)
        self.dev = torch.device("cuda", device)
        self.hash_type, self.arity, self.custom = hash_type, arity, custom
        if hash_type == "BN128":
            from pil2gl import bn128
            self.bn = bn128
            self.MH = bn128.buildMerkleHash(arity, custom)
        else:
            self.MH = pil2gl.buildMerkleHash(split)

    def _st(self):
        return C.c_void_p(self.torch.cuda.current_stream().cuda_stream)

    def _p(self, t):
        return C.c_void_p(t.data_ptr())

    def empty(self, n):
        return self.torch.empty(int(n), dtype=self.torch.int64, device=self.dev)

    def zeros(self, n):
        return self.torch.zeros(int(n), dtype=self.torch.int64, device=self.dev)

    def from_host(self, a):
        return self.torch.from_numpy(np.ascontiguousarray(a, dtype=np.uint64).reshape(-1).view(np.int64)).to(self.dev)

    def to_host(self, t):
        return t.reshape(-1).cpu().numpy().view(np.uint64)

    def interpolate(self, src, C_, nb, dst, nbe): self.gl.interpolate(src, C_, nb, dst, nbe)
    def fft(self, src, C_, nb, dst): self.gl.fft(src, C_, nb, dst)
    def ifft(self, src, C_, nb, dst): self.gl.ifft(src, C_, nb, dst)
    def merkelize(self, buf, w, h): return self.MH.merkelize(buf, w, h)
    def interpolate_cosets(self, src, C_, nb, dst, nbe, cb, cc, ws=None): self.gl.interpolateCosets(src, C_, nb, dst, nbe, cb, cc, ws)
    def merkelize_digest_block(self, parts, N, cc, r, sliced=False):
        world = len(parts)
        nb_ = N // world
        h = nb_ * cc * world
        nodes = self.torch.empty(self.MH._getNNodes(h * 4), dtype=self.torch.int64, device=self.dev)
        leaf = nodes[:h * 4].view(nb_, world, cc * 4)
        for s_, part in enumerate(parts):
            leaf[:, s_, :] = (part.view(nb_, cc * 4) if sliced else part.view(N, cc * 4)[r * nb_:(r + 1) * nb_]).to(self.dev, non_blocking=True)
        self.gl.call("pil2gl_merkelize_digests_dev", self._p(nodes), h, self._st())
        return nodes

    def extend_cosets_unshifted(self, src, C_, nb, dst, nbe, cb, cc):
        call("pil2gl_extend_cosets_unshifted_dev", self._p(src), C_, nb, self._p(dst), nbe, cb, cc, self._st())

    def extend_coefs_brev_cosets(self, coef_brev, C_, nb, dst, nbe, cb, cc):
        call("pil2gl_extend_coefs_brev_cosets_dev", self._p(coef_brev), C_, nb, self._p(dst), nbe, cb, cc, self._st())

    def linear_hash_rows(self, buf, w, h): return self.gl.linearHash(buf[:w * h], w, self.MH.splitLinearHash)
    def linear_hash_rows_into(self, buf, w, h, out): self.gl.linearHash(buf[:w * h], w, self.MH.splitLinearHash, out=out)
    def merkelize_digests(self, leaves, h): return self.MH.merkelizeDigests(leaves, h)

    def merkelize_digest_parts(self, parts, N, cc):
        world, h = len(parts), N * cc * len(parts)
        nodes = self.torch.empty(self.MH._getNNodes(h * 4), dtype=self.torch.int64, device=self.dev)
        leaf = nodes[:h * 4].view(N, world, cc * 4)
        for r, part in enumerate(parts):
            leaf[:, r, :] = part.view(N, cc * 4).to(self.dev, non_blocking=True)
        self.gl.call("pil2gl_merkelize_digests_dev", self._p(nodes), h, self._st())
        return nodes
    def as_torch(self, t): return t
    def from_torch(self, t): return t.to(self.dev)
    def root(self, tree): return self.MH.root(tree)
    def group_proofs(self, tree, idxs):
        return self.MH.getGroupProofs(tree, idxs)

    def get_column(self, buf, width, off, dim, n): return buf.view(n, width)[:, off:off + dim].contiguous().reshape(-1)
    def set_column(self, buf, width, off, dim, n, col): buf.view(n, width)[:, off:off + dim] = col.view(n, dim)
    def gprod(self, num, dn, den, dd): return self.gl.calculateZ(num, den, dn, dd)
    def gsum(self, num, dn, den, dd): return self.gl.calculateS(num, den, dn, dd)
    def h1h2(self, f, t, dim): return self.gl.calculateH1H2(f, t, dim)

    def merkle_siblings(self, nodes, height, idxs):
        tree = {"elements": self.empty(1), "nodes": nodes, "width": 0, "height": height}
        return [mp for _, mp in self.MH.getGroupProofs(tree, idxs)]

    def new_transcript(self):
        if self.hash_type == "BN128":
            return self.bn.Transcript(self.arity if self.custom else 16)
        return self.gl.Transcript()
    def poseidon(self, inp, cap, n): return self.gl.poseidon(inp, cap, n)

    def build_x(self, nb, shift):
        x = self.empty(1 << nb); call("pil2gl_build_x_dev", nb, shift, self._p(x), self._st()); return x

    def geometric(self, first, ratio, n):
        o = self.empty(n); call("pil2gl_geometric_dev", int(first) % P, int(ratio) % P, int(n), self._p(o), self._st()); return o

    def build_zhinv(self, nb, nbe):
        z = self.empty(1 << nbe); call("pil2gl_build_zhinv_dev", nb, nbe, self._p(z), self._st()); return z

    def build_one_row_zerofier_inv(self, nb, nbe, row):
        z = self.empty(1 << nbe); call("pil2gl_build_one_row_zerofier_inv_dev", nb, nbe, row, self._p(z), self._st()); return z

    def build_frame_zerofier(self, nb, nbe, off_min, off_max):
        z = self.empty(1 << nbe); call("pil2gl_build_frame_zerofier_dev", nb, nbe, off_min, off_max, self._p(z), self._st()); return z

    def q_extend(self, qq1, nb, nbe, qDim, qDeg, out):
        c = self.empty((qDim * qDeg) << nb)
        call("pil2gl_compute_q_split_brev_dev", self._p(qq1), nb, nbe, qDim, qDeg, self._p(c), self._st())
        call("pil2gl_extend_coefs_brev_dev", self._p(c), qDim * qDeg, nb, self._p(out), nbe, self._st())

    def q_stark(self, ops, n_tmp, sections, scalars, q_section, nb, nbe, qDim, qDeg, out):
        prog = make_c_program(ops, n_tmp)
        cs = (_lib.GlxSection * len(sections))()
        for i, (t, w) in enumerate(sections):
            cs[i].ptr = None if t is None else t.data_ptr(); cs[i].width = w
        ctx = _lib.GlxCtx(nbe, nbe - nb, len(sections), scalars.size, cs, scalars.ctypes.data_as(_lib.u64p))
        call("pil2gl_compute_q_stark_dev", C.byref(prog), C.byref(ctx), q_section, nb, nbe, qDim, qDeg, self._p(out), self._st())

    def q_split(self, qq1, nb, nbe, qDim, qDeg):
        o = self.empty((qDim * qDeg) << nbe)
        call("pil2gl_compute_q_split_dev", self._p(qq1), nb, nbe, qDim, qDeg, self._p(o), self._st()); return o

    def x_div_x_sub_xi(self, nbe, xis):
        n_open = len(xis); o = self.empty((3 * n_open) << nbe)
        for i, xi in enumerate(xis):
            a = np.array([int(v) % P for v in xi], dtype=np.uint64)
            call("pil2gl_x_div_x_sub_xi_dev", nbe, C.c_void_p(a.ctypes.data), n_open, i, self._p(o), self._st())
        return o

    def x_div_x_sub_xi_cosets(self, nbe, eb, xis, cb, cc):
        n_open = len(xis); o = self.empty((3 * n_open * cc) << (nbe - eb))
        for i, xi in enumerate(xis):
            a = np.array([int(v) % P for v in xi], dtype=np.uint64)
            call("pil2gl_x_div_x_sub_xi_cosets_dev", nbe, eb, C.c_void_p(a.ctypes.data), n_open, i, cb, cc, self._p(o), self._st())
        return o

    def build_lev(self, nb, xi):
        o = self.empty(3 << nb); a = np.array([int(v) % P for v in xi], dtype=np.uint64)
        call("pil2gl_build_lev_dev", nb, C.c_void_p(a.ctypes.data), self._p(o), self._st()); return o

    def compute_evals(self, descs, nb, eb, levs):
        n = len(descs)
        d = (_lib.EvalDesc * n)()
        for i, (buf, width, off, dim, li) in enumerate(descs):
            d[i].buf = buf.data_ptr(); d[i].width = width; d[i].offset = off; d[i].dim = dim; d[i].levIndex = li
        lv = (C.c_void_p * len(levs))(*[t.data_ptr() for t in levs])
        res = np.zeros((n, 3), np.uint64)
        call("pil2gl_compute_evals_dev", d, n, nb, eb, lv, len(levs), C.c_void_p(res.ctypes.data), self._st())
        return [[int(v) for v in r] for r in res]

    def eval_program(self, ops, n_tmp, sections, scalars, nb, prime_shift):
        prog = make_c_program(ops, n_tmp)
        cs = (_lib.GlxSection * len(sections))()
        for i, (t, w) in enumerate(sections):
            cs[i].ptr = t.data_ptr(); cs[i].width = w
        ctx = _lib.GlxCtx(nb, prime_shift, len(sections), scalars.size, cs, scalars.ctypes.data_as(_lib.u64p))
        call("pil2gl_eval_program_dev", C.byref(prog), C.byref(ctx), self._st())

    def fri_polynomial_fast(self, info, bufs, widths, evals, vf1, vf2, nbe, f_ext):
        plan = fri_polynomial_plan(info, evals, vf2)
        if plan is None:
            return False
        coefs, K, n_open, order = plan
        acc = self.empty((3 * n_open) << nbe)
        names = list(coefs)
        ptrs = (C.c_void_p * len(names))(*[bufs[nm].data_ptr() for nm in names])
        ws = np.array([widths[nm] for nm in names], dtype=np.uint64)
        cps = (C.c_void_p * len(names))(*[coefs[nm].ctypes.data for nm in names])
        call("pil2gl_rows_dot_ext_multi_dev", ptrs, C.c_void_p(ws.ctypes.data), len(names), 1 << nbe, cps, n_open, self._p(acc), 0, self._st())
        v1 = np.array([int(c) % P for c in vf1], dtype=np.uint64)
        od = np.array(order, dtype=np.uint32)
        call("pil2gl_fri_combine_order_dev", self._p(acc), C.c_void_p(K.ctypes.data), C.c_void_p(v1.ctypes.data), self._p(bufs["xDivXSubXi_ext"]),
             n_open, C.c_void_p(od.ctypes.data), 1 << nbe, self._p(f_ext), self._st())
        return True

    def fri_polynomial(self, info, bufs, widths, evals, xis, vf1, vf2, nb, nbe, f_ext):
        plan = fri_polynomial_plan(info, evals, vf2)
        if plan is None:
            return False
        coefs, K, n_open, order = plan
        names = list(coefs)
        ptrs = (C.c_void_p * len(names))(*[bufs[nm].data_ptr() for nm in names])
        ws = np.array([widths[nm] for nm in names], dtype=np.uint64)
        cps = (C.c_void_p * len(names))(*[coefs[nm].ctypes.data for nm in names])
        v1 = np.array([int(c) % P for c in vf1], dtype=np.uint64)
        od = np.array(order, dtype=np.uint32)
        xs = np.array([[int(v) % P for v in xi] for xi in xis], dtype=np.uint64)
        call("pil2gl_compute_fri_pol_dev", ptrs, C.c_void_p(ws.ctypes.data), len(names), cps, n_open, C.c_void_p(K.ctypes.data),
             C.c_void_p(v1.ctypes.data), C.c_void_p(od.ctypes.data), C.c_void_p(xs.ctypes.data), nb, nbe, self._p(f_ext), self._st())
        return True

    def eval_matrices(self, info):
        return sorted({("const_ext" if ev["type"] == "const" else "cm%d_ext" % info["cmPolsMap"][ev["id"]]["stage"]) for ev in info["evMap"]})

    def col_sums(self, names, bufs, widths, nb, eb, levs, ranges=None):
        n_lev = len(levs)
        lv = (C.c_void_p * n_lev)(*[t.data_ptr() for t in levs])
        sums = {name: np.zeros((n_lev, widths[name], 3), np.uint64) for name in names}
        live = [nm for nm in names if ranges is None or ranges[nm][1] > ranges[nm][0]]
        for g0 in range(0, len(live), 8):
            grp = live[g0:g0 + 8]
            ptrs = (C.c_void_p * len(grp))(*[bufs[nm].data_ptr() for nm in grp])
            st = np.array([widths[nm] for nm in grp], dtype=np.uint64)
            c0 = np.array([0 if ranges is None else ranges[nm][0] for nm in grp], dtype=np.uint64)
            ws = np.array([widths[nm] if ranges is None else ranges[nm][1] - ranges[nm][0] for nm in grp], dtype=np.uint64)
            part = [np.zeros((n_lev, int(w), 3), np.uint64) for w in ws]
            outs = (C.c_void_p * len(grp))(*[p.ctypes.data for p in part])
            call("pil2gl_cols_dot_ext_range_dev", ptrs, C.c_void_p(st.ctypes.data), C.c_void_p(c0.ctypes.data), C.c_void_p(ws.ctypes.data), len(grp), 1 << nb, 1 << eb, lv, n_lev, outs, self._st())
            for nm, b, w, p in zip(grp, c0, ws, part):
                sums[nm][:, int(b):int(b) + int(w)] = p
        return sums

    def evals_fast(self, info, bufs, widths, nb, eb, levs):
        return evals_from_col_sums(info, self.col_sums(self.eval_matrices(info), bufs, widths, nb, eb, levs))

    def fri_fold(self, pol, pol_bits, out_bits, shift_inv, challenge):
        o = self.empty(3 << out_bits); ch = np.array([int(c) % P for c in challenge], dtype=np.uint64)
        call("pil2gl_fri_fold_dev", self._p(pol), pol_bits, out_bits, shift_inv, C.c_void_p(ch.ctypes.data), self._p(o), self._st()); return o

    def fri_transpose(self, pol, pol_bits, t_bits):
        o = self.empty(3 << pol_bits); call("pil2gl_fri_transpose_dev", self._p(pol), pol_bits, t_bits, self._p(o), self._st()); return o

    def sync(self):
        self.torch.cuda.synchronize()


def evals_from_col_sums(info, sums):
# ... 324 lines not shown
    for h in exprs.get("hintsInfo", []):
        for f in h["fields"]:
            if f.get("op") == "tmp":
                code, dim = _returning_code(exprs, f["id"])
                pre("hint %s.%s" % (h["name"], f["name"]), code, "n", dim)
    im = exprs.get("imPolsCode", [])
    if len(im) >= nStages and im[nStages - 1].get("code"):
        pre("imPols", im[nStages - 1]["code"], "n")
    c_code = expr_code(exprs, info["cExpId"])["code"]
    if quotient_in_one_call(info):
        ops, n_tmp, secs, scalars = encode_code(c_code, "ext", ctx)
        r = pil2gl.precompile_q_stark(ops, n_tmp, [widths[s_] for s_ in secs], scalars, secs.index("q_ext"), nb, nbe, info["qDim"], info["qDeg"])
        done.append(dict(r, program="constraint (sub-coset)"))
    else:
        pre("constraint", c_code, "ext")
    if fri_polynomial_plan(info, ctx["evals"], ctx["challenges"][nStages + 2][1]) is None:
        pre("fri", expr_code(exprs, info["friExpId"])["code"], "ext")
    return done


def stark_gen(be, cm1_n, setup, info, exprs, publics, timings=None):
    import time
    ss = info["starkStruct"]
    nb, nbe = ss["nBits"], ss["nBitsExt"]
    eb, E = nbe - nb, 1 << nbe
    qDim, qDeg = info["qDim"], info["qDeg"]
    nStages = info["nStages"]
    qStage = nStages + 1
    nC = info["nConstants"]
    nQ = info["mapSectionsN"]["cm%d" % qStage]
    assert ss["steps"][0]["nBits"] == nbe
    t_last = [time.perf_counter()]

    def lap(name):
        if timings is not None:
            be.sync(); now = time.perf_counter(); timings[name] = timings.get(name, 0.0) + now - t_last[0]; t_last[0] = now

    ctx = {"pilInfo": info, "publics": list(publics), "challenges": [[] for _ in range(nStages + 3)], "evals": [],
           "subproofValues": [0] * info.get("nSubproofValues", 0)}
    constTree = setup["constTree"]
    bufs = {"const_n": setup["const_n"], "const_ext": constTree["elements"], "cm1_n": cm1_n,
            "x_ext": be.build_x(nbe, SHIFT)}
    widths = section_widths(info)
    for bi, boundary in enumerate(info.get("boundaries", [{"name": "everyRow"}])):
        bufs["Zi_ext#%d" % bi] = build_zi_table(be, boundary, nb, nbe)
    transcript = be.new_transcript()
    hash_commits = bool(ss.get("hashCommits", False))
    transcript.put(setup["constRoot"])
    lap("init")

    def run(code, dom):
        ops, n_tmp, secs, scalars = encode_code(code["code"], dom, ctx)
        be.eval_program(ops, n_tmp, [(bufs[s], widths[s]) for s in secs], scalars, nb if dom == "n" else nbe, 0 if dom == "n" else eb)

    trees, roots = {}, {}
    for st in range(1, nStages + 1):
        name, w = "cm%d" % st, widths["cm%d_n" % st]
        if st > 1:
            n_ch = sum(1 for c in info["challengesMap"] if c["stage"] == st)
            ctx["challenges"][st - 1] = [transcript.getField() for _ in range(n_ch)]
            bufs[name + "_n"] = be.zeros(w << nb)
            if "x_n" not in bufs:
                bufs["x_n"] = be.build_x(nb, 1)
            for sc in exprs.get("stageCode", {}).get(st, []):
                run(sc, "n")
            resolve_hints(be, info, st, bufs, widths, nb, ctx, exprs)
            lap("stage%d_witness" % st)
        else:
            if exprs.get("hintsInfo"):
                resolve_hints(be, info, 1, bufs, widths, nb, ctx, exprs)
            put_commit(be, transcript, list(ctx["publics"]), hash_commits)
        if st == nStages:
            im = exprs.get("imPolsCode", [])
            if len(im) >= st and im[st - 1].get("code"):
                run(im[st - 1], "n")
                lap("im_pols")
        bufs[name + "_ext"] = be.empty(w << nbe)
        be.interpolate(bufs[name + "_n"], w, nb, bufs[name + "_ext"], nbe)
        lap("stage%d_lde" % st)
        trees[st] = be.merkelize(bufs[name + "_ext"], w, E)
        roots[st] = be.root(trees[st]); transcript.put(roots[st])
        lap("stage%d_merkle" % st)

    ctx["challenges"][qStage - 1] = [transcript.getField()]
    qname = "cm%d_ext" % qStage
    bufs[qname] = be.empty(nQ << nbe)
    if hasattr(be, "q_stark") and quotient_in_one_call(info):
        ops, n_tmp, secs, scalars = encode_code(expr_code(exprs, info["cExpId"])["code"], "ext", ctx)
        be.q_stark(ops, n_tmp, [(bufs.get(s), widths[s]) for s in secs], scalars, secs.index("q_ext"), nb, nbe, qDim, qDeg, bufs[qname])
        lap("q_expr")
    else:
        bufs["q_ext"] = be.empty(qDim << nbe)
        run(expr_code(exprs, info["cExpId"]), "ext")
        lap("q_expr")
        qq1 = be.empty(qDim << nbe)
        be.ifft(bufs["q_ext"], qDim, nbe, qq1)
        if hasattr(be, "q_extend") and nQ == qDim * qDeg:
            be.q_extend(qq1, nb, nbe, qDim, qDeg, bufs[qname])
            del qq1
        else:
            qq2 = be.q_split(qq1, nb, nbe, qDim, qDeg)
            del qq1
            be.fft(qq2, nQ, nbe, bufs[qname])
            del qq2
    lap("q_ntt")
    trees[qStage] = be.merkelize(bufs[qname], nQ, E)
    roots[qStage] = be.root(trees[qStage]); transcript.put(roots[qStage])
    lap("q_merkle")

    xi = transcript.getField()
    ctx["challenges"][qStage] = [xi]
    wN = root_of_unity(nb)
    levs, xis = [], []
    for opening in info["openingPoints"]:
        w = pow(wN, abs(opening), P)
        if opening < 0:
            w = _inv(w)
        xis.append(ext_scale(xi, w))
        levs.append(be.build_lev(nb, ext_scale(xi, w * _inv(SHIFT) % P)))
    descs = []
    for ev in info["evMap"]:
        li = info["openingPoints"].index(ev["prime"])
        if ev["type"] == "const":
            descs.append((bufs["const_ext"], nC, ev["id"], 1, li))
        else:
            p = info["cmPolsMap"][ev["id"]]
            descs.append((bufs["cm%d_ext" % p["stage"]], widths["cm%d_ext" % p["stage"]], p["stagePos"], p["dim"], li))
    if hasattr(be, "evals_fast") and len(levs) <= 64:
        ctx["evals"] = be.evals_fast(info, bufs, widths, nb, eb, levs)
    else:
        ctx["evals"] = be.compute_evals(descs, nb, eb, levs)
    del levs
    put_commit(be, transcript, ctx["evals"], hash_commits)
    lap("evals")

    vfs = [transcript.getField(), transcript.getField()]
    ctx["challenges"][qStage + 1] = vfs
    bufs["f_ext"] = be.empty(3 << nbe)
    if not (hasattr(be, "fri_polynomial") and be.fri_polynomial(info, bufs, widths, ctx["evals"], xis, vfs[0], vfs[1], nb, nbe, bufs["f_ext"])):
        bufs["xDivXSubXi_ext"] = be.x_div_x_sub_xi(nbe, xis)
        if not (hasattr(be, "fri_polynomial_fast") and be.fri_polynomial_fast(info, bufs, widths, ctx["evals"], vfs[0], vfs[1], nbe, bufs["f_ext"])):
            run(expr_code(exprs, info["friExpId"]), "ext")
        del bufs["xDivXSubXi_ext"]
    lap("fri_expr")

    steps = ss["steps"]
    friTrees, friProof, challengesFRI = fri_commit_phase(be, ss, bufs["f_ext"], transcript)
    friTrees[0] = [trees[st] for st in range(1, qStage + 1)] + [constTree]
    lap("fri_fold")

    chq = transcript.getField(); challengesFRI.append(chq)
    tq = be.new_transcript(); tq.put(chq)
    queries = tq.getPermutations(ss["nQueries"], steps[0]["nBits"])
    q = list(queries)
    for step in range(len(steps)):
        if step == 0:
            per_tree = [be.group_proofs(t, q) for t in friTrees[0]]
            friProof[0]["polQueries"] = [[list(per_tree[j][i]) for j in range(len(per_tree))] for i in range(len(q))]
        else:
            q = [qi % (1 << steps[step]["nBits"]) for qi in q]
            friProof[step]["polQueries"] = [list(p_) for p_ in be.group_proofs(friTrees[step], q)]
    lap("queries")
    proof = {"root%d" % st: roots[st] for st in range(1, qStage + 1)}
    proof["evals"] = ctx["evals"]; proof["fri"] = friProof
    if info.get("nSubproofValues"):
        proof["subproofValues"] = list(ctx.get("subproofValues", []))
    return {"proof": proof, "publics": list(ctx["publics"]), "challenges": ctx["challenges"], "challengesFRISteps": challengesFRI, "queries": queries}


def ext_inv(a):
    a, b, c = (int(v) % P for v in a)
    aa, ac, ba, bb, bc, cc = a * a % P, a * c % P, b * a % P, b * b % P, b * c % P, c * c % P
    t = (-aa * a - 2 * aa * c + 3 * ba * c + ba * b - ac * c - bb * b + bc * c - cc * c) % P
    ti = _inv(t)
    return [(-aa - 2 * ac + bc + bb - cc) * ti % P, (ba - cc) * ti % P, (-bb + ac + cc) * ti % P]


def _ext_op(op, a, b):
    ta, tb = isinstance(a, list), isinstance(b, list)
    if op == "mul":
        if ta and tb: return ext_mul(a, b)
        if ta: return [x * b % P for x in a]
        if tb: return [x * a % P for x in b]
        return a * b % P
    s = 1 if op == "add" else -1
    if ta and tb: return [(x + s * y) % P for x, y in zip(a, b)]
    if ta: return [(a[0] + s * b) % P, a[1], a[2]]
    if tb: return [(a + s * b[0]) % P, (s * b[1]) % P, (s * b[2]) % P]
    return (a + s * b) % P


def execute_code(code, resolve):
    tmp, res = {}, None
    for c in code:
        src = [tmp[r["id"]] if r["type"] == "tmp" else resolve(r) for r in c["src"]]
        if c["op"] == "muladd":
            res = _ext_op("add", _ext_op("mul", src[0], src[1]), src[2])
        else:
            res = src[0] if c["op"] == "copy" else _ext_op(c["op"], src[0], src[1])
        if c["dest"]["type"] == "tmp":
            tmp[c["dest"]["id"]] = res
    return res


def fri_values_at_queries(be, info, exprs, verifierInfo, proof, publics, challenges, queries, constRoot=None):
    ss = info["starkStruct"]
    nb, nbe, nQueries = ss["nBits"], ss["nBitsExt"], ss["nQueries"]
    qStage = info["nStages"] + 1
    xi = [int(v) for v in challenges[qStage][0]]
    pq0 = proof["fri"][0]["polQueries"]
    roots = list(range(qStage + 1))
    qb = max(1, (nQueries - 1).bit_length())
    rows = 1 << qb
    wN, wE = root_of_unity(nb), root_of_unity(nbe)
    nOpen = len(info["openingPoints"])
    xdiv = np.zeros((rows, 3 * nOpen), np.uint64)
    for i, idx in enumerate(queries):
        x = SHIFT * pow(wE, idx, P) % P
        for k, opening in enumerate(info["openingPoints"]):
            w = pow(wN, abs(opening), P)
            if opening < 0:
                w = _inv(w)
            xw = ext_scale(xi, w)
            xdiv[i, 3 * k:3 * k + 3] = ext_scale(ext_inv([(x - xw[0]) % P, (-xw[1]) % P, (-xw[2]) % P]), x)
    widths = {"const_ext": info["nConstants"], "xDivXSubXi_ext": 3 * nOpen, "f_ext": 3}
    host = {"xDivXSubXi_ext": xdiv}
    for j in range(len(roots)):
        name = "cm%d_ext" % (j + 1) if j < qStage else "const_ext"
        w = widths.setdefault(name, info["mapSectionsN"].get("cm%d" % (j + 1), 0))
        a = np.zeros((rows, w), np.uint64)
        for i in range(nQueries):
            a[i] = [int(v) % P for v in pq0[i][j][0]]
        host[name] = a
    ctx = {"pilInfo": info, "publics": list(publics), "challenges": challenges, "evals": proof["evals"], "subproofValues": proof.get("subproofValues", [])}
    code = list((verifierInfo.get("queryVerifier") or expr_code(exprs, info["friExpId"]))["code"])
    if code[-1]["dest"]["type"] == "tmp":
        code.append({"op": "copy", "dest": {"type": "f", "dim": 3}, "src": [code[-1]["dest"]]})
    ops, n_tmp, secs, scalars = encode_code(code, "ext", ctx)
    bufs = {s: be.from_host(host[s]) for s in secs if s in host}
    bufs["f_ext"] = be.zeros(3 * rows)
    be.eval_program(ops, n_tmp, [(bufs[s], widths[s]) for s in secs], scalars, qb, 0)
    vals = np.asarray(be.to_host(bufs["f_ext"])).view(np.uint64).reshape(rows, 3)
    return vals


def calculate_transcript(be, proof, publics, constRoot, info):
    ss = info["starkStruct"]
    steps, nQueries = ss["steps"], ss["nQueries"]
    nStages = info["nStages"]; qStage = nStages + 1
    t = be.new_transcript()
    hc = bool(info["starkStruct"].get("hashCommits", False))
    t.put(constRoot); put_commit(be, t, list(publics), hc)
    challenges = [[] for _ in range(nStages + 3)]
    for st in range(1, qStage + 1):
        if st > 1:
            n_ch = sum(1 for c in info["challengesMap"] if c["stage"] == st)
            challenges[st - 1] = [t.getField() for _ in range(n_ch)]
        t.put(proof["root%d" % st])
    challenges[qStage] = [t.getField()]
    put_commit(be, t, proof["evals"], hc)
    challenges[qStage + 1] = [t.getField(), t.getField()]
    chF = []
    for step in range(len(steps)):
        chF.append(t.getField())
        if step < len(steps) - 1:
            t.put(proof["fri"][step + 1]["root"])
        else:
            put_commit(be, t, proof["fri"][-1], hc)
    chF.append(t.getField())
    tq = be.new_transcript(); tq.put(chF[-1])
    return {"challenges": challenges, "challengesFRISteps": chF, "friQueries": tq.getPermutations(nQueries, steps[0]["nBits"])}


def stark_verify(be, proof, publics, constRoot, info, exprs, verifierInfo, challenges=None, legacy_transcript_queries=False):
    ss = info["starkStruct"]
    nb, nbe = ss["nBits"], ss["nBitsExt"]
    N, steps, nQueries = 1 << nb, ss["steps"], ss["nQueries"]
    nStages = info["nStages"]; qStage = nStages + 1
    tr = challenges if challenges is not None else calculate_transcript(be, proof, publics, constRoot, info)
    challenges, chF = tr["challenges"], tr["challengesFRISteps"]
    if legacy_transcript_queries and "friQueries" in tr:
        queries = tr["friQueries"]
    else:
        tq = be.new_transcript(); tq.put(chF[-1])
        queries = tq.getPermutations(nQueries, steps[0]["nBits"])
        if "friQueries" in tr and [int(q) for q in tr["friQueries"]] != [int(q) for q in queries]:
            return False, "query positions do not follow from the FRI challenge"
    xi = challenges[qStage][0]

    xN = ext_pow(xi, N)
    Zs = [zi_at(b_, xi, nb) for b_ in info.get("boundaries", [{"name": "everyRow"}])]

    def resolve(r):
        ty = r["type"]
        if ty == "eval": return [int(v) % P for v in proof["evals"][r["id"]]]
        if ty == "challenge": return [int(v) for v in challenges[r["stage"] - 1][r["stageId"]]]
        if ty == "public": return int(publics[r["id"]]) % P
        if ty == "number": return (int(r["value"], 0) if isinstance(r["value"], str) else int(r["value"])) % P
        if ty == "Zi": return list(Zs[r.get("boundaryId", 0)])
        if ty == "x": return [int(v) for v in xi]
        if ty == "subproofValue":
            v = proof["subproofValues"][r["id"]]
            return [int(x) % P for x in v] if isinstance(v, (list, tuple)) else int(v) % P
        raise ValueError("Invalid reference type get: " + ty)
    lhs = execute_code(verifierInfo["qVerifier"]["code"], resolve)
    lhs = lhs if isinstance(lhs, list) else [lhs, 0, 0]
    q_ids = [k for k, pm in enumerate(info["cmPolsMap"]) if pm["stage"] == qStage]
    q, xAcc = [0, 0, 0], [1, 0, 0]
    for i in range(info["qDeg"]):
        evId = next(k for k, e in enumerate(info["evMap"]) if e["type"] == "cm" and e["id"] == q_ids[i])
        q = _ext_op("add", q, ext_mul(xAcc, [int(v) % P for v in proof["evals"][evId]])); xAcc = ext_mul(xAcc, xN)
    if lhs != q:
        return False, "Invalid evaluations"

# ... 14 lines not shown
```

Measured before the change: 1.967 billion trace-cells/s.

## Memoize JIT expression kernels, batch FRI query openings, skip Merkle padding memset

Adds a memo keyed on program structure and scalar-equality pattern, so repeated expression evaluations reuse the compiled JIT function and only recompute the Horner weight limbs from a recorded recipe. This skips recompilation, source generation and cache lookup. Query openings for all FRI trees are gathered with a single batched kernel and one transfer each way, replacing one call per tree. The Merkle node memset is skipped when the height is a power of two. The memo key must capture every input that affects codegen, otherwise a wrong kernel could be reused.

Measured after the change: 1.973 billion trace-cells/s, median of 2. No clear change (+0.3%).

```diff
diff --git a/include/pil2gl.h b/include/pil2gl.h
--- a/include/pil2gl.h
+++ b/include/pil2gl.h
@@ -74,6 +74,9 @@
 
 int pil2gl_group_proofs_dev(const uint64_t *elems, const uint64_t *nodes, uint64_t width, uint64_t height,
                             const uint64_t *hostIdxs, uint32_t nIdx, uint64_t *hostOut, uint32_t *nLevels);
+typedef struct { const uint64_t *elems; const uint64_t *nodes; uint64_t width; uint64_t height; } pil2gl_tree_ref;
+int pil2gl_group_proofs_trees_dev(const pil2gl_tree_ref *trees, uint32_t nTrees, const uint64_t *hostIdxs, uint32_t nIdx,
+                                  uint64_t *hostOut, uint32_t *nLevels );
 int pil2gl_roots_from_group_proofs(const uint64_t *hostProofs, uint64_t width, uint32_t levels, const uint64_t *hostIdxs, uint32_t nIdx,
                                    int splitLinearHash, uint64_t *hostRoots );
 
@@ -312,6 +315,8 @@
 int pil2gl_debug_compact_program(const glx_program *prog, glx_op *outOps, uint32_t *outInfo);
 int pil2gl_debug_jit_compile(const glx_program *prog, const glx_ctx *ctx, uint64_t *codeBytes, uint32_t *fusedOps);
 int pil2gl_debug_plan_program(const glx_program *prog, const glx_ctx *ctx, uint32_t *outInfo);
+int pil2gl_debug_jit_memo_stats(uint64_t out[4]);
+int pil2gl_debug_jit_memo_check(const glx_program *prog, const glx_ctx *a, const glx_ctx *b, uint32_t out[3]);
 uint64_t pil2gl_debug_bn128_path_launches(void);
 #define PIL2GL_PLAN_FFT 0
 #define PIL2GL_PLAN_IFFT 1
diff --git a/pil2-stark-js_amd/csrc/expr.hip b/pil2-stark-js_amd/csrc/expr.hip
--- a/pil2-stark-js_amd/csrc/expr.hip
+++ b/pil2-stark-js_amd/csrc/expr.hip
@@ -225,7 +225,9 @@
     pool.push_back((u32)v & 0x3FFFFF); pool.push_back((u32)(v >> 22) & 0x3FFFFF); pool.push_back((u32)(v >> 44));
 }
 
-static void fuse_horner(std::vector<IOp> &ops, u32 nVal, const glx_ctx *ctx, std::vector<u32> &limbPool) {
+struct LimbRec { u32 x, power, dim; };
+
+static void fuse_horner(std::vector<IOp> &ops, u32 nVal, const glx_ctx *ctx, std::vector<u32> &limbPool, std::vector<LimbRec> *recipe) {
     const u32 NONE = 0xFFFFFFFFu;
     std::vector<u32> def(nVal, NONE), uses(nVal, 0);
     for (u32 k = 0; k < ops.size(); k++) {
@@ -277,8 +279,10 @@
         std::vector<std::array<u64, 3>> pw(n + 1);
         pw[0] = { 1, 0, 0 };
         for (u32 i = 1; i <= n; i++) { u64 t[3]; h_e3_mul(pw[i - 1].data(), xp, t); pw[i] = { t[0], t[1], t[2] }; }
-        auto weight = [&](const std::array<u64, 3> &W, u32 dim) {
+        auto weight = [&](u32 power, u32 dim) {
             const u32 off = (u32)limbPool.size();
+            const std::array<u64, 3> &W = pw[power];
+            if (recipe) recipe->push_back({ L.X.index, power, dim });
             std::array<u64, 3> w = W;
             for (u32 t = 0; t < dim; t++) {
                 for (int q = 0; q < 3; q++) push_limbs(limbPool, w[q]);
@@ -286,16 +290,16 @@
             }
             return off;
         };
-        auto mad = [&](const glx_ref &v, const std::array<u64, 3> &W) {
-            IOp m; memset(&m, 0, sizeof m); m.op = GLX_LZ_MAD; m.src[0] = v; m.aux = weight(W, v.dim); return m;
+        auto mad = [&](const glx_ref &v, u32 power) {
+            IOp m; memset(&m, 0, sizeof m); m.op = GLX_LZ_MAD; m.src[0] = v; m.aux = weight(power, v.dim); return m;
         };
         for (u32 i = 0; i < n; i++) { removed[chain[i].mulIdx] = true; removed[chain[i].addIdx] = true; consumed[chain[i].addIdx] = true; }
         IOp bg; memset(&bg, 0, sizeof bg); bg.op = GLX_LZ_BEGIN;
         insertAt[first].push_back(bg);
-        insertAt[first].push_back(mad(chain[n - 1].A, pw[n]));
+        insertAt[first].push_back(mad(chain[n - 1].A, n));
         for (u32 i = 0; i < n; i++) {
             const Link &lk = chain[n - 1 - i];
-            insertAt[lk.addIdx].push_back(mad(lk.C, pw[n - 1 - i]));
+            insertAt[lk.addIdx].push_back(mad(lk.C, n - 1 - i));
         }
         IOp en; memset(&en, 0, sizeof en); en.op = GLX_LZ_END; en.dest = ops[last].dest;
         insertAt[last].push_back(en);
@@ -338,11 +342,27 @@
     return PIL2GL_OK;
 }
 
-static int compile_program(const glx_program *prog, const glx_ctx *ctx, std::vector<IOp> &ops, u32 &nSlots, std::vector<u32> &limbPool, bool fuse) {
+static void limbs_from_recipe(const std::vector<LimbRec> &recipe, const u64 *scalars, std::vector<u32> &limbPool) {
+    std::map<u32, std::vector<std::array<u64, 3>>> powers;
+    limbPool.clear();
+    for (const LimbRec &r : recipe) {
+        std::vector<std::array<u64, 3>> &pw = powers[r.x];
+        if (pw.empty()) pw.push_back({ 1, 0, 0 });
+        while (pw.size() <= r.power) { u64 t[3]; h_e3_mul(pw.back().data(), scalars + r.x, t); pw.push_back({ t[0], t[1], t[2] }); }
+        std::array<u64, 3> w = pw[r.power];
+        for (u32 t = 0; t < r.dim; t++) {
+            for (int q = 0; q < 3; q++) push_limbs(limbPool, w[q]);
+            w = { w[2], h_add(w[0], w[2]), w[1] };
+        }
+    }
+}
+
+static int compile_program(const glx_program *prog, const glx_ctx *ctx, std::vector<IOp> &ops, u32 &nSlots, std::vector<u32> &limbPool, bool fuse,
+                           std::vector<LimbRec> *recipe = nullptr) {
     P2_TRY(validate_program(prog, ctx));
     u32 nVal = 0;
     P2_TRY(value_number(prog, ctx, ops, nVal));
-    if (fuse && ctx && ctx->scalars) fuse_horner(ops, nVal, ctx, limbPool);
+    if (fuse && ctx && ctx->scalars) fuse_horner(ops, nVal, ctx, limbPool, recipe);
     return allocate_slots(ops, nVal, nSlots);
 }
 
@@ -369,12 +389,16 @@
     const u64 *scalars; const u32 *limbs; u64 *sec[GLX_MAX_SECTIONS]; u32 nBits; u32 pad_;
 };
 struct JitEntry { hipModule_t mod; hipFunction_t fn; };
+struct JitMemo { hipFunction_t fn; size_t nOps; std::vector<LimbRec> recipe; };
+static std::map<std::string, JitMemo> g_jit_memo;
+static u64 g_jit_memo_stats[4];
 static std::map<std::string, JitEntry> g_jit_cache;
 namespace pil2gl {
 void jit_clear() {
     std::lock_guard<std::recursive_mutex> lk(runtime_lock());
     for (auto &kv : g_jit_cache) (void)hipModuleUnload(kv.second.mod);
     g_jit_cache.clear();
+    g_jit_memo.clear();
 }
 }
 
@@ -648,6 +672,40 @@
     if (!g_jit_dir.empty()) g_jit_stats[jit_disk_store(path, id, src, code) ? JS_DISK_WRITES : JS_FAILED_WRITES]++;
     return PIL2GL_OK;
 }
+static bool jit_memo_key(const glx_program *prog, const glx_ctx *ctx, std::string &key) {
+    key.clear();
+    auto put = [&](const void *p, size_t n) { key.append((const char *)p, n); };
+    auto put32 = [&](u32 v) { put(&v, 4); };
+    put32(1); put32(prog->nOps); put32(prog->nTmp);
+    put(prog->ops, (size_t)prog->nOps * sizeof(glx_op));
+    put32(ctx->nBits); put32(ctx->primeShift); put32(ctx->nSections); put32(ctx->nScalars); put32(ctx->scalars ? 1 : 0);
+    if (ctx->nSections && !ctx->sections) return false;
+    for (u32 i = 0; i < ctx->nSections; i++) put(&ctx->sections[i].width, 8);
+    std::map<std::array<u64, 4>, u32> first;
+    for (u32 k = 0; k < prog->nOps; k++) {
+        const glx_op &o = prog->ops[k];
+        if (o.op > GLX_OP_COPY) return false;
+        for (int s = 0; s < (o.op == GLX_OP_COPY ? 1 : 2); s++) {
+            const glx_ref &r = o.src[s];
+            if (r.kind != GLX_SCALAR) continue;
+            if ((r.dim != 1 && r.dim != 3) || (u64)r.index + r.dim > ctx->nScalars) return false;
+            u32 merged = r.index;
+            if (ctx->scalars) {
+                const u64 *w = ctx->scalars + r.index;
+                const std::array<u64, 4> v = { r.dim, w[0], r.dim == 3 ? w[1] : 0, r.dim == 3 ? w[2] : 0 };
+                merged = first.emplace(v, r.index).first->second;
+            }
+            put32(merged);
+        }
+    }
+    for (const char *name : { "PIL2GL_EXPR_JIT", "PIL2GL_EXPR_NOFUSE", "PIL2GL_EXPR_MULCALL", "PIL2GL_EXPR_LAZYMUL" }) {
+        const char *e = getenv(name);
+        key += e ? std::string("=") + e : std::string("-");
+        key.push_back('\0');
+    }
+    return true;
+}
+
 static int jit_get(const std::string &src, hipFunction_t *fn) {
     std::lock_guard<std::recursive_mutex> lk(runtime_lock());
     auto it = g_jit_cache.find(src);
@@ -681,8 +739,9 @@
     const bool want = e ? atoi(e) != 0 : (nOps >= 64 && nBits >= 16);
     return want && nSlots <= 200;
 }
-static int plan_program(const glx_program *prog, const glx_ctx *ctx, std::vector<IOp> &ops, u32 &nSlots, std::vector<u32> &limbPool) {
-    P2_TRY(compile_program(prog, ctx, ops, nSlots, limbPool, getenv("PIL2GL_EXPR_NOFUSE") == nullptr));
+static int plan_program(const glx_program *prog, const glx_ctx *ctx, std::vector<IOp> &ops, u32 &nSlots, std::vector<u32> &limbPool,
+                        std::vector<LimbRec> *recipe = nullptr) {
+    P2_TRY(compile_program(prog, ctx, ops, nSlots, limbPool, getenv("PIL2GL_EXPR_NOFUSE") == nullptr, recipe));
     if (ctx->nSections > GLX_MAX_SECTIONS) return fail(PIL2GL_EINVAL, "too many sections (%u > %d)", ctx->nSections, GLX_MAX_SECTIONS);
     for (size_t k = 0; k < ops.size(); k++)
         for (int s = 0; s < 3; s++) {
@@ -732,14 +791,74 @@
     return PIL2GL_OK;
 }
 
+static int jit_launch(hipFunction_t fn, size_t nOps, const glx_ctx *ctx, const u64 *dScalars, const u32 *dLimbs, hipStream_t st) {
+    if (getenv("PIL2GL_JIT_INFO") && getenv("PIL2GL_JIT_INFO")[0] == '1') {
+        int regs = 0, lds = 0, loc = 0, maxt = 0;
+        (void)hipFuncGetAttribute(&regs, HIP_FUNC_ATTRIBUTE_NUM_REGS, fn); (void)hipFuncGetAttribute(&lds, HIP_FUNC_ATTRIBUTE_SHARED_SIZE_BYTES, fn);
+        (void)hipFuncGetAttribute(&loc, HIP_FUNC_ATTRIBUTE_LOCAL_SIZE_BYTES, fn); (void)hipFuncGetAttribute(&maxt, HIP_FUNC_ATTRIBUTE_MAX_THREADS_PER_BLOCK, fn);
+        fprintf(stderr, "pil2gl jit_eval: %zu ops, regs %d, lds %d, scratch %d, max threads %d\n", nOps, regs, lds, loc, maxt);
+    }
+    JitArgs A; memset(&A, 0, sizeof A);
+    A.scalars = dScalars; A.limbs = dLimbs; A.nBits = ctx->nBits;
+    for (u32 i = 0; i < ctx->nSections; i++) A.sec[i] = ctx->sections[i].ptr;
+    size_t asz = sizeof A;
+    void *cfg[] = { HIP_LAUNCH_PARAM_BUFFER_POINTER, &A, HIP_LAUNCH_PARAM_BUFFER_SIZE, &asz, HIP_LAUNCH_PARAM_END };
+    const u64 nRows = 1ull << ctx->nBits;
+    HIP_TRY(hipModuleLaunchKernel(fn, (unsigned)((nRows + 255) / 256), 1, 1, 256, 1, 1, 0, st, nullptr, cfg));
+    { std::lock_guard<std::recursive_mutex> lk(runtime_lock()); g_jit_memo_stats[3] = (u64)(uintptr_t)fn; }
+    HIP_TRY(hipStreamSynchronize(st));
+    return PIL2GL_OK;
+}
+
+extern "C" int pil2gl_debug_jit_memo_stats(uint64_t out[4]) {
+    if (!out) return fail(PIL2GL_EINVAL, "null argument");
+    std::lock_guard<std::recursive_mutex> lk(runtime_lock());
+    for (int k = 0; k < 4; k++) out[k] = g_jit_memo_stats[k];
+    out[2] = g_jit_memo.size();
+    return PIL2GL_OK;
+}
+
+extern "C" int pil2gl_debug_jit_memo_check(const glx_program *prog, const glx_ctx *a, const glx_ctx *b, uint32_t out[3]) {
+    if (!prog || !a || !b || !out || (prog->nOps && !prog->ops)) return fail(PIL2GL_EINVAL, "null argument");
+    std::string ka, kb;
+    if (!jit_memo_key(prog, a, ka) || !jit_memo_key(prog, b, kb)) return fail(PIL2GL_EINVAL, "program or context not valid");
+    std::vector<IOp> oa, ob; std::vector<u32> pa, pb, rebuilt; std::vector<LimbRec> ra; u32 na = 0, nb = 0;
+    P2_TRY(plan_program(prog, a, oa, na, pa, &ra));
+    P2_TRY(plan_program(prog, b, ob, nb, pb));
+    const bool same = jit_source(oa, na, a) == jit_source(ob, nb, b);
+    out[0] = ka == kb;
+    if (out[0]) { if (b->scalars) limbs_from_recipe(ra, b->scalars, rebuilt); out[1] = same; out[2] = rebuilt == pb; }
+    else { out[1] = !same; out[2] = 0; }
+    return PIL2GL_OK;
+}
+
 extern "C" int pil2gl_eval_program_dev(const glx_program *prog, const glx_ctx *ctx, void *stream) {
     P2_TRY(ensure_init());
     if (!prog || !ctx || (prog->nOps && !prog->ops)) return fail(PIL2GL_EINVAL, "null program");
     if (ctx->nBits > 31) return fail(PIL2GL_EINVAL, "domain too large");
     if (prog->nOps == 0) return PIL2GL_OK;
     hipStream_t st = as_stream(stream);
+    std::string memoKey;
+    const bool keyed = jit_memo_key(prog, ctx, memoKey);
+    hipFunction_t memoFn = nullptr; size_t memoOps = 0;
+    std::vector<LimbRec> recipe;
+    if (keyed) {
+        std::lock_guard<std::recursive_mutex> lk(runtime_lock());
+        auto it = g_jit_memo.find(memoKey);
+        if (it != g_jit_memo.end()) { g_jit_memo_stats[0]++; g_jit_stats[JS_MEM_HITS]++; memoFn = it->second.fn; memoOps = it->second.nOps; recipe = it->second.recipe; }
+    }
+    if (memoFn) {
+        std::vector<u32> limbs;
+        if (ctx->scalars) limbs_from_recipe(recipe, ctx->scalars, limbs);
+        const u64 limbWords = (limbs.size() * 4 + 7) / 8;
+        u64 *d;
+        P2_TRY(scratch(SCR_EXPR_PROGRAM, ctx->nScalars + limbWords + 2, &d));
+        if (ctx->nScalars) HIP_TRY(hipMemcpyAsync(d, ctx->scalars, (u64)ctx->nScalars * 8, hipMemcpyHostToDevice, st));
+        if (!limbs.empty()) HIP_TRY(hipMemcpyAsync(d + ctx->nScalars + 1, limbs.data(), limbs.size() * 4, hipMemcpyHostToDevice, st));
+        return jit_launch(memoFn, memoOps, ctx, d, (const u32 *)(d + ctx->nScalars + 1), st);
+    }
     std::vector<IOp> ops; std::vector<u32> limbPool; u32 nSlots = 0;
-    P2_TRY(plan_program(prog, ctx, ops, nSlots, limbPool));
+    P2_TRY(plan_program(prog, ctx, ops, nSlots, limbPool, &recipe));
     std::vector<DevOp> dops(ops.size());
     for (size_t k = 0; k < ops.size(); k++) {
         auto cv = [&](const glx_ref &r) { DevRef d; d.kind_dim = (u32)r.kind | ((u32)r.dim << 8); d.section = r.section; d.rowOff = (int32_t)((int64_t)r.prime * ((int64_t)1 << ctx->primeShift)); d.index = r.index; return d; };
@@ -761,25 +880,17 @@
     {
         if (jit_routed(ops.size(), ctx->nBits, nSlots)) {
             hipFunction_t fn;
+            { std::lock_guard<std::recursive_mutex> lk(runtime_lock()); g_jit_memo_stats[1]++; }
             if (jit_get(jit_source(ops, nSlots, ctx), &fn) != PIL2GL_OK) {
                 static bool warned = false;
                 if (!warned) { fprintf(stderr, "pil2gl: run-time compilation unavailable (%s); using the interpreter kernel\n", pil2gl_last_error()); warned = true; }
                 goto interpreter;
             }
-            if (getenv("PIL2GL_JIT_INFO") && getenv("PIL2GL_JIT_INFO")[0] == '1') {
-                int regs = 0, lds = 0, loc = 0, maxt = 0;
-                (void)hipFuncGetAttribute(&regs, HIP_FUNC_ATTRIBUTE_NUM_REGS, fn); (void)hipFuncGetAttribute(&lds, HIP_FUNC_ATTRIBUTE_SHARED_SIZE_BYTES, fn);
-                (void)hipFuncGetAttribute(&loc, HIP_FUNC_ATTRIBUTE_LOCAL_SIZE_BYTES, fn); (void)hipFuncGetAttribute(&maxt, HIP_FUNC_ATTRIBUTE_MAX_THREADS_PER_BLOCK, fn);
-                fprintf(stderr, "pil2gl jit_eval: %zu ops, regs %d, lds %d, scratch %d, max threads %d\n", ops.size(), regs, lds, loc, maxt);
-            }
-            JitArgs A; memset(&A, 0, sizeof A);
-            A.scalars = c.scalars; A.limbs = c.limbs; A.nBits = ctx->nBits;
-            for (u32 i = 0; i < ctx->nSections; i++) A.sec[i] = ctx->sections[i].ptr;
-            size_t asz = sizeof A;
-            void *cfg[] = { HIP_LAUNCH_PARAM_BUFFER_POINTER, &A, HIP_LAUNCH_PARAM_BUFFER_SIZE, &asz, HIP_LAUNCH_PARAM_END };
-            HIP_TRY(hipModuleLaunchKernel(fn, (unsigned)((nRows + 255) / 256), 1, 1, 256, 1, 1, 0, st, nullptr, cfg));
-            HIP_TRY(hipStreamSynchronize(st));
-            return PIL2GL_OK;
+            if (keyed) {
+                std::lock_guard<std::recursive_mutex> lk(runtime_lock());
+                g_jit_memo[memoKey] = JitMemo{ fn, ops.size(), recipe };
+            }
+            return jit_launch(fn, ops.size(), ctx, c.scalars, c.limbs, st);
         }
     }
 interpreter:
diff --git a/pil2-stark-js_amd/csrc/merkle.hip b/pil2-stark-js_amd/csrc/merkle.hip
--- a/pil2-stark-js_amd/csrc/merkle.hip
+++ b/pil2-stark-js_amd/csrc/merkle.hip
@@ -258,6 +258,23 @@
     }
 }
 
+struct TreeDesc { const u64 *elems; const u64 *nodes; u64 width, height, outOff; u32 nLevels, pad_; };
+__global__ void group_proofs_trees_kernel(const TreeDesc *__restrict__ trees, const u64 *__restrict__ idxs, u32 nIdx, u64 *__restrict__ out) {
+    const TreeDesc T = trees[blockIdx.y];
+    const u64 stride = T.width + 4ull * T.nLevels;
+    u64 *o = out + T.outOff + (u64)blockIdx.x * stride;
+    u64 idx = idxs[(u64)blockIdx.y * nIdx + blockIdx.x];
+    for (u64 c = threadIdx.x; c < T.width; c += blockDim.x) o[c] = T.elems[idx * T.width + c];
+    if (threadIdx.x < 4) {
+        u64 offset = 0, n = T.height * 4;
+        for (u32 l = 0; l < T.nLevels; l++) {
+            o[T.width + 4 * l + threadIdx.x] = T.nodes[offset + (idx ^ 1) * 4 + threadIdx.x];
+            const u64 nextN = ((n - 1) / 8 + 1) * 4;
+            offset += nextN * 2; n = nextN; idx >>= 1;
+        }
+    }
+}
+
 }
 
 using namespace pil2gl;
@@ -317,7 +334,8 @@
     if (!nodes) return fail(PIL2GL_EINVAL, "null buffer");
     hipStream_t st = as_stream(stream);
     u64 total = pil2gl_merkle_num_nodes(height);
-    if (total > height * 4) HIP_TRY(hipMemsetAsync(nodes + height * 4, 0, (total - height * 4) * 8, st));
+    const bool noPadding = height >= 2 && (height & (height - 1)) == 0;
+    if (total > height * 4 && !noPadding) HIP_TRY(hipMemsetAsync(nodes + height * 4, 0, (total - height * 4) * 8, st));
     u64 pIn = 0, n64 = height * 4;
     u64 nextN64 = ((n64 - 1) / 8 + 1) * 4;
     u64 pOut = pIn + nextN64 * 2;
@@ -377,6 +395,37 @@
     return PIL2GL_OK;
 }
 
+int pil2gl_group_proofs_trees_dev(const pil2gl_tree_ref *trees, uint32_t nTrees, const uint64_t *hostIdxs, uint32_t nIdx,
+                                  uint64_t *hostOut, uint32_t *nLevels) {
+    P2_TRY(ensure_init());
+    if (!nTrees || !nIdx) return PIL2GL_OK;
+    if (!trees || !hostIdxs || !hostOut) return fail(PIL2GL_EINVAL, "null buffer");
+    if (nTrees > 65535) return fail(PIL2GL_EINVAL, "too many trees");
+    const u64 descWords = (u64)nTrees * (sizeof(TreeDesc) / 8), idxWords = (u64)nTrees * nIdx;
+    std::vector<u64> h(descWords + idxWords);
+    TreeDesc *desc = (TreeDesc *)h.data();
+    u64 outWords = 0;
+    for (u32 t = 0; t < nTrees; t++) {
+        const pil2gl_tree_ref &r = trees[t];
+        if (!r.nodes || !r.height || (!r.elems && r.width)) return fail(PIL2GL_EINVAL, "null buffer");
+        u32 lv = 0;
+        for (u64 n = r.height * 4; n > 4; n = ((n - 1) / 8 + 1) * 4) lv++;
+        for (u32 i = 0; i < nIdx; i++) if (hostIdxs[(u64)t * nIdx + i] >= r.height) return fail(PIL2GL_EINVAL, "Out of range");
+        desc[t].elems = r.elems; desc[t].nodes = r.nodes; desc[t].width = r.width; desc[t].height = r.height; desc[t].outOff = outWords;
+        desc[t].nLevels = lv; desc[t].pad_ = 0;
+        if (nLevels) nLevels[t] = lv;
+        outWords += (u64)nIdx * (r.width + 4ull * lv);
+    }
+    memcpy(h.data() + descWords, hostIdxs, idxWords * 8);
+    u64 *d;
+    P2_TRY(scratch(SCR_GROUP_PROOFS, h.size() + outWords, &d));
+    HIP_TRY(hipMemcpy(d, h.data(), h.size() * 8, hipMemcpyHostToDevice));
+    group_proofs_trees_kernel<<<dim3(nIdx, nTrees), 64>>>((const TreeDesc *)d, d + descWords, nIdx, d + h.size());
+    KERNEL_CHECK();
+    HIP_TRY(hipMemcpy(hostOut, d + h.size(), outWords * 8, hipMemcpyDeviceToHost));
+    return PIL2GL_OK;
+}
+
 int pil2gl_roots_from_group_proofs(const uint64_t *hostProofs, uint64_t width, uint32_t levels, const uint64_t *hostIdxs, uint32_t nIdx,
                                    int splitLinearHash, uint64_t *hostRoots) {
     P2_TRY(ensure_init());
diff --git a/pil2-stark-js_amd/python/pil2gl/__init__.py b/pil2-stark-js_amd/python/pil2gl/__init__.py
--- a/pil2-stark-js_amd/python/pil2gl/__init__.py
+++ b/pil2-stark-js_amd/python/pil2gl/__init__.py
@@ -354,6 +354,35 @@
         call("pil2gl_group_proofs_dev", _ptr(tree["elements"]), _ptr(tree["nodes"]), width, height, _ptr(ii), len(idxs), _ptr(out), C.byref(lv))
         vals, sibs = out[:, :width].tolist(), out[:, width:].reshape(len(idxs), nl, 4).tolist()
         return list(zip(vals, sibs))
+
+    def getGroupProofsTrees(self, trees, idx_lists):
+        from ._lib import TreeRef
+        n_idx = len(idx_lists[0])
+        refs = (TreeRef * len(trees))()
+        for t, (tree, idxs) in enumerate(zip(trees, idx_lists)):
+            if len(idxs) != n_idx or not _is_dev(tree["nodes"]):
+                raise Pil2glError("getGroupProofsTrees: device trees and index lists of one length")
+            for i in idxs:
+                if i < 0 or i >= tree["height"]:
+                    raise Pil2glError("Out of range")
+            refs[t].elems = tree["elements"].data_ptr(); refs[t].nodes = tree["nodes"].data_ptr()
+            refs[t].width = tree["width"]; refs[t].height = tree["height"]
+        nls = []
+        for tree in trees:
+            nl = 0; n = tree["height"] * 4
+            while n > 4:
+                n = ((n - 1) // 8 + 1) * 4; nl += 1
+            nls.append(nl)
+        ii = np.array(idx_lists, dtype=np.uint64).reshape(-1)
+        out = np.zeros(sum(n_idx * (tree["width"] + 4 * nl) for tree, nl in zip(trees, nls)), np.uint64)
+        lv = (C.c_uint32 * len(trees))()
+        call("pil2gl_group_proofs_trees_dev", refs, len(trees), _ptr(ii), n_idx, _ptr(out), lv)
+        res, o = [], 0
+        for tree, nl in zip(trees, nls):
+            w = tree["width"]
+            blk = out[o:o + n_idx * (w + 4 * nl)].reshape(n_idx, w + 4 * nl); o += blk.size
+            res.append(list(zip(blk[:, :w].tolist(), blk[:, w:].reshape(n_idx, nl, 4).tolist())))
+        return res
 
     def calculateRootFromGroupProof(self, mp, idx, vals):
         value = self.lh.hash(vals)
diff --git a/pil2-stark-js_amd/python/pil2gl/_lib.py b/pil2-stark-js_amd/python/pil2gl/_lib.py
--- a/pil2-stark-js_amd/python/pil2gl/_lib.py
+++ b/pil2-stark-js_amd/python/pil2gl/_lib.py
@@ -48,6 +48,10 @@
 class TupleSide(C.Structure):
     _fields_ = [("base", C.c_void_p), ("stride", C.c_uint64), ("hostCols", C.c_void_p), ("sel", C.c_void_p),
                 ("selStride", C.c_uint64), ("selCol", C.c_uint64)]
+
+
+class TreeRef(C.Structure):
+    _fields_ = [("elems", C.c_void_p), ("nodes", C.c_void_p), ("width", C.c_uint64), ("height", C.c_uint64)]
 
 
 class G1Poly(C.Structure):
@@ -103,6 +107,7 @@
     "pil2gl_merkelize_digests_dev": (_I, [vp, _U64, vp]),
     "pil2gl_group_proof_dev": (_I, [vp, vp, _U64, _U64, _U64, vp, vp, C.POINTER(_U32)]),
     "pil2gl_group_proofs_dev": (_I, [vp, vp, _U64, _U64, vp, _U32, vp, C.POINTER(_U32)]),
+    "pil2gl_group_proofs_trees_dev": (_I, [C.POINTER(TreeRef), _U32, vp, _U32, vp, C.POINTER(_U32)]),
     "pil2gl_roots_from_group_proofs": (_I, [vp, _U64, _U32, vp, _U32, C.c_int, vp]),
     "pil2gl_sponge_absorb": (_I, [vp, _U64, vp, vp]),
     "pil2gl_bn128_sponge_absorb": (_I, [vp, _U64, _U32, vp, vp]),
@@ -147,6 +152,8 @@
     "pil2gl_debug_compact_program": (_I, [C.POINTER(GlxProgram), C.POINTER(GlxOp), C.POINTER(_U32)]),
     "pil2gl_debug_jit_compile": (_I, [C.POINTER(GlxProgram), C.POINTER(GlxCtx), C.POINTER(_U64), C.POINTER(_U32)]),
     "pil2gl_debug_plan_program": (_I, [C.POINTER(GlxProgram), C.POINTER(GlxCtx), C.POINTER(_U32)]),
+    "pil2gl_debug_jit_memo_stats": (_I, [C.POINTER(_U64)]),
+    "pil2gl_debug_jit_memo_check": (_I, [C.POINTER(GlxProgram), C.POINTER(GlxCtx), C.POINTER(GlxCtx), C.POINTER(_U32)]),
     "pil2gl_debug_plan_transform": (_I, [_U32, _U32, _U64, _U32, _U32, C.POINTER(_U32), _U32, C.POINTER(_U32)]),
     "pil2gl_debug_plan_transform_grid": (_I, [_U32, _U32, _U64, _U32, _U32, C.POINTER(_U32), _U32, C.POINTER(_U32)]),
     "pil2gl_debug_transform_walk": (_I, [_U32, _U32, _U64, _U32, _U32, _U32, _U32, _U32, vp]),
diff --git a/pil2-stark-js_amd/python/pil2gl/stark.py b/pil2-stark-js_amd/python/pil2gl/stark.py
--- a/pil2-stark-js_amd/python/pil2gl/stark.py
+++ b/pil2-stark-js_amd/python/pil2gl/stark.py
@@ -676,6 +676,11 @@
     def group_proofs(self, tree, idxs):
         return self.MH.getGroupProofs(tree, idxs)
 
+    def group_proofs_trees(self, trees, idx_lists):
+        if self.hash_type == "BN128" or not all(isinstance(t, dict) for t in trees):
+            return [self.group_proofs(t, q) for t, q in zip(trees, idx_lists)]
+        return self.MH.getGroupProofsTrees(trees, idx_lists)
+
     def get_column(self, buf, width, off, dim, n): return buf.view(n, width)[:, off:off + dim].contiguous().reshape(-1)
     def set_column(self, buf, width, off, dim, n, col): buf.view(n, width)[:, off:off + dim] = col.view(n, dim)
     def gprod(self, num, dn, den, dd): return self.gl.calculateZ(num, den, dn, dd)
@@ -1306,14 +1311,18 @@
     chq = transcript.getField(); challengesFRI.append(chq)
     tq = be.new_transcript(); tq.put(chq)
     queries = tq.getPermutations(ss["nQueries"], steps[0]["nBits"])
-    q = list(queries)
-    for step in range(len(steps)):
-        if step == 0:
-            per_tree = [be.group_proofs(t, q) for t in friTrees[0]]
-            friProof[0]["polQueries"] = [[list(per_tree[j][i]) for j in range(len(per_tree))] for i in range(len(q))]
-        else:
-            q = [qi % (1 << steps[step]["nBits"]) for qi in q]
-            friProof[step]["polQueries"] = [list(p_) for p_ in be.group_proofs(friTrees[step], q)]
+    qs = [list(queries)]
+    for step in range(1, len(steps)):
+        qs.append([qi % (1 << steps[step]["nBits"]) for qi in qs[-1]])
+    n0 = len(friTrees[0])
+    all_trees, all_idxs = list(friTrees[0]) + friTrees[1:], [qs[0]] * n0 + qs[1:]
+    if hasattr(be, "group_proofs_trees"):
+        opened = be.group_proofs_trees(all_trees, all_idxs)
+    else:
+        opened = [be.group_proofs(t, ii) for t, ii in zip(all_trees, all_idxs)]
+    friProof[0]["polQueries"] = [[list(opened[j][i]) for j in range(n0)] for i in range(len(qs[0]))]
+    for step in range(1, len(steps)):
+        friProof[step]["polQueries"] = [list(p_) for p_ in opened[n0 + step - 1]]
     lap("queries")
     proof = {"root%d" % st: roots[st] for st in range(1, qStage + 1)}
     proof["evals"] = ctx["evals"]; proof["fri"] = friProof
```
